# fengpeng-yue/speech-to-speech-translation

Hardware: AMD Instinct MI355X
Metric: mel-frames/sec (fwd+bwd+opt) on Fisher-shaped fbank80->mel80 (higher is better)
Workload: dtype bf16; 1 GPU; s2st_transformer base 12enc/6dec d512 nfps4 + aux ASR/ST(1x64) + CTC, recipe dropouts, max-tokens=20000 Fisher-shaped batches, update-freq 1; parallelism=dp1

## Files before the change

### include/s2st_hip.h

```cpp
#ifndef S2ST_HIP_H
#define S2ST_HIP_H
#include <stdint.h>
#ifdef __cplusplus
extern "C" {
#endif

#define S2ST_OK 0
#define S2ST_ERR_LAUNCH (-1)
#define S2ST_ERR_SHAPE (-2)
#define S2ST_ERR_WORKSPACE (-3)
#define S2ST_ERR_ARG (-4)
#define S2ST_ERR_COMM (-5)

typedef struct { int64_t ld; int64_t bs; int32_t per; int32_t _pad; } s2st_split;

typedef struct {
  const void* p;
  int32_t kmajor;
  int32_t dtype;
  s2st_split sp;
  int64_t zo, zi;
} s2st_gemm_operand;

#define S2ST_F32 0
// ... 53 lines not shown
  float scale, drop_p;
  uint64_t seed;
  int32_t ld_drop;
  const uint16_t* doh;
  float *dq, *dk, *dv;
  uint16_t *dqh, *dkh, *dvh;
  float *dbq, *dbk, *dbv;
} s2st_attn_args;
int s2st_flash_attn_fwd_bf16(const s2st_attn_args* args, void* stream);
int s2st_flash_attn_bwd_bf16(const s2st_attn_args* args, const float* dO, float* dvec_scratch, void* stream);

int s2st_layernorm_fwd_f32(const float* x, const float* gamma, const float* beta, float* y, float* mean, float* rstd, int32_t rows, int32_t cols, float eps, void* stream);

int s2st_layernorm_bwd_f32(const float* dy, const float* x, const float* gamma, const float* mean, const float* rstd, float* dx, int32_t dx_accumulate, float* dgamma, float* dbeta, float* scratch, int32_t rows, int32_t cols, void* stream);
int64_t s2st_layernorm_bwd_scratch(int32_t rows, int32_t cols);

int s2st_softmax_fwd_f32(const float* s, float* p, float* pd, const int32_t* klen, int32_t B, int32_t H, int32_t T, int32_t S, int32_t ld, int32_t causal, float drop_p, uint64_t seed, void* stream);

int s2st_softmax_bwd_f32(const float* p, const float* dpd, float* ds, int32_t B, int32_t H, int32_t T, int32_t S, int32_t ld, float drop_p, uint64_t seed, void* stream);

int s2st_colsum_f32(const float* x, int64_t ld, int32_t rows, int32_t cols, float* out, int32_t accumulate, void* stream);

int s2st_attn_headmean_f32(const float* p, float* out, int32_t B, int32_t H, int32_t T, int32_t S, int32_t ld, void* stream);

int s2st_copy_rows_f32(const float* x, s2st_split xsp, float* y, s2st_split ysp, int32_t rows, int32_t C, void* stream);

int s2st_glu_fwd_f32(const float* a, float* y, s2st_split ysp, int32_t rows, int32_t C, void* stream);

int s2st_glu_bwd_f32(const float* a, const float* dy, s2st_split dysp, float* da, s2st_split dasp, int32_t rows, int32_t C, void* stream);

int s2st_add_pe_f32(const float* x, float* y, const int32_t* pos, const float* table, int32_t rows, int32_t C, float scale, const float* alpha_ptr, float drop_p, uint64_t seed, void* stream);

int s2st_pe_alpha_bwd_f32(const float* dy, const int32_t* pos, const float* table, int32_t rows, int32_t C, float drop_p, uint64_t seed, float* dalpha, void* stream);

int s2st_embed_fwd_f32(const int64_t* tokens, const float* table, float* y, int32_t rows, int32_t C, float scale, void* stream);

int s2st_embed_bwd_f32(const int64_t* tokens, const float* dy, float* dtable, int32_t rows, int32_t C, float scale, int64_t pad, void* stream);
int s2st_embed_bwd_ordered_f32(const int64_t* tokens, const float* dy, float* dtable, int32_t rows, int32_t C, int32_t V, float scale, int64_t pad, void* stream);

int s2st_dropout_f32(const float* x, float* y, int64_t n, float a, float p, uint64_t seed, int32_t accumulate, void* stream);

int s2st_relu_drop_bwd_f32(const float* dy, const float* y, float* dz, int64_t n, float p, void* stream);

int s2st_conv_w_permute_f32(const float* w, float* wf, float* wd, int32_t O, int32_t I, int32_t Kw, void* stream);

int s2st_conv_w_unpermute_acc_f32(const float* dwf, float* dw, int32_t O, int32_t I, int32_t Kw, void* stream);

#define S2ST_BN_TMP_FLOATS(C) (130 * (long)(C))
int s2st_bn_stats_f32(const float* x, int32_t rows, int32_t C, float* mean, float* var, float* run_mean, float* run_var, float momentum, float* tmp, void* stream);

int s2st_bn_apply_f32(const float* x, const float* mean, const float* var, const float* gamma, const float* beta, float* y, s2st_split ysp, const float* resid, int32_t rows, int32_t C, float eps, int32_t tanh_, float drop_p, uint64_t seed, void* stream);

int s2st_bn_bwd_f32(const float* dy, s2st_split dysp, const float* x, const float* mean, const float* var, const float* gamma, const float* beta, float* dx, s2st_split dxsp, float* dgamma, float* dbeta, float* tmp, int32_t rows, int32_t C, float eps, int32_t tanh_, float drop_p, uint64_t seed, void* stream);

int s2st_mel_loss_f32(const float* feat, const float* post, const float* eos, const float* tgt, const int32_t* lens, int32_t B, int32_t D, int32_t F, float pos_weight, float* stats, float c_l1, float c_mse, float c_eos, float* dfeat, float* dpost, float* deos, void* stream);

int s2st_ls_ce_f32(const float* logits, const int64_t* target, int32_t rows, int32_t V, int64_t pad, float eps, float* stats, float* dlogits, float gscale, void* stream);

int s2st_log_softmax_rows_f32(const float* x, int64_t ldx, float* y, int64_t ldy, int32_t rows, int32_t V, int32_t log_out, void* stream);

int s2st_ctc_f32(const float* logits, const int64_t* targets, int32_t Lmax, const int32_t* in_lens, const int32_t* tgt_lens, int32_t B, int32_t E, int32_t V, float* lprobs, float* loss_per_utt, float* dlogits, float gscale, float* ws, void* stream);

int s2st_sumsq_f32(const float* x, int64_t n, float* out, void* stream);
int s2st_sumsq_parts_f32(const float* x, int64_t n, float* parts, void* stream);
int64_t s2st_sumsq_parts_count(int64_t n);

int s2st_adam_f32(float* p, float* g, float* m, float* v, int64_t n, const float* sumsq, float gmul, const float* gmul_dev, float max_norm, float lr, float beta1, float beta2, float eps, float wd, int32_t step, float* gnorm_out, void* p_bf16, int32_t* skipped, int32_t sumsq_parts, int32_t zero_grad, void* stream);

int s2st_grad_pack_bf16_f32(const float* g, uint16_t* out, int64_t n, void* stream);
int s2st_exchange_proxy_f32(const float* bucket, float* scratch, int64_t n, int64_t move_bytes, int32_t wgs, float gbps, void* stream);
int s2st_grad_unpack_bf16_f32(const uint16_t* in, float* g, int64_t n, void* stream);

int64_t s2st_ctc_workspace(int32_t B, int32_t E, int32_t Lmax);

typedef struct {
  int32_t enc_layers, dec_layers, enc_dim, dec_dim, enc_ffn, dec_ffn, enc_heads, dec_heads;
  int32_t enc_pre_ln, dec_pre_ln;
  int32_t in_dim, conv_channels, conv_k;
  int32_t out_dim;
  int32_t prenet_layers, prenet_dim, postnet_layers, postnet_dim, postnet_k;
  int32_t tap_asr, tap_st;
  int32_t has_asr, has_st, has_ctc;
  int32_t asr_layers, asr_dim, st_layers, st_dim, src_vocab, tgt_vocab;
  int32_t no_scale_embedding;
  int32_t precise;
  int32_t tap_dec, has_ctc_tgt;
  int32_t text_input, enc_conv_layers, enc_conv_k;
  int32_t n_speakers, spk_frozen;
  int32_t spk_dim;
  float dropout, attn_dropout, act_dropout, prenet_dropout, postnet_dropout;
  float ctc_weight, asr_weight, st_weight, w_l1, w_mse, w_eos, bce_pos_weight, label_smoothing;
  float ctc_tgt_weight;
  float enc_dropout;
  int32_t s2t_mode;
} s2st_model_config;

typedef struct {
  char name[120];
  int64_t offset;
  int64_t numel;
  int32_t ndim;
  int32_t shape[4];
  int32_t is_buffer;
} s2st_param_info;

typedef struct {
// ... 250 lines not shown
```

### speech-to-speech-translation_amd/csrc/attention.hip

```cpp
#include <cstdlib>
#include <type_traits>

#include "s2st_ops.h"
#include "s2st_prof.h"

namespace {

typedef unsigned short bf16_t;

template <int DH>
struct Img {
  static constexpr int PITCH = DH * 2;
  static constexpr int CH = DH / 8;
  static constexpr int BYTES = 32 * PITCH;
  __device__ static __forceinline__ int trkey(int row) { return DH >= 128 ? (row & 7) : ((row >> 1) & 3); }
  __device__ static __forceinline__ int row_off(int row, int ch) { return row * PITCH + ((ch ^ (row & (CH - 1))) << 4); }
  __device__ static __forceinline__ int tr_off(int row, int ch) {
    return row * PITCH + (((((ch >> 1) ^ trkey(row)) << 1) | (ch & 1)) << 4);
  }
  __device__ static __forceinline__ bf16x8 row_frag(const unsigned char* img, int rt, int ks, int lane) {
    const int row = rt + (lane & 15), ch = 4 * ks + (lane >> 4);
    return *reinterpret_cast<const bf16x8*>(img + row_off(row, ch));
  }
  __device__ static __forceinline__ bf16x8 tr_frag(const unsigned char* img, int dt, int lane) {
// ... 187 lines not shown
#pragma unroll
    for (int t2 = 0; t2 < 2; ++t2) {
      x[t2] = f32x4{0.f, 0.f, 0.f, 0.f};
#pragma unroll
      for (int ks = 0; ks < KS; ++ks)
        x[t2] = __builtin_amdgcn_mfma_f32_16x16x32_bf16(Img<DH>::row_frag(kimg, 16 * t2, ks, lane), qf[ks], x[t2], 0, 0, 0);
    }
    float s[8];
    float mt = -INFINITY;
#pragma unroll
    for (int e = 0; e < 8; ++e) {
      const int key = kt + 16 * (e >> 2) + 4 * g + (e & 3);
      const bool ok = key < klim && (!a.causal || key <= qi);
      s[e] = ok ? x[e >> 2][e & 3] * a.scale : -INFINITY;
      mt = fmaxf(mt, s[e]);
    }
    mt = fmaxf(mt, __shfl_xor(mt, 16));
    mt = fmaxf(mt, __shfl_xor(mt, 32));
    const float mn = fmaxf(m, mt);
    const float mu = mn == -INFINITY ? 0.f : mn;
    const float alpha = __expf(m - mu);
    float p[8], ps = 0.f;
#pragma unroll
    for (int e = 0; e < 8; ++e) {
      p[e] = __expf(s[e] - mu);
      ps += p[e];
    }
    if (a.drop_p > 0.f) {
#pragma unroll
      for (int e = 0; e < 8; ++e)
        p[e] *= drop_scale(a.seed, drow + (uint64_t)(kt + 16 * (e >> 2) + 4 * g + (e & 3)), a.drop_p, inv_keep);
    }
    l = l * alpha + ps;
    m = mn;
    const bf16x8 pf = pack_frag(p);
#pragma unroll
    for (int d = 0; d < DT; ++d) {
      o[d] *= alpha;
      o[d] = __builtin_amdgcn_mfma_f32_16x16x32_bf16(Img<DH>::tr_frag(vimg, d, lane), pf, o[d], 0, 0, 0);
    }
  };
  for (int kt = 0; kt < kmax; kt += 64) {
    tile(stg[0], kt);
    if (kt + 32 < kmax) tile(stg[1], kt + 32);
  }
  l += __shfl_xor(l, 16);
  l += __shfl_xor(l, 32);
  const float inv_l = l > 0.f ? 1.f / l : 0.f;
  if (qi < a.T) {
    const long ro = ((long)b * a.T + qi) * ((long)a.H * DH) + h * DH;
#pragma unroll
    for (int d = 0; d < DT; ++d) {
      const float4 v = make_float4(o[d][0] * inv_l, o[d][1] * inv_l, o[d][2] * inv_l, o[d][3] * inv_l);
      *reinterpret_cast<float4*>(a.o + ro + 16 * d + 4 * g) = v;
      if (a.oh) *reinterpret_cast<uint2*>(a.oh + ro + 16 * d + 4 * g) = pack_bf16x4(v.x, v.y, v.z, v.w);
    }
    if (g == 0 && a.lse) a.lse[(long)bh * a.T + qi] = l > 0.f ? m + __logf(l) : -INFINITY;
  }
}

template <int DH>
__global__ __launch_bounds__(256) void attn_dvec_kernel(const float* __restrict__ dO, const float* __restrict__ O,
                                                        float* __restrict__ D, int B, int H, int T) {
  constexpr int LPR = DH / 4;
  const long row = ((long)blockIdx.x * 256 + threadIdx.x) / LPR;
  const int l = threadIdx.x % LPR;
  const bool ok = row < (long)B * T * H;
  float s = 0.f;
  int h = 0;
  long bt = 0;
  if (ok) {
    h = (int)(row % H);
    bt = row / H;
    const long o = bt * ((long)H * DH) + (long)h * DH + 4 * l;
    const float4 a = *reinterpret_cast<const float4*>(dO + o);
    const float4 c = *reinterpret_cast<const float4*>(O + o);
    s = a.x * c.x + a.y * c.y + a.z * c.z + a.w * c.w;
  }
#pragma unroll
  for (int m = LPR / 2; m >= 1; m >>= 1) s += __shfl_xor(s, m);
  if (ok && l == 0) {
    const int t = (int)(bt % T), bb = (int)(bt / T);
    D[((long)bb * H + h) * T + t] = s;
  }
}

template <int DH, int NW>
__device__ __forceinline__ void flash_bwd_kv_body(const AttnArgs& a, unsigned char* smem, const int bx, const int bh) {
  constexpr int KS = DH / 32, DT = DH / 16;
  unsigned char* q_row = smem;
  unsigned char* q_tr = smem + Img<DH>::BYTES;
  unsigned char* do_row = smem + 2 * Img<DH>::BYTES;
  unsigned char* do_tr = smem + 3 * Img<DH>::BYTES;
  const int tid = threadIdx.x, lane = tid & 63, wave = tid >> 6, g = lane >> 4;
  const int b = bh / a.H, h = bh - b * a.H;
  const int k0 = bx * (16 * NW) + wave * 16;
  const int ki = k0 + (lane & 15);
  const bf16_t* qb = a.q + (long)b * a.T * a.ldq + h * DH;
  const bf16_t* kb = a.k + (long)b * a.S * a.ldk + h * DH;
  const bf16_t* vb = a.v + (long)b * a.S * a.ldv + h * DH;
  const bf16_t* dob = a.doh + (long)b * a.T * ((long)a.H * DH) + h * DH;
  const int klim = a.klen ? min((int)a.klen[b], a.S) : a.S;
  const bool key_ok = ki < klim;
  const int qbeg = a.causal ? (bx * (16 * NW)) & ~31 : 0;

  ATTN_STAMP(0);
  bf16x8 kf[KS], vf[KS];
// ... 474 lines not shown
  const float inv_keep = a.drop_p > 0.f ? 1.f / (1.f - a.drop_p) : 1.f;
  const uint64_t drow = ((uint64_t)bh * a.T + qi) * (uint64_t)a.ld_drop;
  for (int kt = 0; kt < kmax; kt += 32) {
    f32x4 x[2];
#pragma unroll
    for (int t2 = 0; t2 < 2; ++t2) {
      x[t2] = f32x4{0.f, 0.f, 0.f, 0.f};
#pragma unroll
      for (int ks = 0; ks < KS; ++ks)
        x[t2] = __builtin_amdgcn_mfma_f32_16x16x32_bf16(I::row_frag(kimg, kt + 16 * t2, ks, lane), qf[ks], x[t2], 0, 0, 0);
    }
    float sc[8];
    float mt = -INFINITY;
#pragma unroll
    for (int e = 0; e < 8; ++e) {
      const int key = kt + 16 * (e >> 2) + 4 * g + (e & 3);
      const bool ok = key < klim && (!a.causal || key <= qi);
      sc[e] = ok ? x[e >> 2][e & 3] * a.scale : -INFINITY;
      mt = fmaxf(mt, sc[e]);
    }
    mt = fmaxf(mt, __shfl_xor(mt, 16));
    mt = fmaxf(mt, __shfl_xor(mt, 32));
    const float mn = fmaxf(m, mt);
    const float mu = mn == -INFINITY ? 0.f : mn;
    const float alpha = __expf(m - mu);
    float p[8], ps = 0.f;
#pragma unroll
    for (int e = 0; e < 8; ++e) {
      p[e] = __expf(sc[e] - mu);
      ps += p[e];
    }
    if (a.drop_p > 0.f) {
#pragma unroll
      for (int e = 0; e < 8; ++e)
        p[e] *= drop_scale(a.seed, drow + (uint64_t)(kt + 16 * (e >> 2) + 4 * g + (e & 3)), a.drop_p, inv_keep);
    }
    l = l * alpha + ps;
    m = mn;
    const bf16x8 pf = pack_frag(p);
#pragma unroll
    for (int d = 0; d < DT; ++d) {
      o[d] *= alpha;
      o[d] = __builtin_amdgcn_mfma_f32_16x16x32_bf16(I::tr_frag(vimg, kt, d, lane), pf, o[d], 0, 0, 0);
    }
  }
  l += __shfl_xor(l, 16);
  l += __shfl_xor(l, 32);
  const float inv_l = l > 0.f ? 1.f / l : 0.f;
  if (qi < a.T) {
    const long ro = ((long)b * a.T + qi) * ((long)a.H * DH) + h * DH;
#pragma unroll
    for (int d = 0; d < DT; ++d) {
      const float4 v = make_float4(o[d][0] * inv_l, o[d][1] * inv_l, o[d][2] * inv_l, o[d][3] * inv_l);
      *reinterpret_cast<float4*>(a.o + ro + 16 * d + 4 * g) = v;
      if (a.oh) *reinterpret_cast<uint2*>(a.oh + ro + 16 * d + 4 * g) = pack_bf16x4(v.x, v.y, v.z, v.w);
    }
    if (g == 0 && a.lse) a.lse[(long)bh * a.T + qi] = l > 0.f ? m + __logf(l) : -INFINITY;
  }
}

constexpr int ANW = 4;
constexpr int attn_nw() { return ANW; }

bool short_configure() {
  static int ok = -1;
  if (ok < 0) {
    auto set = [](auto kern, int bytes) {
      return hipFuncSetAttribute(reinterpret_cast<const void*>(kern), hipFuncAttributeMaxDynamicSharedMemorySize, bytes) == hipSuccess;
    };
    ok = set(flash_fwd_short_kernel<128, 8>, short_fwd_lds_bytes(128, 128)) && set(flash_fwd_short_kernel<64, 8>, short_fwd_lds_bytes(64, 128)) &&
         set(flash_fwd_short_kernel<128, 4>, short_fwd_lds_bytes(128, 64)) && set(flash_fwd_short_kernel<64, 4>, short_fwd_lds_bytes(64, 64)) &&
         set(flash_bwd_short_kernel<128, 8>, short_lds_bytes(128, 128, 128)) && set(flash_bwd_short_kernel<64, 8>, short_lds_bytes(64, 128, 128)) &&
         set(flash_bwd_short_kernel<128, 4>, short_lds_bytes(128, 64, 64)) && set(flash_bwd_short_kernel<64, 4>, short_lds_bytes(64, 64, 64)) ? 1 : 0;
  }
  return ok == 1;
}
bool short_enabled() {
  const char* e = s2st_env_str("S2ST_ATTN_SHORT");
  return !(e && atoi(e) == 0);
}
bool short_fwd_enabled() { return short_enabled(); }

bool attn_args_ok(const s2st_attn_args& p) {
  auto al = [](const void* x, int n) { return ((uintptr_t)x % n) == 0; };
  return (p.dh == 64 || p.dh == 128) && p.ldq % 8 == 0 && p.ldk % 8 == 0 && p.ldv % 8 == 0 && al(p.q, 16) &&
         al(p.k, 16) && al(p.v, 16) && p.B > 0 && p.H > 0 && p.T > 0 && p.S > 0;
}

AttnArgs to_args(const s2st_attn_args& p) {
  AttnArgs a{};
  a.q = p.q; a.k = p.k; a.v = p.v;
  a.ldq = p.ldq; a.ldk = p.ldk; a.ldv = p.ldv;
  a.o = p.o; a.oh = p.oh; a.lse = p.lse; a.klen = p.klen;
  a.B = p.B; a.H = p.H; a.T = p.T; a.S = p.S; a.causal = p.causal;
  a.scale = p.scale; a.drop_p = p.drop_p; a.seed = p.seed; a.ld_drop = p.ld_drop;
  a.doh = p.doh; a.dq = p.dq; a.dk = p.dk; a.dv = p.dv;
  a.dqh = p.dqh; a.dkh = p.dkh; a.dvh = p.dvh; a.dbq = p.dbq; a.dbk = p.dbk; a.dbv = p.dbv;
  a.plain_order = 0;
  return a;
}

}

int s2st_flash_attn_supported(int dh) { return dh == 64 || dh == 128; }

int s2st_flash_attn_preload(hipStream_t st) {
  AttnArgs a{};
  auto go = [&](auto nwc) {
    constexpr int NW = decltype(nwc)::value;
    S2ST_LAUNCH((flash_fwd_kernel<128, NW>), dim3(1, 1), dim3(64 * NW), 0, st, a);
    S2ST_LAUNCH((flash_fwd_kernel<64, NW>), dim3(1, 1), dim3(64 * NW), 0, st, a);
    S2ST_LAUNCH((flash_bwd_kv_kernel<128, NW>), dim3(1, 1), dim3(64 * NW), 0, st, a);
    S2ST_LAUNCH((flash_bwd_kv_kernel<64, NW>), dim3(1, 1), dim3(64 * NW), 0, st, a);
    S2ST_LAUNCH((flash_bwd_q_kernel<128, NW>), dim3(1, 1), dim3(64 * NW), 0, st, a);
    S2ST_LAUNCH((flash_bwd_q_kernel<64, NW>), dim3(1, 1), dim3(64 * NW), 0, st, a);
    S2ST_LAUNCH((flash_bwd_kernel<128, NW>), dim3(1, 1), dim3(64 * NW), 0, st, a, 1);
    S2ST_LAUNCH((flash_bwd_kernel<64, NW>), dim3(1, 1), dim3(64 * NW), 0, st, a, 1);
  };
  go(std::integral_constant<int, ANW>{});
  if (!short_configure()) return S2ST_ERR_LAUNCH;
  S2ST_LAUNCH((flash_fwd_short_kernel<128, 8>), dim3(1), dim3(512), 0, st, a);
  S2ST_LAUNCH((flash_fwd_short_kernel<64, 8>), dim3(1), dim3(512), 0, st, a);
  S2ST_LAUNCH((flash_fwd_short_kernel<128, 4>), dim3(1), dim3(256), 0, st, a);
  S2ST_LAUNCH((flash_fwd_short_kernel<64, 4>), dim3(1), dim3(256), 0, st, a);
  S2ST_LAUNCH((flash_bwd_short_kernel<128, 8>), dim3(1), dim3(512), 0, st, a);
  S2ST_LAUNCH((flash_bwd_short_kernel<64, 8>), dim3(1), dim3(512), 0, st, a);
  S2ST_LAUNCH((flash_bwd_short_kernel<128, 4>), dim3(1), dim3(256), 0, st, a);
  S2ST_LAUNCH((flash_bwd_short_kernel<64, 4>), dim3(1), dim3(256), 0, st, a);
  return hipGetLastError() == hipSuccess ? 0 : S2ST_ERR_LAUNCH;
}

int s2st_flash_attn_fwd(const s2st_attn_args* p, hipStream_t st) {
  if (!p || !attn_args_ok(*p) || !p->o || !p->lse) return S2ST_ERR_ARG;
  AttnArgs a = to_args(*p);
  if (p->T <= SHORT_MAX && p->S <= SHORT_MAX && short_fwd_enabled() && short_configure()) {
    const double fl = 4.0 * p->B * p->H * (double)p->T * p->S * p->dh * (p->causal ? 0.5 : 1.0);
    const dim3 grid(p->B * p->H);
    const int lds = short_fwd_lds_bytes(p->dh, p->S);
    const bool w4 = p->T <= 64 && p->S <= 64;
    if (p->dh == 128 && w4) s2st_launch("flash_fwd_short_kernel<128, 4>", fl, 0.0, flash_fwd_short_kernel<128, 4>, grid, dim3(256), lds, st, a);
    else if (p->dh == 128) s2st_launch("flash_fwd_short_kernel<128, 8>", fl, 0.0, flash_fwd_short_kernel<128, 8>, grid, dim3(512), lds, st, a);
    else if (w4) s2st_launch("flash_fwd_short_kernel<64, 4>", fl, 0.0, flash_fwd_short_kernel<64, 4>, grid, dim3(256), lds, st, a);
    else s2st_launch("flash_fwd_short_kernel<64, 8>", fl, 0.0, flash_fwd_short_kernel<64, 8>, grid, dim3(512), lds, st, a);
    return hipGetLastError() == hipSuccess ? 0 : S2ST_ERR_LAUNCH;
  }
  auto go = [&](auto nwc) {
    constexpr int NW = decltype(nwc)::value;
    dim3 grid((p->T + 16 * NW - 1) / (16 * NW), p->B * p->H);
    const double fl = 4.0 * p->B * p->H * (double)p->T * p->S * p->dh * (p->causal ? 0.5 : 1.0);
    if (p->dh == 128) s2st_launch("flash_fwd_kernel<128>", fl, 0.0, flash_fwd_kernel<128, NW>, grid, dim3(64 * NW), 0, st, a);
    else s2st_launch("flash_fwd_kernel<64>", fl, 0.0, flash_fwd_kernel<64, NW>, grid, dim3(64 * NW), 0, st, a);
  };
  go(std::integral_constant<int, ANW>{});
  return hipGetLastError() == hipSuccess ? 0 : S2ST_ERR_LAUNCH;
}

long s2st_flash_attn_db_scratch_floats(const s2st_attn_args* p) {
  if (!p || (!p->dbq && !p->dbk && !p->dbv)) return 0;
  const int nw = attn_nw();
  const long C = (long)p->H * p->dh;
  const long sq = (long)p->B * ((p->T + 16 * nw - 1) / (16 * nw)) * nw, sk = (long)p->B * ((p->S + 16 * nw - 1) / (16 * nw)) * nw;
  return (sq + 2 * sk) * C;
}

void s2st_flash_attn_db_layout(const s2st_attn_args* p, int* slots_q, int* slots_k) {
  const int nw = attn_nw();
  *slots_q = p->B * ((p->T + 16 * nw - 1) / (16 * nw)) * nw;
  *slots_k = p->B * ((p->S + 16 * nw - 1) / (16 * nw)) * nw;
}

int s2st_flash_attn_bwd(const s2st_attn_args* p, const float* dO, float* dvec_scratch, hipStream_t st, int phase,
                        float* db_part) {
  if (!p || !attn_args_ok(*p) || !p->doh || (!p->dq && !p->dqh) || (!p->dk && !p->dkh) || (!p->dv && !p->dvh) || !p->lse)
    return S2ST_ERR_ARG;
  const bool own_d = p->oh && phase == 0;
  if (!own_d && (!dO || !dvec_scratch || !p->o)) return S2ST_ERR_ARG;
  AttnArgs a = to_args(*p);
  a.dvec = own_d ? nullptr : dvec_scratch;
#ifdef S2ST_ATTN_STAMP
  a.stamp = reinterpret_cast<long*>(dvec_scratch);
#endif
  const int nwp = attn_nw();
  const long Cp = (long)p->H * p->dh;
  const long slots_q = (long)p->B * ((p->T + 16 * nwp - 1) / (16 * nwp)) * nwp, slots_k = (long)p->B * ((p->S + 16 * nwp - 1) / (16 * nwp)) * nwp;
  const bool part = db_part && phase == 0 && (p->dbq || p->dbk || p->dbv);
  if (part) {
// ... 85 lines not shown
```

### speech-to-speech-translation_amd/csrc/c_api.cpp

```cpp
#include <hip/hip_ext.h>
#include "s2st_ops.h"

extern "C" {

int s2st_version(void) { return 100; }

int s2st_experimental_build(void) {
#ifdef S2ST_EXPERIMENTAL
  return 1;
#else
  return 0;
#endif
}

int s2st_device_count(void) {
  int n = 0;
  if (hipGetDeviceCount(&n) != hipSuccess) return 0;
  return n;
}

int s2st_exchange_proxy_f32(const float* bucket, float* scratch, int64_t n, int64_t move_bytes, int32_t wgs, float gbps, void* stream) {
  return s2st_exchange_proxy(bucket, scratch, (long)n, (long)move_bytes, wgs, gbps, (hipStream_t)stream);
}
int s2st_grad_pack_bf16_f32(const float* g, uint16_t* out, int64_t n, void* stream) {
// ... 50 lines not shown
}

int s2st_glu_bwd_f32(const float* a, const float* dy, s2st_split dysp, float* da, s2st_split dasp, int32_t rows, int32_t C, void* stream) {
  return s2st_glu_bwd(a, dy, dysp, da, dasp, rows, C, (hipStream_t)stream);
}

int s2st_add_pe_f32(const float* x, float* y, const int32_t* pos, const float* table, int32_t rows, int32_t C, float scale, const float* alpha_ptr, float drop_p, uint64_t seed, void* stream) {
  return s2st_add_pe(x, y, pos, table, rows, C, scale, alpha_ptr, drop_p, seed, (hipStream_t)stream);
}

int s2st_pe_alpha_bwd_f32(const float* dy, const int32_t* pos, const float* table, int32_t rows, int32_t C, float drop_p, uint64_t seed, float* dalpha, void* stream) {
  return s2st_pe_alpha_bwd(dy, pos, table, rows, C, drop_p, seed, dalpha, (hipStream_t)stream);
}

int s2st_embed_fwd_f32(const int64_t* tokens, const float* table, float* y, int32_t rows, int32_t C, float scale, void* stream) {
  return s2st_embed_fwd((const long*)tokens, table, y, rows, C, scale, (hipStream_t)stream);
}

int s2st_embed_bwd_f32(const int64_t* tokens, const float* dy, float* dtable, int32_t rows, int32_t C, float scale, int64_t pad, void* stream) {
  return s2st_embed_bwd((const long*)tokens, dy, dtable, rows, C, scale, pad, (hipStream_t)stream);
}

int s2st_embed_bwd_ordered_f32(const int64_t* tokens, const float* dy, float* dtable, int32_t rows, int32_t C, int32_t V, float scale, int64_t pad, void* stream) {
  if (V <= 0) return S2ST_ERR_ARG;
  return s2st_embed_bwd((const long*)tokens, dy, dtable, rows, C, scale, (long)pad, (hipStream_t)stream, V);
}

int s2st_dropout_f32(const float* x, float* y, int64_t n, float a, float p, uint64_t seed, int32_t accumulate, void* stream) {
  return s2st_dropout(x, y, n, a, p, seed, accumulate, (hipStream_t)stream);
}

int s2st_relu_drop_bwd_f32(const float* dy, const float* y, float* dz, int64_t n, float p, void* stream) {
  return s2st_relu_drop_bwd(dy, y, dz, n, p, (hipStream_t)stream);
}

int s2st_conv_w_permute_f32(const float* w, float* wf, float* wd, int32_t O, int32_t I, int32_t Kw, void* stream) {
  return s2st_conv_w_permute(w, wf, wd, O, I, Kw, (hipStream_t)stream);
}

int s2st_conv_w_unpermute_acc_f32(const float* dwf, float* dw, int32_t O, int32_t I, int32_t Kw, void* stream) {
  return s2st_conv_w_unpermute_acc(dwf, dw, O, I, Kw, (hipStream_t)stream);
}

int s2st_bn_stats_f32(const float* x, int32_t rows, int32_t C, float* mean, float* var, float* run_mean, float* run_var, float momentum, float* tmp, void* stream) {
  return s2st_bn_stats(x, rows, C, mean, var, run_mean, run_var, momentum, tmp, (hipStream_t)stream);
}

int s2st_bn_apply_f32(const float* x, const float* mean, const float* var, const float* gamma, const float* beta, float* y, s2st_split ysp, const float* resid, int32_t rows, int32_t C, float eps, int32_t tanh_, float drop_p, uint64_t seed, void* stream) {
  return s2st_bn_apply(x, mean, var, gamma, beta, y, ysp, resid, rows, C, eps, tanh_, drop_p, seed, (hipStream_t)stream);
}

int s2st_bn_bwd_f32(const float* dy, s2st_split dysp, const float* x, const float* mean, const float* var, const float* gamma, const float* beta, float* dx, s2st_split dxsp, float* dgamma, float* dbeta, float* tmp, int32_t rows, int32_t C, float eps, int32_t tanh_, float drop_p, uint64_t seed, void* stream) {
  return s2st_bn_bwd(dy, dysp, x, mean, var, gamma, beta, dx, dxsp, dgamma, dbeta, tmp, rows, C, eps, tanh_, drop_p, seed, (hipStream_t)stream);
}

int s2st_mel_loss_f32(const float* feat, const float* post, const float* eos, const float* tgt, const int32_t* lens, int32_t B, int32_t D, int32_t F, float pos_weight, float* stats, float c_l1, float c_mse, float c_eos, float* dfeat, float* dpost, float* deos, void* stream) {
  return s2st_mel_loss(feat, post, eos, tgt, lens, B, D, F, pos_weight, stats, c_l1, c_mse, c_eos, dfeat, dpost, deos, (hipStream_t)stream);
}

int s2st_ls_ce_f32(const float* logits, const int64_t* target, int32_t rows, int32_t V, int64_t pad, float eps, float* stats, float* dlogits, float gscale, void* stream) {
  return s2st_ls_ce(logits, (const long*)target, rows, V, pad, eps, stats, dlogits, gscale, (hipStream_t)stream);
}

int s2st_ctc_f32(const float* logits, const int64_t* targets, int32_t Lmax, const int32_t* in_lens, const int32_t* tgt_lens, int32_t B, int32_t E, int32_t V, float* lprobs, float* loss_per_utt, float* dlogits, float gscale, float* ws, void* stream) {
  return s2st_ctc(logits, (const long*)targets, Lmax, in_lens, tgt_lens, B, E, V, lprobs, loss_per_utt, dlogits, gscale, ws, (hipStream_t)stream);
}

int s2st_sumsq_parts_f32(const float* x, int64_t n, float* parts, void* stream) {
  return s2st_sumsq_parts(x, n, parts, (hipStream_t)stream);
}
int64_t s2st_sumsq_parts_count(int64_t n) { return s2st_sumsq_nparts((long)n); }
int s2st_sumsq_f32(const float* x, int64_t n, float* out, void* stream) {
  return s2st_sumsq(x, n, out, (hipStream_t)stream);
}

int s2st_adam_f32(float* p, float* g, float* m, float* v, int64_t n, const float* sumsq, float gmul, const float* gmul_dev, float max_norm, float lr, float beta1, float beta2, float eps, float wd, int32_t step, float* gnorm_out, void* p_bf16, int32_t* skipped, int32_t sumsq_parts, int32_t zero_grad, void* stream) {
  return s2st_adam(p, g, m, v, n, sumsq, gmul, gmul_dev, max_norm, lr, beta1, beta2, eps, wd, step, gnorm_out, (hipStream_t)stream, (uint16_t*)p_bf16, skipped, sumsq_parts, zero_grad);
}

int64_t s2st_layernorm_bwd_scratch(int32_t rows, int32_t cols) { return (int64_t)s2st_layernorm_bwd_blocks(rows, cols) * 2 * cols; }
int64_t s2st_ctc_workspace(int32_t B, int32_t E, int32_t Lmax) { return s2st_ctc_workspace_floats(B, E, Lmax); }

int s2st_flash_attn_fwd_bf16(const s2st_attn_args* args, void* stream) { return s2st_flash_attn_fwd(args, (hipStream_t)stream); }
int s2st_flash_attn_bwd_bf16(const s2st_attn_args* args, const float* dO, float* dvec_scratch, void* stream) {
  return s2st_flash_attn_bwd(args, dO, dvec_scratch, (hipStream_t)stream, 0);
}

int s2st_argmax_dim1_f32(const float* x, int64_t* idx, int32_t B, int32_t E, int32_t D, void* stream) {
  return s2st_argmax_dim1(x, (long*)idx, B, E, D, (hipStream_t)stream);
}
int s2st_affine_cols_f32(const float* x, const float* scale, const float* shift, float* y, int64_t rows, int32_t C, void* stream) {
  return s2st_affine_cols(x, scale, shift, y, rows, C, (hipStream_t)stream);
}
int s2st_exp_transpose_f32(const float* x, float* y, int32_t T, int32_t C, void* stream) {
  return s2st_exp_transpose(x, y, T, C, (hipStream_t)stream);
}
int s2st_clamp_min_f32(float* x, int64_t n, float lo, void* stream) { return s2st_clamp_min(x, n, lo, (hipStream_t)stream); }
int s2st_gl_polar_f32(const float* mag, const float* ang, float* X, int32_t F, int32_t T, void* stream) {
  return s2st_gl_polar(mag, ang, X, F, T, (hipStream_t)stream);
}
int s2st_gl_project_f32(const float* mag, const float* Y, float* X, int32_t F, int32_t T, void* stream) {
  return s2st_gl_project(mag, Y, X, F, T, (hipStream_t)stream);
}
int s2st_reflect_pad_f32(const float* x, float* y, int32_t n, int32_t pad, void* stream) {
  return s2st_reflect_pad(x, y, n, pad, (hipStream_t)stream);
}
// ... 156 lines not shown
```

### speech-to-speech-translation_amd/csrc/elementwise.hip

```cpp
#include <cstdlib>

#include "s2st_ops.h"
#include "s2st_prof.h"

namespace {

constexpr int EW_BLOCK = 256;

inline unsigned ew_grid(long n, int per_thread = 1) {
  long b = (n + (long)EW_BLOCK * per_thread - 1) / ((long)EW_BLOCK * per_thread);
  return (unsigned)(b < 1 ? 1 : b);
}

__global__ __launch_bounds__(256) void copy_rows_kernel(const float* __restrict__ x, Split xsp,
                                                        float* __restrict__ y, Split ysp, int rows,
                                                        int C4) {
  long i = (long)blockIdx.x * EW_BLOCK + threadIdx.x;
  long n = (long)rows * C4;
  if (i >= n) return;
  int r = (int)(i / C4), c = (int)(i - (long)r * C4);
  reinterpret_cast<float4*>(y + split_off(ysp, r))[c] =
      reinterpret_cast<const float4*>(x + split_off(xsp, r))[c];
}

// ... 88 lines not shown
  const int local = (int)(id - t.tile0[lo]), tc = (C + 63) / 64;
  const int r0 = (local / tc) * 64, c0 = (local % tc) * 64;
  for (int i = threadIdx.x; i < 64 * 8; i += 256) {
    const int r = i >> 3, c = (i & 7) * 8;
    uint4 v = make_uint4(0, 0, 0, 0);
    if (r0 + r < R && c0 + c < C) v = *reinterpret_cast<const uint4*>(x + (long)(r0 + r) * C + c0 + c);
    *reinterpret_cast<uint4*>(&tile[r][c]) = v;
  }
  __syncthreads();
  for (int i = threadIdx.x; i < 64 * 8; i += 256) {
    const int c = i >> 3, r = (i & 7) * 8;
    if (r0 + r < R && c0 + c < C) {
      unsigned w[4];
#pragma unroll
      for (int j = 0; j < 4; ++j) w[j] = (unsigned)tile[r + 2 * j][c] | ((unsigned)tile[r + 2 * j + 1][c] << 16);
      *reinterpret_cast<uint4*>(y + (long)(c0 + c) * R + r0 + r) = make_uint4(w[0], w[1], w[2], w[3]);
    }
  }
}

__device__ __forceinline__ float sigmoidf_(float v) { return 1.f / (1.f + expf(-v)); }

__global__ __launch_bounds__(256) void glu_fwd_kernel(const float* __restrict__ a,
                                                      float* __restrict__ y, Split ysp, int rows,
                                                      int C) {
  long i = (long)blockIdx.x * EW_BLOCK + threadIdx.x;
  long n = (long)rows * C;
  if (i >= n) return;
  int r = (int)(i / C), c = (int)(i - (long)r * C);
  const float* ar = a + (long)r * 2 * C;
  y[split_off(ysp, r) + c] = ar[c] * sigmoidf_(ar[c + C]);
}

__global__ __launch_bounds__(256) void glu_bwd_kernel(const float* __restrict__ a,
                                                      const float* __restrict__ dy, Split dysp,
                                                      float* __restrict__ da, Split dasp, int rows,
                                                      int C, uint16_t* __restrict__ dah, long ldh) {
  long i = (long)blockIdx.x * EW_BLOCK + threadIdx.x;
  long n = (long)rows * C;
  if (i >= n) return;
  int r = (int)(i / C), c = (int)(i - (long)r * C);
  const float* ar = a + (long)r * 2 * C;
  float g = dy[split_off(dysp, r) + c];
  float s = sigmoidf_(ar[c + C]);
  float* dr = da + split_off(dasp, r);
  const float d0 = g * s, d1 = g * ar[c] * s * (1.f - s);
  dr[c] = d0;
  dr[c + C] = d1;
  if (dah) {
    const unsigned pk = pack_bf16x4(d0, d1, 0.f, 0.f).x;
    dah[(long)r * ldh + c] = (uint16_t)(pk & 0xffffu);
    dah[(long)r * ldh + c + C] = (uint16_t)(pk >> 16);
  }
}

__global__ __launch_bounds__(256) void add_pe_kernel(const float* __restrict__ x,
                                                     float* __restrict__ y,
                                                     const int* __restrict__ pos,
                                                     const float* __restrict__ table, int rows,
                                                     int C, float scale,
                                                     const float* __restrict__ alpha_ptr,
                                                     float drop_p, uint64_t seed,
                                                     const float* __restrict__ spk_table,
                                                     const long* __restrict__ spk_ids, int T) {
  long i = (long)blockIdx.x * EW_BLOCK + threadIdx.x;
  long n = (long)rows * C;
  if (i >= n) return;
  int r = (int)(i / C), c = (int)(i - (long)r * C);
  float alpha = alpha_ptr ? alpha_ptr[0] : 1.f;
  float v = scale * x[i] + alpha * table[(long)pos[r] * C + c];
  if (spk_table) v += spk_table[spk_ids[r / T] * C + c];
  if (drop_p > 0.f) v *= drop_scale(seed, (uint64_t)i, drop_p, 1.f / (1.f - drop_p));
  y[i] = v;
}

__global__ __launch_bounds__(256) void speaker_bwd_kernel(const float* __restrict__ dy, const long* __restrict__ ids, int B,
                                                          int T, int T_sum, int C, int n_spk, float drop_p, uint64_t seed,
                                                          float* __restrict__ dtable) {
  const int c = blockIdx.x * 256 + threadIdx.x, sp = blockIdx.y;
  if (c >= C || sp >= n_spk) return;
  const float inv_keep = drop_p > 0.f ? 1.f / (1.f - drop_p) : 1.f;
  float a = 0.f;
  for (int b = 0; b < B; ++b) {
    if (ids[b] != sp) continue;
    for (int t = 0; t < T_sum; ++t) {
      const long i = ((long)b * T + t) * C + c;
      float g = dy[i];
      if (drop_p > 0.f) g *= drop_scale(seed, (uint64_t)i, drop_p, inv_keep);
      a += g;
    }
  }
  dtable[(long)sp * C + c] += a;
}

__global__ __launch_bounds__(256) void speaker_set_rows_kernel(const float* __restrict__ table, const long* __restrict__ ids,
                                                               float* __restrict__ y, int B, int T, int C) {
  const long i = (long)blockIdx.x * 256 + threadIdx.x;
  if (i >= (long)B * C) return;
  const int b = (int)(i / C), c = (int)(i - (long)b * C);
  y[(long)b * T * C + c] = table[ids[b] * C + c];
}

__global__ __launch_bounds__(256) void speaker_fill_cols_kernel(const float* __restrict__ table, const long* __restrict__ ids,
                                                                float* __restrict__ y, int B, int T, int ld, int coff, int Sd) {
  const long i = (long)blockIdx.x * 256 + threadIdx.x;
  if (i >= (long)B * T * Sd) return;
// ... 260 lines not shown
  }
}
__global__ __launch_bounds__(256) void colreduce2_fold_kernel(const float* __restrict__ part, int slabs, int cols,
                                                              float* __restrict__ out0, float* __restrict__ out1,
                                                              float* __restrict__ acc0, float* __restrict__ acc1) {
  const int c = blockIdx.x * 256 + threadIdx.x;
  if (c >= cols) return;
  float s0 = 0.f, s1 = 0.f;
  for (int sb = 0; sb < slabs; sb += 16) {
    float v0[16], v1[16];
#pragma unroll
    for (int j = 0; j < 16; ++j) {
      const int s = min(sb + j, slabs - 1);
      v0[j] = part[((long)s * 2 + 0) * cols + c];
      v1[j] = part[((long)s * 2 + 1) * cols + c];
    }
#pragma unroll
    for (int j = 0; j < 16; ++j)
      if (sb + j < slabs) {
        s0 += v0[j];
        s1 += v1[j];
      }
  }
  out0[c] = s0;
  if (out1) out1[c] = s1;
  if (acc0) acc0[c] += s0;
  if (acc1) acc1[c] += s1;
}

template <class F>
int colreduce2(F f, int rows, int cols, float* out0, float* out1, float* scratch, hipStream_t st,
               float* acc0 = nullptr, float* acc1 = nullptr, int* slabs_out = nullptr) {
  int cb = (cols + 63) / 64;
  int slabs = (512 + cb - 1) / cb;
  if (slabs > CR_MAX_SLABS) slabs = CR_MAX_SLABS;
  int rpb = (rows + slabs - 1) / slabs;
  if (rpb < 16) rpb = 16;
  slabs = (rows + rpb - 1) / rpb;
  S2ST_LAUNCH((colreduce2_kernel<F>), dim3(cb, slabs), dim3(256), 0, st, f, rows, cols, rpb, scratch);
  if (slabs_out) *slabs_out = slabs;
  if (out0)
    S2ST_LAUNCH(colreduce2_fold_kernel, dim3((cols + 255) / 256), dim3(256), 0, st, (const float*)scratch, slabs,
                       cols, out0, out1, acc0, acc1);
  return hipGetLastError() == hipSuccess ? 0 : S2ST_ERR_LAUNCH;
}

struct ShiftSqF {
  const float* x; int C;
  __device__ float2 operator()(int r, int c) const {
    const float d = x[(long)r * C + c] - x[c];
    return make_float2(d, d * d);
  }
};
__global__ __launch_bounds__(256) void bn_finalize_shift_kernel(const float* __restrict__ x0, const float* __restrict__ part,
                                                                int slabs, float* __restrict__ mean,
                                                                float* __restrict__ var, float* __restrict__ run_mean,
                                                                float* __restrict__ run_var, int C, int rows,
                                                                float momentum) {
  int c = blockIdx.x * EW_BLOCK + threadIdx.x;
  if (c >= C) return;
  float s1 = 0.f, s2 = 0.f;
  for (int sb = 0; sb < slabs; sb += 16) {
    float v1[16], v2[16];
#pragma unroll
    for (int j = 0; j < 16; ++j) {
      const long s = min(sb + j, slabs - 1);
      v1[j] = part[(s * 2 + 0) * C + c];
      v2[j] = part[(s * 2 + 1) * C + c];
    }
#pragma unroll
    for (int j = 0; j < 16; ++j)
      if (sb + j < slabs) { s1 += v1[j]; s2 += v2[j]; }
  }
  const float d1 = s1 / rows;
  const float m = x0[c] + d1;
  const float v = fmaxf(s2 / rows - d1 * d1, 0.f);
  mean[c] = m;
  var[c] = v;
  if (run_mean) {
    run_mean[c] = (1.f - momentum) * run_mean[c] + momentum * m;
    float unb = rows > 1 ? v * ((float)rows / (float)(rows - 1)) : v;
    run_var[c] = (1.f - momentum) * run_var[c] + momentum * unb;
  }
}


__global__ __launch_bounds__(256) void bn_apply_kernel(
    const float* __restrict__ x, const float* __restrict__ mean, const float* __restrict__ var,
    const float* __restrict__ gamma, const float* __restrict__ beta, float* __restrict__ y,
    Split ysp, const float* __restrict__ resid, int rows, int C, float eps, int tanh_, float drop_p,
    uint64_t seed) {
  long i = (long)blockIdx.x * EW_BLOCK + threadIdx.x;
  long n = (long)rows * C;
  if (i >= n) return;
  int r = (int)(i / C), c = (int)(i - (long)r * C);
  float u = gamma[c] * (x[i] - mean[c]) * rsqrtf(var[c] + eps) + beta[c];
  if (tanh_ == 1) u = tanhf(u);
  else if (tanh_ == 2) u = fmaxf(u, 0.f);
  if (drop_p > 0.f) u *= drop_scale(seed, (uint64_t)i, drop_p, 1.f / (1.f - drop_p));
  if (resid) u += resid[i];
  y[split_off(ysp, r) + c] = u;
}

__global__ __launch_bounds__(256) void bn_apply_img_kernel(
    const float* __restrict__ x, const float* __restrict__ mean, const float* __restrict__ var,
    const float* __restrict__ gamma, const float* __restrict__ beta, float* __restrict__ y, uint16_t* __restrict__ img,
    int B, int T, int pad, int C4, float eps, int tanh_, float drop_p, uint64_t seed) {
  const long i = (long)blockIdx.x * EW_BLOCK + threadIdx.x;
  const int Th = T + 2 * pad;
  if (i >= (long)B * Th * C4) return;
  const int c = (int)(i % C4) * 4;
  const long bu = i / C4;
  const int u = (int)(bu % Th), b = (int)(bu / Th);
  uint2 h = make_uint2(0u, 0u);
  if (u >= pad && u < pad + T) {
    const long e0 = ((long)b * T + (u - pad)) * (4L * C4) + c;
    const float4 xv = *reinterpret_cast<const float4*>(x + e0);
    const float xs[4] = {xv.x, xv.y, xv.z, xv.w};
    float o[4];
#pragma unroll
    for (int k = 0; k < 4; ++k) {
      float t = gamma[c + k] * (xs[k] - mean[c + k]) * rsqrtf(var[c + k] + eps) + beta[c + k];
      if (tanh_ == 1) t = tanhf(t);
      else if (tanh_ == 2) t = fmaxf(t, 0.f);
      if (drop_p > 0.f) t *= drop_scale(seed, (uint64_t)(e0 + k), drop_p, 1.f / (1.f - drop_p));
      o[k] = t;
    }
    if (y) *reinterpret_cast<float4*>(y + e0) = make_float4(o[0], o[1], o[2], o[3]);
    h = pack_bf16x4(o[0], o[1], o[2], o[3]);
  }
  reinterpret_cast<uint2*>(img)[i] = h;
}

struct BnBwdF {
  const float* dy; Split dysp; const float* x; const float* mean; const float* var;
  const float* gamma; const float* beta; int C; float eps; int tanh_; float drop_p; uint64_t seed;
  __device__ float2 operator()(int r, int c) const {
    long i = (long)r * C + c;
    float xh = (x[i] - mean[c]) * rsqrtf(var[c] + eps);
    float g = dy[split_off(dysp, r) + c];
    if (drop_p > 0.f) g *= drop_scale(seed, (uint64_t)i, drop_p, 1.f / (1.f - drop_p));
    if (tanh_ == 1) {
      float t = tanhf(gamma[c] * xh + beta[c]);
      g *= (1.f - t * t);
    } else if (tanh_ == 2) {
      g = (gamma[c] * xh + beta[c]) > 0.f ? g : 0.f;
    }
    return make_float2(g, g * xh);
  }
};

__global__ __launch_bounds__(256) void bn_bwd_dx_kernel(BnBwdF f, const float* __restrict__ sums,
                                                        float* __restrict__ dx, Split dxsp,
                                                        int rows, int C, uint16_t* __restrict__ dxh, long ldh) {
  long i = (long)blockIdx.x * EW_BLOCK + threadIdx.x;
  long n = (long)rows * C;
  if (i >= n) return;
  int r = (int)(i / C), c = (int)(i - (long)r * C);
  float2 v = f(r, c);
  float rstd = rsqrtf(f.var[c] + f.eps);
  float xh = (f.x[i] - f.mean[c]) * rstd;
  float inv = 1.f / rows;
  const float d = f.gamma[c] * rstd * (v.x - sums[c] * inv - xh * sums[C + c] * inv);
  dx[split_off(dxsp, r) + c] = d;
  if (dxh) dxh[(long)r * ldh + c] = (uint16_t)(pack_bf16x4(d, 0.f, 0.f, 0.f).x & 0xffffu);
}

__global__ __launch_bounds__(256) void add_vec_kernel(const float* __restrict__ a,
                                                      float* __restrict__ b, int n) {
  int i = blockIdx.x * EW_BLOCK + threadIdx.x;
  if (i < n) b[i] += a[i];
}

}

#define LAUNCH_OK() (hipGetLastError() == hipSuccess ? 0 : S2ST_ERR_LAUNCH)

int s2st_copy_rows(const float* x, Split xsp, float* y, Split ysp, int rows, int C,
                   hipStream_t st) {
  if (rows <= 0) return 0;
  if (C % 4) return S2ST_ERR_SHAPE;
  long n = (long)rows * (C / 4);
  S2ST_LAUNCH(copy_rows_kernel, dim3(ew_grid(n)), dim3(EW_BLOCK), 0, st, x, xsp, y, ysp, rows, C / 4);
  return LAUNCH_OK();
}

int s2st_copy_rows_bf16(const uint16_t* x, Split xsp, uint16_t* y, Split ysp, int rows, int C, hipStream_t st) {
  if (rows <= 0 || C <= 0) return 0;
  if (C % 4 || xsp.ld % 4 || ysp.ld % 4 || xsp.bs % 4 || ysp.bs % 4 || ((uintptr_t)x % 8) || ((uintptr_t)y % 8))
    return S2ST_ERR_SHAPE;
  long n = (long)rows * (C / 4);
  S2ST_LAUNCH(copy_rows_bf16_kernel, dim3(ew_grid(n)), dim3(EW_BLOCK), 0, st, x, xsp, y, ysp, rows, C / 4);
  return LAUNCH_OK();
}

int s2st_halo_image_bf16(const uint16_t* x, long ldx, uint16_t* y, int B, int Tout, int Th, int O, int pad, int stride,
                         hipStream_t st) {
  if (B <= 0 || Th <= 0 || O <= 0) return 0;
  if (O % 8 || ldx % 8 || stride < 1 || ((uintptr_t)x % 16) || ((uintptr_t)y % 16)) return S2ST_ERR_SHAPE;
  const long n = (long)B * Th * (O / 8);
  S2ST_LAUNCH(halo_image_bf16_kernel, dim3(ew_grid(n)), dim3(EW_BLOCK), 0, st, x, ldx, y, B, Tout, Th, O / 8, pad, stride);
  return LAUNCH_OK();
}

int s2st_cast_bf16_halo(const float* x, uint16_t* y, int B, int T, int pad, int C, hipStream_t st, int plain) {
  if (B <= 0 || T + 2 * pad <= 0 || C <= 0) return 0;
  if (C % 4 || ((uintptr_t)x % 16) || ((uintptr_t)y % 8)) return S2ST_ERR_SHAPE;
  const long n = (long)B * (T + 2 * pad) * (C / 4);
  S2ST_LAUNCH(cast_bf16_halo_kernel, dim3(ew_grid(n)), dim3(EW_BLOCK), 0, st, x, y, B, T, pad, C / 4, plain);
  return LAUNCH_OK();
}

int s2st_cast_bf16_rows(const float* x, long ldx, uint16_t* y, long ldy, long rows, int cols, hipStream_t st) {
  if (rows <= 0 || cols <= 0) return 0;
  if (ldy % 4 != 0 || ldy < cols) return S2ST_ERR_SHAPE;
  const int vec = ((uintptr_t)x % 16 == 0) && (ldx % 4 == 0);
  long n = rows * (ldy >> 2);
  S2ST_LAUNCH(cast_bf16_rows_kernel, dim3(ew_grid(n)), dim3(EW_BLOCK), 0, st, x, ldx, y, ldy, rows, cols, vec);
  return hipGetLastError() == hipSuccess ? 0 : S2ST_ERR_LAUNCH;
}

int s2st_transpose_bf16(const uint16_t* x, uint16_t* y, int R, int C, hipStream_t st) {
  if (R <= 0 || C <= 0) return 0;
  S2ST_LAUNCH(transpose_bf16_kernel, dim3((C + 63) / 64, (R + 63) / 64), dim3(256), 0, st, x, y, R, C);
  return hipGetLastError() == hipSuccess ? 0 : S2ST_ERR_LAUNCH;
}

int s2st_transpose_bf16_batched(const uint16_t* x_base, uint16_t* y_base, const s2st_transpose_table& t, hipStream_t st) {
  if (t.n <= 0) return 0;
  if (t.n > S2ST_TRANSPOSE_MAX) return S2ST_ERR_ARG;
  S2ST_LAUNCH(transpose_bf16_batched_kernel, dim3(t.tile0[t.n]), dim3(256), 0, st, x_base, y_base, t);
  return hipGetLastError() == hipSuccess ? 0 : S2ST_ERR_LAUNCH;
}

int s2st_glu_fwd(const float* a, float* y, Split ysp, int rows, int C, hipStream_t st) {
  long n = (long)rows * C;
  if (n <= 0) return 0;
  S2ST_LAUNCH(glu_fwd_kernel, dim3(ew_grid(n)), dim3(EW_BLOCK), 0, st, a, y, ysp, rows, C);
  return LAUNCH_OK();
}

int s2st_glu_bwd(const float* a, const float* dy, Split dysp, float* da, Split dasp, int rows,
                 int C, hipStream_t st, uint16_t* dah, long ldh) {
  long n = (long)rows * C;
  if (n <= 0) return 0;
  S2ST_LAUNCH(glu_bwd_kernel, dim3(ew_grid(n)), dim3(EW_BLOCK), 0, st, a, dy, dysp, da, dasp, rows, C, dah, ldh);
  return LAUNCH_OK();
}

int s2st_add_pe(const float* x, float* y, const int* pos, const float* table, int rows, int C,
                float scale, const float* alpha_ptr, float drop_p, uint64_t seed, hipStream_t st,
                const float* spk_table, const long* spk_ids, int T) {
  long n = (long)rows * C;
  if (n <= 0) return 0;
  if (spk_table && (!spk_ids || T <= 0)) return S2ST_ERR_ARG;
  S2ST_LAUNCH(add_pe_kernel, dim3(ew_grid(n)), dim3(EW_BLOCK), 0, st, x, y, pos, table, rows, C,
                     scale, alpha_ptr, drop_p, seed, spk_table, spk_ids, T > 0 ? T : 1);
  return LAUNCH_OK();
}

int s2st_speaker_bwd(const float* dy, const long* ids, int B, int T, int T_sum, int C, int n_spk, float drop_p,
                     uint64_t seed, float* dtable, hipStream_t st) {
  if (B <= 0 || C <= 0 || n_spk <= 0) return 0;
  S2ST_LAUNCH(speaker_bwd_kernel, dim3((C + 255) / 256, n_spk), dim3(256), 0, st, dy, ids, B, T, T_sum, C, n_spk, drop_p,
              seed, dtable);
  return LAUNCH_OK();
}

int s2st_speaker_fill_cols(const float* table, const long* ids, float* y, int B, int T, int ld, int coff, int Sd, hipStream_t st) {
  if (B <= 0 || T <= 0 || Sd <= 0) return 0;
  if (!table || !ids || !y || coff < 0 || coff + Sd > ld) return S2ST_ERR_ARG;
  S2ST_LAUNCH(speaker_fill_cols_kernel, dim3((unsigned)(((long)B * T * Sd + 255) / 256)), dim3(256), 0, st, table, ids, y, B, T,
              ld, coff, Sd);
  return LAUNCH_OK();
}

int s2st_speaker_cols_bwd(const float* dy, const long* ids, int B, int T, int ld, int coff, int Sd, int n_spk, float* dtable,
                          hipStream_t st) {
  if (B <= 0 || T <= 0 || Sd <= 0 || n_spk <= 0) return 0;
  if (!dy || !ids || !dtable || coff < 0 || coff + Sd > ld) return S2ST_ERR_ARG;
  S2ST_LAUNCH(speaker_cols_bwd_kernel, dim3((Sd + 255) / 256, n_spk), dim3(256), 0, st, dy, ids, B, T, ld, coff, Sd, n_spk, dtable);
  return LAUNCH_OK();
}

int s2st_split_cols(const float* g, int ldg, float* dx, int ldx, int rows, int C, int acc, hipStream_t st) {
  if (rows <= 0 || C <= 0) return 0;
  if (!g || !dx || C > ldg || C > ldx) return S2ST_ERR_ARG;
  S2ST_LAUNCH(split_cols_kernel, dim3((unsigned)(((long)rows * C + 255) / 256)), dim3(256), 0, st, g, ldg, dx, ldx, rows, C, acc);
  return LAUNCH_OK();
}

// ... 127 lines not shown
  dim3 grid(cb, slabs);
  if (!dbias) part = nullptr;
  if (mode == 0) S2ST_LAUNCH(dpre_kernel<0>, grid, dim3(256), 0, st, dy, y, yb, dph, ldp, dpre, dbias, M, N, rpb, p, ik, seed, part);
  else if (mode == 1) S2ST_LAUNCH(dpre_kernel<1>, grid, dim3(256), 0, st, dy, y, yb, dph, ldp, dpre, dbias, M, N, rpb, p, ik, seed, part);
  else S2ST_LAUNCH(dpre_kernel<2>, grid, dim3(256), 0, st, dy, y, yb, dph, ldp, dpre, dbias, M, N, rpb, p, ik, seed, part);
  if (part && slabs_out) { *slabs_out = slabs; return LAUNCH_OK(); }
  if (part) return s2st_colsum_fold(part, slabs, N, dbias, st);
  return LAUNCH_OK();
}

int s2st_axpy(const float* x, float* y, long n, float a, hipStream_t st) {
  if (n <= 0) return 0;
  S2ST_LAUNCH(axpy_kernel, dim3(ew_grid(n)), dim3(EW_BLOCK), 0, st, x, y, n, a);
  return LAUNCH_OK();
}

int s2st_scale(float* x, long n, float a, hipStream_t st) {
  if (n <= 0) return 0;
  S2ST_LAUNCH(scale_kernel, dim3(ew_grid(n)), dim3(EW_BLOCK), 0, st, x, n, a);
  return LAUNCH_OK();
}

int s2st_conv_w_permute(const float* w, float* wf, float* wd, int O, int I, int Kw, hipStream_t st, uint16_t* wfh,
                        uint16_t* wdh) {
  long n = (long)O * I * Kw;
  if (n <= 0) return 0;
  if (O >= 32 && I >= 32 && Kw <= 64) {
    S2ST_LAUNCH(conv_w_permute_tiled_kernel, dim3((I + 31) / 32, (O + 31) / 32, Kw), dim3(256), 0, st, w, wf, wd, O, I, Kw,
                wfh, wdh);
    return LAUNCH_OK();
  }
  S2ST_LAUNCH(conv_w_permute_kernel, dim3(ew_grid(n)), dim3(EW_BLOCK), 0, st, w, wf, wd, O, I, Kw, wfh, wdh);
  return LAUNCH_OK();
}

int s2st_conv_w_unpermute_acc(const float* dwf, float* dw, int O, int I, int Kw, hipStream_t st, int slabs) {
  long n = (long)O * I * Kw;
  if (n <= 0) return 0;
  S2ST_LAUNCH(conv_w_unpermute_acc_kernel, dim3(ew_grid(n)), dim3(EW_BLOCK), 0, st, dwf, dw, O, I, Kw, slabs < 1 ? 1 : slabs);
  return LAUNCH_OK();
}

int s2st_bn_stats(const float* x, int rows, int C, float* mean, float* var, float* run_mean,
                  float* run_var, float momentum, float* tmp, hipStream_t st) {
  if (rows <= 0 || C <= 0) return 0;
  int slabs = 0;
  int rc = colreduce2(ShiftSqF{x, C}, rows, C, nullptr, nullptr, tmp + 2 * (long)C, st, nullptr, nullptr, &slabs);
  if (rc) return rc;
  S2ST_LAUNCH(bn_finalize_shift_kernel, dim3((C + EW_BLOCK - 1) / EW_BLOCK), dim3(EW_BLOCK), 0, st, x,
              (const float*)(tmp + 2 * (long)C), slabs, mean, var, run_mean, run_var, C, rows, momentum);
  return LAUNCH_OK();
}

int s2st_bn_apply(const float* x, const float* mean, const float* var, const float* gamma,
                  const float* beta, float* y, Split ysp, const float* resid, int rows, int C,
                  float eps, int tanh_, float drop_p, uint64_t seed, hipStream_t st) {
  long n = (long)rows * C;
  if (n <= 0) return 0;
  S2ST_LAUNCH(bn_apply_kernel, dim3(ew_grid(n)), dim3(EW_BLOCK), 0, st, x, mean, var, gamma,
                     beta, y, ysp, resid, rows, C, eps, tanh_, drop_p, seed);
  return LAUNCH_OK();
}

int s2st_bn_apply_img(const float* x, const float* mean, const float* var, const float* gamma, const float* beta, float* y,
                      uint16_t* img, int B, int T, int pad, int C, float eps, int tanh_, float drop_p, uint64_t seed,
                      hipStream_t st) {
  if (B <= 0 || T <= 0 || C <= 0) return 0;
  if (C % 4 || ((uintptr_t)x % 16) || ((uintptr_t)img % 8) || (y && (uintptr_t)y % 16)) return S2ST_ERR_SHAPE;
  const long n = (long)B * (T + 2 * pad) * (C / 4);
  S2ST_LAUNCH(bn_apply_img_kernel, dim3(ew_grid(n)), dim3(EW_BLOCK), 0, st, x, mean, var, gamma, beta, y, img, B, T, pad, C / 4,
              eps, tanh_, drop_p, seed);
  return LAUNCH_OK();
}

int s2st_bn_bwd(const float* dy, Split dysp, const float* x, const float* mean, const float* var,
                const float* gamma, const float* beta, float* dx, Split dxsp, float* dgamma,
                float* dbeta, float* tmp, int rows, int C, float eps, int tanh_, float drop_p,
                uint64_t seed, hipStream_t st, uint16_t* dxh, long ldh) {
  long n = (long)rows * C;
  if (n <= 0) return 0;
  BnBwdF f{dy, dysp, x, mean, var, gamma, beta, C, eps, tanh_, drop_p, seed};
  int rc = colreduce2(f, rows, C, tmp, tmp + C, tmp + 2 * (long)C, st, dbeta, dgamma);
  if (rc) return rc;
  S2ST_LAUNCH(bn_bwd_dx_kernel, dim3(ew_grid(n)), dim3(EW_BLOCK), 0, st, f, tmp, dx, dxsp, rows, C, dxh, ldh);
  return LAUNCH_OK();
}
```

### speech-to-speech-translation_amd/csrc/engine.cpp

```cpp
#include <cmath>
#include <cstdio>
#include <cstdlib>
#include <cstring>
#include <functional>
#include <string>
#include <vector>

#include "s2st_ops.h"
#include <hip/hip_ext.h>

namespace {

struct PInfo {
  std::string name;
  long off, numel;
  int ndim;
  int shape[4];
  int is_buffer;
};

struct Ten {
  float* d = nullptr;
  float* g = nullptr;
  bf16raw* h = nullptr;
  bf16raw* gh = nullptr;
  int rows = 0, cols = 0;
  bool needs_grad = true;
  bool want_gh = false;
  int act_mode = 0;
  float act_p = 0.f;
  long act_bias = -1;
  bool drop2_ok = false, ln_seen = false;
  float drop2_p = 0.f;
  uint64_t drop2_seed = 0;
  long drop2_bias = -1;
  bool lin_plain = false;
  bf16raw* gpre_h = nullptr;
  long n() const { return (long)rows * cols; }
  int hld() const { return (cols + 7) & ~7; }
};

struct LinP { long w, b; int N, K; };
struct LNP { long g, b; int C; };
struct AttnP { long kvq_w, kvq_b, out_w, out_b; };
struct XAttnP { long kv_w, kv_b, q_w, q_b, out_w, out_b; };
struct EncLayerP { AttnP sa; LNP ln1; LinP fc1, fc2; LNP ln2; };
struct DecLayerP { AttnP sa; LNP ln1; XAttnP xa; LNP ln2; LinP fc1, fc2; LNP ln3; };
struct ConvP { long w, b; int O, I, Kw; };
struct BNP { long g, b, rm, rv; int C; };
struct AuxP {
  long embed; int V, in_dim, d, layers, out_dim;
  long proj_in;
  std::vector<DecLayerP> L;
  LNP ln; bool has_ln;
  long proj_out;
  long out_proj;
};

}

struct s2st_engine {
  s2st_model_config c;
  std::vector<PInfo> infos;
  long n_params = 0, n_buffers = 0;
  float *P = nullptr, *G = nullptr, *BUF = nullptr;
  hipStream_t side_ = nullptr;
  hipEvent_t ev_fork_ = nullptr, ev_join_ = nullptr, ev_taps_ = nullptr;
  bool overlap_aux = true;
  bool hoist_kv = true;
  hipEvent_t ev_kv_ = nullptr;
  bool kv_wait_ = false;
  hipEvent_t ev_auxb_ = nullptr;
  size_t aux_wait_idx = 0, aux_lo_idx = 0, aux_hi_idx = 0;
  bool aux_bwd_on_side = false;
  int dec_overlap = 3;
  hipEvent_t ev_head_ = nullptr;
  bool side_events_ = false;
  size_t tail_lo_idx = 0, tail_hi_idx = 0;
  bool tail_bwd_on_side = false, tail_side_ = false;
  bool dec_early_active = false;
  size_t xattn0_idx = 0;
// ... 68 lines not shown
  int chain_parts(int rows, Part* p) {
    if (chain_count(rows) == 1) {
      if (live()) sync_chains();
      p[0] = Part{0, rows, st_, 0};
      return 1;
    }
    const int per = rows / bt.B, b0 = bt.B / 2;
    if (live()) ensure_forked();
    p[0] = Part{0, b0 * per, main_, 0};
    p[1] = Part{b0 * per, rows - b0 * per, chain1_, CHAIN_SALT};
    return 2;
  }
  void ensure_forked() {
    if (forked_) return;
    hipEventRecord(ev_cfork_, main_);
    hipStreamWaitEvent(chain1_, ev_cfork_, 0);
    forked_ = true;
  }
  void sync_chains() {
    if (!forked_) return;
    hipEventRecord(ev_cjoin_, chain1_);
    hipStreamWaitEvent(main_, ev_cjoin_, 0);
    forked_ = false;
  }
  void set_aware() {
    tape_aware.resize(tape.size(), 0);
    if (!tape.empty()) tape_aware.back() = in_region_ ? 1 : 0;
  }
  void chains_wait(hipEvent_t ev) {
    if (forked_) hipStreamWaitEvent(chain1_, ev, 0);
  }
  const s2st_decode_replay* replay_ = nullptr;
  const int* dec_row_map = nullptr;
  bool stop_after_encoder = false;
  Ten* enc_out_keep = nullptr;
  struct Dec {
    float* base = nullptr; int B = 0, E = 0, maxT = 0; const int* enc_lens = nullptr; const float* pe_dec = nullptr;
    float* pe_alpha = nullptr;
  } dec_st;
  float* dec_selfK(int l) const { return dec_st.base + (long)l * 2 * dec_st.B * dec_st.maxT * c.dec_dim; }
  float* dec_selfV(int l) const { return dec_selfK(l) + (long)dec_st.B * dec_st.maxT * c.dec_dim; }
  float* dec_crossKV(int l) const {
    return dec_st.base + (long)c.dec_layers * 2 * dec_st.B * dec_st.maxT * c.dec_dim + (long)l * dec_st.B * dec_st.E * 2 * c.dec_dim;
  }
  bool use_ln_skinny = true;
  bool use_skinny = true;
  bool use_ln_fuse = true;
  bool use_only_h = true;
  bool use_attn_gfuse = true;
  int attn_gfuse_mode = 1;
  bool ordered_sums = true;
  bool use_act_fuse = true;
  bool use_flash = true;
  int ffn_act = 1;
  bool is_hubert = false;
  s2st_hubert_config hc{};
  struct HubP {
    long conv_w[8]; long gn_g, gn_b; LNP ln; LinP proj; long pos_w, pos_b; std::vector<EncLayerP> L; LNP enc_ln;
  } hp;
  float* ws_for(hipStream_t s) const { return (side_ && s == side_) ? skws_side : ((chain1_ && s == chain1_) ? skws_c1 : skws); }
  float* skws = nullptr;
  long skws_n = 0;
  bool ph_fresh = false;
  bf16raw* PHT = nullptr;
  bool pht_valid = false;
  struct WT { long off; int N, K; };
  std::vector<WT> wt_list;
  void reg_wt(long off, int N, int K) { if (N % 8 == 0 && K % 8 == 0) wt_list.push_back(WT{off, N, K}); }
  bool has_wt(long off, int N, int K) const {
    if (!pht_valid) return false;
    for (const WT& t : wt_list) if (t.off == off && t.N == N && t.K == K) return true;
    return false;
  }
  std::vector<s2st_transpose_table> wt_tables;
  void build_wt_tables() {
    s2st_transpose_table cur{};
    for (const WT& t : wt_list) {
      if (cur.n == S2ST_TRANSPOSE_MAX) { wt_tables.push_back(cur); cur = s2st_transpose_table{}; }
      const int i = cur.n++;
      cur.off[i] = (unsigned)t.off; cur.rows8[i] = (unsigned short)(t.N / 8); cur.cols8[i] = (unsigned short)(t.K / 8);
      cur.tile0[i + 1] = cur.tile0[i] + (unsigned)(((t.N + 63) / 64) * ((t.K + 63) / 64));
    }
    if (cur.n) wt_tables.push_back(cur);
  }
  bf16raw* PH = nullptr;
  bool f32_operands = false;
  bool fast() const { return c.precise == 0 && !f32_operands; }

  ConvP sub[2];
  std::vector<EncLayerP> enc;
  LNP enc_ln; bool has_enc_ln = false;
  LNP asr_norm, st_norm;
  long pos_alpha = 0;
  std::vector<LinP> prenet;
  std::vector<DecLayerP> dec;
  LNP dec_ln; bool has_dec_ln = false;
  LinP feat_proj, eos_proj;
  std::vector<ConvP> post_conv;
  std::vector<BNP> post_bn;
  LinP ctc_proj, ctc_proj_tgt;
  AuxP asr, st;
  AuxP s2t;

  float* ws = nullptr;
  long ws_cap = 0, ws_top = 0, ws_peak = 0;
  bool dry = false, oom = false;
// ... 612 lines not shown
```

### speech-to-speech-translation_amd/csrc/engine_convnets.h

```cpp
  ConvW make_conv_scratch(const ConvP& p, bool need_wd, bool tr) {
    ConvW s;
    const bool fm = fast();
    long n = (long)p.O * p.I * p.Kw;
    s.wf = fm ? nullptr : alloc(n);
    s.wd = (need_wd && !fm) ? alloc(n) : nullptr;
    s.dwf = alloc(n, tr);
    bf16raw* wfh = fm ? alloc_h((n + 7) / 8 * 8) : nullptr;
    bf16raw* wdh = fm && need_wd ? alloc_h((n + 7) / 8 * 8) : nullptr;
    if (live() && adam_pending && st_ != side_) adam_wait_upto(p.w + n);
    if (live()) chk(s2st_conv_w_permute(P + p.w, s.wf, s.wd, p.O, p.I, p.Kw, st_, wfh, wdh));
    s.wfh = wfh;
    s.wdh = wdh;
    return s;
  }

  Ten* postnet(Ten* feat, int B, int D, bool tr, std::vector<ConvW>& csp, float* post_out) {
    const bool fm = fast();
    Ten* cur = feat;
    const int pp = c.postnet_k / 2;
    float* curh = fm ? nullptr : alloc((long)B * (D + 2 * pp) * c.out_dim, true);
    if (live() && !fm) {
      Split xs{(long)c.out_dim, 0, 0, 0};
      Split ys{(long)c.out_dim, (long)(D + 2 * pp) * c.out_dim, D, 0};
      chk(s2st_copy_rows(feat->d, xs, curh + (long)pp * c.out_dim, ys, B * D, c.out_dim, st_));
    }
    const bf16raw* curhh = fm ? cast_halo(feat->d, B, D, pp, c.out_dim, true) : nullptr;
    Ten* post = nullptr;
    float* bn_tmp = alloc(S2ST_BN_TMP_FLOATS(c.postnet_dim > c.out_dim ? c.postnet_dim : c.out_dim));
    for (int i = 0; i < c.postnet_layers; ++i) {
      const ConvP& pc = post_conv[i];
      const BNP& bn = post_bn[i];
      const bool last = i == c.postnet_layers - 1;
      Ten* z = conv(ConvIn{curh, cur, D, curhh}, pc, B, 1, csp[i]);
      float* mean = alloc(bn.C);
      float* var = alloc(bn.C);
      touch(bn.b + bn.C);
      const float pdrop = tr ? c.postnet_dropout : 0.f;
      const uint64_t sd = pdrop > 0.f ? next_seed(S2ST_SITE_NORM, pdrop, (long)B * D, bn.C) : 0;
      float* nexth = nullptr;
      bf16raw* nexthh = nullptr;
      Ten* out;
      Split osp;
      if (last) {
        out = newT(B * D, bn.C, post_out);
        osp = Split{(long)bn.C, 0, 0, 0};
      } else if (fm) {
        nexthh = alloc_h(((long)B * (D + 2 * pp) * bn.C + 7) / 8 * 8);
        out = newT(B * D, bn.C, nullptr, false);
        osp = Split{(long)bn.C, 0, 0, 0};
      } else {
        nexth = alloc((long)B * (D + 2 * pp) * bn.C, true);
        out = newT(B * D, bn.C, nexth + (long)pp * bn.C);
        osp = Split{(long)bn.C, (long)(D + 2 * pp) * bn.C, D, 0};
      }
      if (live()) {
        const float *m = BUF + bn.rm, *v = BUF + bn.rv;
        if (tr) {
          chk(s2st_bn_stats(z->d, B * D, bn.C, mean, var, BUF + bn.rm, BUF + bn.rv, 0.1f, bn_tmp, st_));
          m = mean; v = var;
        }
        if (nexthh)
          chk(s2st_bn_apply_img(z->d, m, v, P + bn.g, P + bn.b, nullptr, nexthh, B, D, pp, bn.C, 1e-5f, 1, pdrop, sd, st_));
        else
          chk(s2st_bn_apply(z->d, m, v, P + bn.g, P + bn.b, out->d, osp, last ? feat->d : nullptr, B * D,
                            bn.C, 1e-5f, last ? 0 : 1, pdrop, sd, st_));
      }
      BNP bnp = bn;
      tape.push_back([=]() {
        if (!out->g) return;
        if (last) {
          bool acc;
          float* df = gradbuf(feat, acc);
          if (live()) chk(s2st_dropout(out->g, df, feat->n(), 1.f, 0.f, 0, acc ? 1 : 0, st_));
        }
        bool acc;
        float* dz = gradbuf(z, acc);
        (void)acc;
        Split ps{(long)bnp.C, 0, 0, 0};
        if (fast() && !z->gh) z->gh = alloc_h((long)z->rows * z->hld());
        if (live())
          chk(s2st_bn_bwd(out->g, ps, z->d, mean, var, P + bnp.g, P + bnp.b, dz, ps, G + bnp.g, G + bnp.b,
                          bn_tmp, B * D, bnp.C, 1e-5f, last ? 0 : 1, pdrop, sd, st_, z->gh, z->hld()));
      });
      cur = out;
      curh = nexth;
      curhh = nexthh;
      if (last) post = out;
    }
    return post;
  }

  Ten* text_prenet(Ten* emb, int B, int T, bool tr, std::vector<ConvW>& csp) {
    const bool fm = fast();
    const int C = c.enc_dim, pp = c.enc_conv_k / 2;
    Ten* cur = emb;
    float* curh = fm ? nullptr : alloc((long)B * (T + 2 * pp) * C, true);
    if (live() && !fm) {
      Split xs{(long)C, 0, 0, 0};
      Split ys{(long)C, (long)(T + 2 * pp) * C, T, 0};
      chk(s2st_copy_rows(emb->d, xs, curh + (long)pp * C, ys, B * T, C, st_));
    }
    const bf16raw* curhh = fm ? cast_halo(emb->d, B, T, pp, C, true) : nullptr;
    float* bn_tmp = alloc(S2ST_BN_TMP_FLOATS(C));
    const int n = (int)enc_conv.size();
    for (int i = 0; i < n; ++i) {
      const ConvP& pc = enc_conv[i];
      const BNP& bn = enc_bn[i];
      const bool last = i == n - 1;
      Ten* z = conv(ConvIn{curh, cur, T, curhh}, pc, B, 1, csp[i]);
      float* mean = alloc(C);
      float* var = alloc(C);
      touch(bn.b + C);
      const float pdrop = tr ? c.enc_dropout : 0.f;
      const uint64_t sd = pdrop > 0.f ? next_seed(S2ST_SITE_NORM, pdrop, (long)B * T, C) : 0;
      float* nexth = nullptr;
      bf16raw* nexthh = nullptr;
      Ten* out;
      Split osp;
      if (last) {
        out = newT(B * T, C);
        osp = Split{(long)C, 0, 0, 0};
      } else if (fm) {
        nexthh = alloc_h(((long)B * (T + 2 * pp) * C + 7) / 8 * 8);
        out = newT(B * T, C, nullptr, false);
        osp = Split{(long)C, 0, 0, 0};
      } else {
        nexth = alloc((long)B * (T + 2 * pp) * C, true);
        out = newT(B * T, C, nexth + (long)pp * C);
        osp = Split{(long)C, (long)(T + 2 * pp) * C, T, 0};
      }
      if (live()) {
        const float *m = BUF + bn.rm, *v = BUF + bn.rv;
        if (tr) {
          chk(s2st_bn_stats(z->d, B * T, C, mean, var, BUF + bn.rm, BUF + bn.rv, 0.1f, bn_tmp, st_));
          m = mean; v = var;
        }
        if (nexthh)
          chk(s2st_bn_apply_img(z->d, m, v, P + bn.g, P + bn.b, nullptr, nexthh, B, T, pp, C, 1e-5f, 2 , pdrop, sd, st_));
        else
          chk(s2st_bn_apply(z->d, m, v, P + bn.g, P + bn.b, out->d, osp, nullptr, B * T, C, 1e-5f, 2 , pdrop, sd, st_));
      }
      BNP bnp = bn;
      tape.push_back([=]() {
        if (!out->g) return;
        bool acc;
        float* dz = gradbuf(z, acc);
        (void)acc;
        Split ps{(long)bnp.C, 0, 0, 0};
        if (fast() && !z->gh) z->gh = alloc_h((long)z->rows * z->hld());
        if (live())
          chk(s2st_bn_bwd(out->g, ps, z->d, mean, var, P + bnp.g, P + bnp.b, dz, ps, G + bnp.g, G + bnp.b, bn_tmp, B * T,
                          bnp.C, 1e-5f, 2, pdrop, sd, st_, z->gh, z->hld()));
      });
      cur = out;
      curh = nexth;
      curhh = nexthh;
    }
    return cur;
  }
```

### speech-to-speech-translation_amd/csrc/engine_ops.h

```cpp
  Ten* linear(Ten* x, long w, long b, int N, int K, int act = 0, float drop_p = 0.f,
              Ten* resid = nullptr, float* ext_out = nullptr, bool only_h = false, const float* resid_row = nullptr) {
    const int M = x->rows;
    const bool fm = fast();
    const bool skinny = fm && !bt.training && use_skinny && M <= S2ST_SKINNY_MAX_ROWS && K % 32 == 0 && x->d && x->cols == K &&
                        (act == 0 || act == 1 || act == 3);
    only_h = only_h && fast() && use_only_h && N % 8 == 0 && !ext_out && !resid && !skinny;
    Ten* y = newT(M, N, ext_out, !only_h);
    touch(w + (long)N * K);
    if (b >= 0) touch(b + N);
    const uint64_t sd = drop_p > 0.f ? next_seed(S2ST_SITE_LINEAR, drop_p, M, N) : 0;
    if (skinny) {
      const uint64_t* seed_ptr = nullptr;
      if (replay_ && drop_p > 0.f) {
        if (site < 1 || site > 8) { if (!err) err = S2ST_ERR_SHAPE; return y; }
        seed_ptr = replay_->seeds + (site - 1);
      }
      if (live())
        chk(s2st_gemm_skinny(x->d, K, PH + w, K, y->d, N, b >= 0 ? P + b : nullptr, act, drop_p, sd,
                             resid ? resid->d : resid_row, resid ? N : 0, M, N, K, st_, nullptr, nullptr, 1e-5f, seed_ptr,
                             drop_p > 0.f ? dec_row_map : nullptr));
      return y;
    }
    if (replay_ && drop_p > 0.f && !err) err = S2ST_ERR_SHAPE;
    const bf16raw* xh = fm ? half_of(x) : nullptr;
// ... 70 lines not shown
          if (live()) chk(s2st_relu_drop_bwd(dy, y->d, dpre, y->n(), drop_p, st_));
        } else if (drop_p > 0.f) {
          dpre = alloc(y->n());
          if (live()) chk(s2st_dropout(dy, dpre, y->n(), 1.f, drop_p, sd, 0, st_));
        }
        if (fm) {
          bf16raw* t = alloc_h((long)M * ldp);
          if (live()) chk(s2st_cast_bf16_rows(dpre, N, t, ldp, M, N, st_));
          dph = t;
        }
      }
      float* cpart = (b >= 0 && !bias_done && ordered_sums) ? alloc(s2st_colsum_scratch_floats(M, N)) : nullptr;
      if (live()) {
        GemmArgs g{};
        g.A = fm ? gemm_colmajor(dph, ldp) : gemm_colmajor(dpre, N);
        g.B = fm ? gemm_colmajor(xh, x->hld()) : gemm_colmajor(x->d, x->cols);
        g.C = gemm_out(G + w, K);
        g.ep = gemm_epi_default();
        g.ep.accumulate = 1;
        constexpr bool on_main = false;
        g.M = N; g.N = K; g.K = M; g.batch = 1; g.zdiv = 1; g.precise = c.precise;
        if (fm && !on_main && group_wgrad && s2st_gemm_group_ok(g)) {
          push_wgrad(g);
        } else {
          if (!(fm && !on_main)) sync_chains();
          hipStream_t ws_st = fm && !on_main ? fork_side() : st_;
          g.ws = ws_for(ws_st); g.ws_floats = skws_n;
          chk(s2st_gemm(g, ws_st));
        }
        if (b >= 0 && !bias_done) {
          int slabs = 0;
          chk(s2st_colsum(dpre, N, M, N, G + b, 1, st_, cpart, cpart ? &slabs : nullptr));
          if (cpart) add_fold(cpart, slabs, N, G + b);
        }
      }
      if (x->needs_grad) {
        bool acc;
        float* dx = gradbuf(x, acc);
        if (fm && !acc && x->want_gh && x->hld() == x->cols) x->gh = alloc_h(x->n());
        const bool fuse_act = fm && !acc && x->act_mode == 1 && x->h && x->hld() == x->cols && use_act_fuse;
        if (fuse_act) x->gpre_h = alloc_h(x->n());
        float* cs_part[2] = {nullptr, nullptr};
        for (int ci = 0; ci < nb; ++ci)
          cs_part[ci] = (fuse_act && ordered_sums && x->act_bias >= 0) ? alloc((long)2 * ((M + 63) / 64) * K) : nullptr;
        if (live()) {
          if (nb == 2) ensure_forked();
          for (int ci = 0; ci < nb; ++ci) {
            const long r0 = bp[ci].r0;
            GemmArgs g{};
            g.A = fm ? gemm_rowmajor(dph + r0 * ldp, ldp) : gemm_rowmajor(dpre + r0 * N, N);
            g.B = fm ? (has_wt(w, N, K) ? gemm_rowmajor(PHT + w, N) : gemm_colmajor(PH + w, K)) : gemm_colmajor(P + w, K);
            g.C = gemm_out(dx + r0 * x->cols, x->cols);
            if (fm && !acc && x->gh) g.C.h = x->gh + r0 * x->cols;
            g.ep = gemm_epi_default();
            if (fuse_act) {
              g.C.p = nullptr;
              g.C.h = x->gpre_h + r0 * x->cols;
              g.ep.mask_y = x->h + r0 * x->cols;
              g.ep.mask_scale = x->act_p > 0.f ? 1.f / (1.f - x->act_p) : 1.f;
              g.ep.colsum = x->act_bias >= 0 ? G + x->act_bias : nullptr;
            }
            g.ep.accumulate = acc ? 1 : 0;
            g.ws = ws_for(bp[ci].st); g.ws_floats = skws_n;
            g.M = bp[ci].nr; g.N = K; g.K = N; g.batch = 1; g.zdiv = 1; g.precise = c.precise;
            if (fuse_act && g.ep.colsum && ordered_sums) {
              g.ep.colsum_part = cs_part[ci];
              int tile = 0;
              chk(s2st_gemm(g, bp[ci].st, &tile));
              const int bm = tile / 1000;
              if (bm > 0) add_fold(cs_part[ci], 2 * ((bp[ci].nr + bm - 1) / bm), K, g.ep.colsum);
              else if (!err) err = S2ST_ERR_LAUNCH;
            } else
            chk(s2st_gemm(g, bp[ci].st));
          }
        }
      }
    });
    set_aware();
    return y;
  }

  Ten* ln_linear(Ten* x, const LNP& ln, long w, long b, int N, int K, int act = 0, float* ext_out = nullptr) {
    const bool fused = fast() && !bt.training && use_skinny && use_ln_skinny && x->rows <= S2ST_SKINNY_MAX_ROWS && K % 64 == 0 &&
                       x->d && x->cols == K && (act == 0 || act == 1 || act == 3);
    if (!fused) return linear(layernorm(x, ln), w, b, N, K, act, 0.f, nullptr, ext_out);
    Ten* y = newT(x->rows, N, ext_out);
    touch(w + (long)N * K);
    if (b >= 0) touch(b + N);
    touch(ln.b + ln.C);
    if (live())
      chk(s2st_gemm_skinny(x->d, K, PH + w, K, y->d, N, b >= 0 ? P + b : nullptr, act, 0.f, 0, nullptr, 0, x->rows, N, K,
                           st_, P + ln.g, P + ln.b, 1e-5f));
    return y;
  }

  Ten* layernorm(Ten* x, const LNP& p, float* ext_out = nullptr, bool only_h = false) {
    only_h = only_h && fast() && use_only_h && x->cols % 8 == 0 && !ext_out;
    Ten* y = newT(x->rows, x->cols, ext_out, !only_h);
    float* mean = alloc(x->rows);
    float* rstd = alloc(x->rows);
    touch(p.b + p.C);
    if (fast() && x->cols % 8 == 0) y->h = alloc_h(y->n());
    Part pt[2];
    const int np = chain_parts(x->rows, pt);
    if (live())
      for (int ci = 0; ci < np; ++ci) {
// ... 9 lines not shown
      if (!y->g) return;
      const bool region_was = in_region_;
      in_region_ = region;
      struct Restore { bool& r; bool v; ~Restore() { r = v; } } restore_{in_region_, region_was};
      Part bp[2];
      const int nb = chain_parts(x->rows, bp);
      bool acc;
      float* dx = gradbuf(x, acc);
      const bool fuse = fuse_cand && !x->gpre_h;
      float* scratch = alloc((long)s2st_layernorm_bwd_blocks(x->rows, x->cols) * (fuse ? 3 : 2) * x->cols);
      float* scratch1 = nb == 2 ? alloc((long)s2st_layernorm_bwd_blocks(x->rows, x->cols) * (fuse ? 3 : 2) * x->cols) : nullptr;
      bf16raw* dph = nullptr;
      if (fuse) dph = x->gpre_h = alloc_h(x->n());
      float* dbias = fuse && x->drop2_bias >= 0 ? G + x->drop2_bias : nullptr;
      if (live()) {
        if (nb == 2) ensure_forked();
        if (!ln_bwd_split) {
          for (int ci = 0; ci < nb; ++ci) {
            const long r0 = bp[ci].r0, o = r0 * x->cols;
            float* sc = ci == 0 ? scratch : scratch1;
            chk(s2st_layernorm_bwd(y->g + o, x->d + o, P + pp.g, mean + r0, rstd + r0, dx + o, acc ? 1 : 0, G + pp.g, G + pp.b, sc,
                                   bp[ci].nr, x->cols, bp[ci].st, 3, dph ? dph + o : nullptr, x->drop2_p, x->drop2_seed ^ bp[ci].salt,
                                   dbias));
            if (pending_lnfold.n == S2ST_LNFOLD_MAX) flush_lnfold();
            chk(s2st_lnfold_add(pending_lnfold, sc, bp[ci].nr, x->cols, fuse ? 3 : 2, G + pp.g, G + pp.b, dbias));
          }
        } else {
          auto pass = [&](int ci, int phase, hipStream_t st) {
            const long r0 = bp[ci].r0, o = r0 * x->cols;
            chk(s2st_layernorm_bwd(y->g + o, x->d + o, P + pp.g, mean + r0, rstd + r0, dx + o, acc ? 1 : 0, G + pp.g, G + pp.b,
                                   ci == 0 ? scratch : scratch1, bp[ci].nr, x->cols, st, phase, dph ? dph + o : nullptr, x->drop2_p,
                                   x->drop2_seed ^ bp[ci].salt, dbias));
          };
          for (int ci = 0; ci < nb; ++ci) pass(ci, 1, bp[ci].st);
          hipStream_t rs = side_ ? fork_side() : (sync_chains(), st_);
          for (int ci = 0; ci < nb; ++ci) pass(ci, 2, rs);
        }
      }
    });
    set_aware();
    return y;
  }

  struct AttnIO {
    Ten* qt; int qoff, ldq;
    Ten* kt; int koff, ldk;
    Ten* vt; int voff, ldv;
  };
  Ten* attention(const AttnIO& io, int B, int T, int S, int H, int dh, const int* klen, int causal,
                 float drop_p, float* attn_mean_out ) {
    const int C = H * dh;
    const int ld = (S + 7) / 8 * 8;
    const bool fm = fast();
    Ten* o = newT(B * T, C);
    o->want_gh = true;
    if (fm && C % 8 == 0) o->h = alloc_h(o->n());
    if (fm && use_flash && s2st_flash_attn_supported(dh) && !attn_mean_out && o->h && io.ldq % 8 == 0 &&
        io.ldk % 8 == 0 && io.ldv % 8 == 0) {
      const uint64_t sd = drop_p > 0.f ? next_seed(S2ST_SITE_ATTN, drop_p, B, H, T, S, ld) : 0;
      float* lse = alloc((long)B * H * T);
      s2st_attn_args fa{};
      fa.q = half_of(io.qt) + io.qoff; fa.k = half_of(io.kt) + io.koff; fa.v = half_of(io.vt) + io.voff;
      fa.ldq = io.ldq; fa.ldk = io.ldk; fa.ldv = io.ldv;
      fa.o = o->d; fa.oh = o->h; fa.lse = lse; fa.klen = klen;
      fa.B = B; fa.H = H; fa.T = T; fa.S = S; fa.dh = dh; fa.causal = causal;
      fa.scale = 1.0f / sqrtf((float)dh); fa.drop_p = drop_p; fa.seed = sd; fa.ld_drop = ld;
      auto chain_args = [=](s2st_attn_args a, int b0, int nbat, uint64_t salt) {
        a.q += (long)b0 * T * a.ldq; a.k += (long)b0 * S * a.ldk; a.v += (long)b0 * S * a.ldv;
        a.o += (long)b0 * T * C; if (a.oh) a.oh += (long)b0 * T * C;
        a.lse += (long)b0 * H * T; if (a.klen) a.klen += b0;
        if (a.doh) a.doh += (long)b0 * T * C;
        if (a.dq) a.dq += (long)b0 * T * a.ldq; if (a.dk) a.dk += (long)b0 * S * a.ldk; if (a.dv) a.dv += (long)b0 * S * a.ldv;
        if (a.dqh) a.dqh += (long)b0 * T * a.ldq; if (a.dkh) a.dkh += (long)b0 * S * a.ldk; if (a.dvh) a.dvh += (long)b0 * S * a.ldv;
        a.B = nbat; a.seed ^= salt;
        return a;
      };
      Part pt[2];
      const int np = chain_parts(B * T, pt);
      if (live())
        for (int ci = 0; ci < np; ++ci) {
          const s2st_attn_args a = chain_args(fa, pt[ci].r0 / T, pt[ci].nr / T, pt[ci].salt);
          chk(s2st_flash_attn_fwd(&a, pt[ci].st));
        }
      AttnIO io3 = io;
      const bool region = in_region_;
      tape.push_back([=]() {
        if (!o->g) return;
        const bool region_was = in_region_;
        in_region_ = region;
        struct Restore { bool& r; bool v; ~Restore() { r = v; } } restore_{in_region_, region_was};
        float* dvec = alloc((long)B * H * T);
        s2st_attn_args fb = fa;
        fb.doh = ghalf_of(o);
        Part bp[2];
        const int nb = chain_parts(B * T, bp);
        const bool gf = use_attn_gfuse && io3.qt->lin_plain && io3.kt->lin_plain && io3.vt->lin_plain &&
                        !io3.qt->g && !io3.kt->g && !io3.vt->g;
        if (gf) {
          for (Ten* t : {io3.qt, io3.kt, io3.vt})
            if (!t->gpre_h) t->gpre_h = alloc_h(t->n());
          fb.dqh = io3.qt->gpre_h + io3.qoff; fb.dkh = io3.kt->gpre_h + io3.koff; fb.dvh = io3.vt->gpre_h + io3.voff;
        } else {
          bool aq, ak, av;
          float* gq = gradbuf(io3.qt, aq);
          float* gk = gradbuf(io3.kt, ak);
          float* gv = gradbuf(io3.vt, av);
          (void)aq; (void)ak; (void)av;
          fb.dq = gq + io3.qoff; fb.dk = gk + io3.koff; fb.dv = gv + io3.voff;
        }
        const bool gf_db = gf && attn_gfuse_mode != 3;
        float* dbp[2] = {nullptr, nullptr};
        if (gf_db) {
          if (io3.qt->act_bias >= 0) fb.dbq = G + io3.qt->act_bias + io3.qoff;
          if (io3.kt->act_bias >= 0) fb.dbk = G + io3.kt->act_bias + io3.koff;
          if (io3.vt->act_bias >= 0) fb.dbv = G + io3.vt->act_bias + io3.voff;
          if (attn_gfuse_mode != 2)
            for (int ci = 0; ci < nb; ++ci) dbp[ci] = alloc(s2st_flash_attn_db_scratch_floats(&fb));
        }
        for (int ci = 0; ci < nb; ++ci) {
          const int b0 = bp[ci].r0 / T, nbat = bp[ci].nr / T;
          const s2st_attn_args a = chain_args(fb, b0, nbat, bp[ci].salt);
          if (live()) chk(s2st_flash_attn_bwd(&a, o->g + (long)b0 * T * C, dvec + (long)b0 * H * T, bp[ci].st, 0, dbp[ci]));
// ... 114 lines not shown
    }
    AttnIO io{q, 0, C, kv, 0, 2 * C, kv, C, 2 * C};
    Ten* o = attention(io, B, T, S, H, C / H, klen, 0, bt.training ? c.attn_dropout : 0.f, attn_mean_out);
    if (kv_pre && !xattn0_idx) xattn0_idx = tape.size() - 1;
    return linear(o, a.out_w, a.out_b, C, C, 0, bt.training ? c.dropout : 0.f, resid);
  }
  Ten* ffn_block(Ten* x, const LinP& fc1, const LinP& fc2, Ten* resid) {
    Ten* h = linear(x, fc1.w, fc1.b, fc1.N, fc1.K, ffn_act, bt.training ? c.act_dropout : 0.f, nullptr, nullptr,
                    ffn_act == 1 || is_hubert || is_w2v);
    return linear(h, fc2.w, fc2.b, fc2.N, fc2.K, 0, bt.training ? c.dropout : 0.f, resid);
  }
  Ten* enc_layer(Ten* x, const EncLayerP& l, int B, int T) {
    const int H = c.enc_heads;
    if (c.enc_pre_ln) {
      x = self_attn_block(layernorm(x, l.ln1, nullptr, true), l.sa, B, T, H, bt.enc_lens, 0, x);
      return ffn_block(layernorm(x, l.ln2, nullptr, true), l.fc1, l.fc2, x);
    }
    x = layernorm(self_attn_block(x, l.sa, B, T, H, bt.enc_lens, 0, x), l.ln1);
    return layernorm(ffn_block(x, l.fc1, l.fc2, x), l.ln2);
  }
  struct DecHead { Ten* x = nullptr; Ten* q = nullptr; };
  DecHead dec_head(Ten* x, const DecLayerP& l, int B, int T, int H, bool pre_ln, const int* self_klen) {
    DecHead h;
    Ten* xn;
    if (pre_ln) {
      h.x = self_attn_block(layernorm(x, l.ln1, nullptr, true), l.sa, B, T, H, self_klen, 1, x);
      xn = layernorm(h.x, l.ln2, nullptr, true);
    } else {
      h.x = xn = layernorm(self_attn_block(x, l.sa, B, T, H, self_klen, 1, x), l.ln1);
    }
    const int C = xn->cols;
    h.q = linear(xn, l.xa.q_w, l.xa.q_b, C, C, 0, 0.f, nullptr, nullptr, true);
    return h;
  }
  Ten* dec_layer(Ten* x, Ten* encx, const DecLayerP& l, int B, int T, int S, int H, bool pre_ln,
                 const int* self_klen, float* attn_mean_out, Ten* kv_pre = nullptr, const DecHead* head = nullptr) {
    const DecHead h = head ? *head : dec_head(x, l, B, T, H, pre_ln, self_klen);
    x = cross_attn_block(h.q, encx, l.xa, B, T, S, H, bt.enc_lens, h.x, attn_mean_out, kv_pre);
    if (pre_ln) return ffn_block(layernorm(x, l.ln3, nullptr, true), l.fc1, l.fc2, x);
    x = layernorm(x, l.ln2);
    return layernorm(ffn_block(x, l.fc1, l.fc2, x), l.ln3);
  }

  struct ConvIn { float* xh; Ten* src; int Tin; const bf16raw* xhh; };
  struct ConvW { float *wf, *wd, *dwf; const bf16raw *wfh, *wdh; };
  Ten* conv(const ConvIn& in, const ConvP& p, int B, int stride, const ConvW& cw) {
    float *wf = cw.wf, *wd = cw.wd, *dwf = cw.dwf;
    const bf16raw *wfh = cw.wfh, *wdh = cw.wdh;
    const bool fm = fast();
    const int pad = p.Kw / 2;
    const int Tin = in.Tin, Tout = (Tin + 2 * pad - p.Kw) / stride + 1;
    const int Th = Tin + 2 * pad;
    Ten* z = newT(B * Tout, p.O);
    touch(p.w + (long)p.O * p.I * p.Kw);
    touch(p.b + p.O);
    if (live()) {
      GemmArgs g{};
      g.A = fm ? gemm_rowmajor(in.xhh, (long)stride * p.I) : gemm_rowmajor(in.xh, (long)stride * p.I);
      g.A.sp.per = Tout; g.A.sp.bs = (long)Th * p.I;
      g.B = fm ? gemm_rowmajor(wfh, (long)p.Kw * p.I) : gemm_rowmajor(wf, (long)p.Kw * p.I);
      g.C = gemm_out(z->d, p.O);
      g.ep = gemm_epi_default();
      g.ep.bias = P + p.b;
      g.M = B * Tout; g.N = p.O; g.K = p.Kw * p.I; g.batch = 1; g.zdiv = 1; g.precise = c.precise;
      chk(s2st_gemm(g, st_));
    }
    ConvP pp = p;
    ConvIn in2 = in;
    tape.push_back([=]() {
      if (!z->g) return;
      const int M = B * Tout;
      const bf16raw* dzh = fm ? ghalf_of(z) : nullptr;
      float* cpart = ordered_sums ? alloc(s2st_colsum_scratch_floats(M, pp.O)) : nullptr;
      const bool no_dgrad = !(in2.src && in2.src->needs_grad);
      const bool direct = fm && pp.O % 8 == 0;
      const bool need_img = !no_dgrad;
      float* up = (need_img && !direct) ? alloc((long)B * Th * pp.O, true) : nullptr;
      bf16raw* upd = (need_img && direct) ? alloc_h((long)B * Th * pp.O) : nullptr;
      if (need_img && live()) {
        Split xs{(long)pp.O, 0, 0, 0};
        Split ys{(long)stride * pp.O, (long)Th * pp.O, Tout, 0};
        if (direct) {
          chk(s2st_halo_image_bf16(dzh, z->hld(), upd, B, Tout, Th, pp.O, pad, stride, st_));
        } else {
          chk(s2st_copy_rows(z->g, xs, up + (long)pad * pp.O, ys, M, pp.O, st_));
        }
      }
      if (live()) {
        hipStream_t side_st = fm ? fork_side() : st_;
        hipStream_t ws_st = (fm && !no_dgrad) ? side_st : st_;
        {
          GemmArgs g{};
          g.A = fm ? gemm_colmajor(dzh, z->hld()) : gemm_colmajor(z->g, pp.O);
          g.B = fm ? gemm_colmajor(in2.xhh, (long)stride * pp.I) : gemm_colmajor(in2.xh, (long)stride * pp.I);
          g.B.sp.per = Tout; g.B.sp.bs = (long)Th * pp.I;
          g.C = gemm_out(dwf, (long)pp.Kw * pp.I);
          g.ep = gemm_epi_default();
          g.ep.accumulate = 1;
          g.ws = ws_for(ws_st); g.ws_floats = skws_n;
          g.M = pp.O; g.N = pp.Kw * pp.I; g.K = M; g.batch = 1; g.zdiv = 1; g.precise = c.precise;
          chk(s2st_gemm(g, ws_st));
        }
        {
          int slabs = 0;
          chk(s2st_colsum(z->g, pp.O, M, pp.O, G + pp.b, 1, side_st, cpart, cpart ? &slabs : nullptr));
          if (cpart) add_fold(cpart, slabs, pp.O, G + pp.b);
        }
        chk(s2st_conv_w_unpermute_acc(dwf, G + pp.w, pp.O, pp.I, pp.Kw, ws_st, 1));
      }
      if (!no_dgrad) {
        bool acc;
        float* dx = gradbuf(in2.src, acc);
        const bf16raw* uph = direct ? upd : (fm ? cast_buf(up, (long)B * Th * pp.O) : nullptr);
        if (live()) {
          GemmArgs g{};
          g.A = fm ? gemm_rowmajor(uph, pp.O) : gemm_rowmajor(up, pp.O);
          g.A.sp.per = Tin; g.A.sp.bs = (long)Th * pp.O;
          g.B = fm ? gemm_rowmajor(wdh, (long)pp.Kw * pp.O) : gemm_rowmajor(wd, (long)pp.Kw * pp.O);
          g.C = gemm_out(dx, pp.I);
          g.ep = gemm_epi_default();
          g.ep.accumulate = acc ? 1 : 0;
          g.ws = ws_for(st_); g.ws_floats = skws_n;
          g.M = B * Tin; g.N = pp.I; g.K = pp.Kw * pp.O; g.batch = 1; g.zdiv = 1; g.precise = c.precise;
          chk(s2st_gemm(g, st_));
        }
      }
    });
    return z;
  }

  Ten* glu_to(Ten* z, float* y, Split ysp, int Cc) {
    Ten* holder = newT(z->rows, Cc, y);
    if (live()) chk(s2st_glu_fwd(z->d, y, ysp, z->rows, Cc, st_));
    tape.push_back([=]() {
      if (!holder->g) return;
      bool acc;
      float* dz = gradbuf(z, acc);
      (void)acc;
      Split ds{(long)Cc, 0, 0, 0}, das{(long)2 * Cc, 0, 0, 0};
      if (fast() && !z->gh) z->gh = alloc_h((long)z->rows * z->hld());
      if (live()) chk(s2st_glu_bwd(z->d, holder->g, ds, dz, das, z->rows, Cc, st_, z->gh, z->hld()));
    });
    return holder;
  }

  Ten* add_pe(Ten* x, const int* pos, const float* table, float scale, long alpha_off, float drop_p, long spk_off = -1,
              int T = 0) {
    Ten* y = newT(x->rows, x->cols);
    const uint64_t sd = drop_p > 0.f ? next_seed(S2ST_SITE_ROWS, drop_p, x->rows, x->cols) : 0;
    if (alpha_off >= 0) touch(alpha_off + 1);
    const bool spk = spk_off >= 0 && bt.speaker != nullptr;
    if (spk) touch_spk(spk_off + (long)c.n_speakers * x->cols);
    const long* spk_ids = (const long*)bt.speaker;
    const int Bn = T > 0 ? x->rows / T : 0;
    if (live())
      chk(s2st_add_pe(x->d, y->d, pos, table, x->rows, x->cols, scale, alpha_off >= 0 ? P + alpha_off : nullptr,
                      drop_p, sd, st_, spk ? spk_tab(spk_off) : nullptr, spk ? spk_ids : nullptr, T));
    tape.push_back([=]() {
      if (!y->g) return;
      if (spk && !c.spk_frozen && live())
        chk(s2st_speaker_bwd(y->g, spk_ids, Bn, T, T, x->cols, c.n_speakers, drop_p, sd, G + spk_off, st_));
      float* apart = (alpha_off >= 0 && ordered_sums) ? alloc(1024) : nullptr;
      if (alpha_off >= 0 && live()) {
        int np = 0;
        chk(s2st_pe_alpha_bwd(y->g, pos, table, x->rows, x->cols, drop_p, sd, G + alpha_off, st_, apart, apart ? &np : nullptr));
        if (apart) add_fold(apart, np, 1, G + alpha_off);
      }
      if (x->needs_grad) {
        bool acc;
        float* dx = gradbuf(x, acc);
        if (live()) chk(s2st_dropout(y->g, dx, x->n(), scale, drop_p, sd, acc ? 1 : 0, st_));
      }
    });
    return y;
  }

  Ten* aux_decoder(const AuxP& a, Ten* tap, const long* prev_tok, const int* pos, const int* lens, int B,
                   int L, const float* pe, float* logits_out) {
    const int E = bt.E;
    Ten* emb = newT(B * L, a.in_dim);
    const float scale = c.no_scale_embedding ? 1.f : sqrtf((float)a.d);
    touch(a.embed + (long)a.V * a.in_dim);
    if (live()) chk(s2st_embed_fwd(prev_tok, P + a.embed, emb->d, B * L, a.in_dim, scale, st_));
    long embed_off = a.embed;
    int in_dim = a.in_dim;
    const int vocab = a.V;
    tape.push_back([=]() {
      if (!emb->g) return;
      if (live()) chk(s2st_embed_bwd(prev_tok, emb->g, G + embed_off, B * L, in_dim, scale, 1, st_, ordered_sums ? vocab : 0));
    });
    Ten* x = emb;
    if (a.proj_in >= 0) x = linear(x, a.proj_in, -1, a.d, a.in_dim);
    const char* who = &a == &asr ? "asr" : (&a == &st ? "st" : "s2t");
    snprintf(site_ctx, sizeof site_ctx, "%s.pe", who);
// ... 11 lines not shown
```

### speech-to-speech-translation_amd/csrc/engine_step.h

```cpp
  bool use_streamk = s2st_env_on("S2ST_GEMM_STREAMK");
  void reset_call() {
    pending_wgrad.clear();
    pending_lnfold = s2st_lnfold_table{};
    s2st_gemm_streamk_unbind_all();
    for (Ten* t : tens) delete t;
    tens.clear();
    tape.clear();
    tape_aware.clear();
    forked_ = false;
    in_region_ = false;
    marks.clear();
    ws_top = 0;
    ws_peak = 0;
    oom = false;
    err = 0;
    site = 0;
    site_log.clear();
    xattn0_idx = 0;
    tail_bwd_on_side = tail_side_ = dec_early_active = false;
    site_ctx[0] = 0;
    param_watermark = 0;
    next_segment = 0;
    skws = nullptr; skws_n = 0; skws_side = nullptr;
  }
// ... 112 lines not shown
      const uint64_t site0 = site;
      const long wm0 = param_watermark;
      const size_t t0 = tape.size(), l0 = site_log.size();
      early.site_first = site0;
      early.site_lo = site = site0 + n_enc_sites;
      if (live()) { st_ = fork_side(); dec_early_active = st_ == side_; }
      Ten* prev = newT(B * D, c.out_dim, const_cast<float*>(bt.prev));
      prev->needs_grad = false;
      early.y = dec_front(prev);
      early.n_front = tape.size() - t0;
      early.wm_front = param_watermark;
      set_ctx("dec.L%d", 0);
      early.head = dec_head(early.y, dec[0], B, D, c.dec_heads, c.dec_pre_ln != 0, bt.tgt_lens);
      early.wm_head = param_watermark;
      early.site_hi = site;
      early.tape.assign(std::make_move_iterator(tape.begin() + t0), std::make_move_iterator(tape.end()));
      tape.resize(t0);
      if (tape_aware.size() > t0) tape_aware.resize(t0);
      early.log.assign(site_log.begin() + l0, site_log.end());
      site_log.resize(l0);
      site = site0;
      param_watermark = wm0;
      site_ctx[0] = 0;
      if (live()) hipEventRecord(ev_head_, st_);
      st_ = main_st;
    }

    mark();
    Ten* x = nullptr;
    if (c.text_input) {
      Ten* emb = newT(B * E, C);
      touch(enc_embed + (long)c.src_vocab * C);
      if (live()) chk(s2st_embed_fwd((const long*)bt.src_txt, P + enc_embed, emb->d, B * E, C, 1.f, st_));
      const long eoff = enc_embed;
      tape.push_back([=]() {
        if (!emb->g) return;
        if (live()) chk(s2st_embed_bwd((const long*)bt.src_txt, emb->g, G + eoff, B * E, C, 1.f, 1, st_, ordered_sums ? c.src_vocab : 0));
      });
      set_ctx("enc.prenet");
      Ten* pn = text_prenet(emb, B, E, tr, cst);
      Ten* pj = linear(pn, enc_prenet_proj.w, enc_prenet_proj.b, C, C);
      set_ctx("enc.pe");
      x = add_pe(pj, bt.enc_pos, pe_enc, 1.f, enc_pos_alpha, tr ? c.dropout : 0.f);
    } else {
    float* xh0 = fm ? nullptr : alloc((long)B * (S + 2 * pad) * c.in_dim, true);
    if (live() && !fm) {
      Split xs{(long)c.in_dim, 0, 0, 0};
      Split ys{(long)c.in_dim, (long)(S + 2 * pad) * c.in_dim, S, 0};
      chk(s2st_copy_rows(bt.src, xs, xh0 + (long)pad * c.in_dim, ys, B * S, c.in_dim, st_));
    }
    const bf16raw* xh0h = fm ? cast_halo(bt.src, B, S, pad, c.in_dim, true) : nullptr;
    Ten* z1 = conv(ConvIn{xh0, nullptr, S, xh0h}, sub[0], B, 2, cs0);
    const int C1 = c.conv_channels / 2;
    float* g1h = alloc((long)B * (T1 + 2 * pad) * C1, !fm);
    Ten* g1 = glu_to(z1, g1h + (long)pad * C1, Split{(long)C1, (long)(T1 + 2 * pad) * C1, T1, 0}, C1);
    const bf16raw* g1hh = fm ? cast_halo(g1h, B, T1, pad, C1) : nullptr;
    Ten* z2 = conv(ConvIn{g1h, g1, T1, g1hh}, sub[1], B, 2, cs1);
    float* x0d = alloc((long)B * E * C);
    Ten* x0 = glu_to(z2, x0d, Split{(long)C, 0, 0, 0}, C);
    set_ctx("enc.pe");
    x = add_pe(x0, bt.enc_pos, pe_enc, c.no_scale_embedding ? 1.f : sqrtf((float)C), -1,
                    tr ? c.dropout : 0.f, enc_spk, E);
    }
    mark();
    Ten *tap_asr = nullptr, *tap_st = nullptr;
    in_region_ = two_chains;
    for (int i = 0; i < c.enc_layers; ++i) {
      set_ctx("enc.L%d", i);
      x = enc_layer(x, enc[i], B, E);
      if (i == c.tap_asr) tap_asr = x;
      if (i == c.tap_st) tap_st = x;
      if (i % 3 == 2) mark();
    }
    const bool t2s_spk = c.text_input && enc_spk >= 0 && bt.speaker != nullptr;
    Ten* enc_out = has_enc_ln ? layernorm(x, enc_ln, t2s_spk ? nullptr : outs.enc_out) : x;
    in_region_ = false;
    if (live()) sync_chains();
    if (t2s_spk) {
      const int Sd = c.spk_dim;
      Ten* cat = newT(B * E, C + Sd);
      Ten* xin = enc_out;
      touch_spk(enc_spk + (long)c.n_speakers * Sd);
      if (live()) {
        chk(s2st_copy_rows(xin->d, Split{(long)C, 0, 0, 0}, cat->d, Split{(long)(C + Sd), 0, 0, 0}, B * E, C, st_));
        chk(s2st_speaker_fill_cols(spk_tab(enc_spk), (const long*)bt.speaker, cat->d, B, E, C + Sd, C, Sd, st_));
      }
      const long soff = enc_spk;
      tape.push_back([=]() {
        if (!cat->g) return;
        if (!c.spk_frozen && live())
          chk(s2st_speaker_cols_bwd(cat->g, (const long*)bt.speaker, B, E, C + Sd, C, Sd, c.n_speakers, G + soff, st_));
        if (xin->needs_grad) {
          bool acc;
          float* dx = gradbuf(xin, acc);
          if (live()) chk(s2st_split_cols(cat->g, C + Sd, dx, C, B * E, C, acc ? 1 : 0, st_));
        }
      });
      enc_out = linear(cat, enc_spk_proj.w, enc_spk_proj.b, C, C + Sd, 0, 0.f, nullptr, outs.enc_out);
    } else if (!has_enc_ln && outs.enc_out && live())
      hipMemcpyAsync(outs.enc_out, x->d, sizeof(float) * (size_t)x->n(), hipMemcpyDeviceToDevice, st_);
    if (!c.has_asr && tap_asr && outs.tap0 && live())
      hipMemcpyAsync(outs.tap0, tap_asr->d, sizeof(float) * (size_t)tap_asr->n(), hipMemcpyDeviceToDevice, st_);
    if (c.has_asr && tap_asr) tap_asr = layernorm(tap_asr, asr_norm, outs.tap0);
    if (c.has_st && tap_st) tap_st = layernorm(tap_st, st_norm, outs.tap1);
    const bool aux_on_side = side_ && ev_taps_ && live() && overlap_aux && !(c.text_input && c.has_ctc);
    const bool kv_on_side = side_ && ev_taps_ && ev_kv_ && live() && hoist_kv && !stop_after_encoder;
    if (aux_on_side || kv_on_side) hipEventRecord(ev_taps_, st_);
    aux_wait_idx = tape.size();
    mark();
// ... 120 lines not shown
    float* ctc_per = (with_loss && c.has_ctc) ? alloc(B) : nullptr;
    float *ctc_lp = nullptr, *ctc_ws = nullptr, *ctc_dl = nullptr;
    if (with_loss && c.has_ctc && ctc_logits) {
      ctc_lp = (outs.ctc_lprobs && !t2s_ctc) ? outs.ctc_lprobs : alloc((long)B * ctc_T * c.src_vocab);
      ctc_ws = alloc(s2st_ctc_workspace_floats(B, ctc_T, bt.Ls));
      ctc_dl = tr ? alloc(ctc_logits->n()) : nullptr;
      if (live()) {
        hipStream_t cs = aux_on_side ? st_ : fork_side();
        chk(s2st_ctc(ctc_logits->d, (const long*)bt.src_txt, bt.Ls, ctc_ilens, bt.src_txt_lens, B, ctc_T,
                     c.src_vocab, ctc_lp, ctc_per, ctc_dl, ctc_dl ? c.ctc_weight / B : 0.f, ctc_ws, cs));
      }
    }
    Ten *asr_logits = nullptr, *st_logits = nullptr;
    if (c.has_asr && tap_asr && bt.prev_src_txt)
      asr_logits = aux_decoder(asr, tap_asr, (const long*)bt.prev_src_txt, bt.src_txt_pos, bt.src_txt_lens, B,
                               bt.Ls, pe_asr, outs.asr_logits);
    if (c.has_st && tap_st && bt.prev_tgt_txt)
      st_logits = aux_decoder(st, tap_st, (const long*)bt.prev_tgt_txt, bt.tgt_txt_pos, bt.tgt_txt_lens, B,
                              bt.Lt, pe_st, outs.st_logits);
    st_ = main_st;
    aux_hi_idx = tape.size();
    aux_bwd_on_side = aux_on_side && tr;
    mark();
    if (with_loss) {
      float* stats = outs.stats;
      const float nr = (float)bt.ntokens, nf = nr * c.out_dim;
      float* loss_ws = alloc(3L * S2ST_LOSS_ORDERED_FLOATS);
      if (live()) {
        hipMemsetAsync(stats, 0, sizeof(float) * 32, st_);
        s2st_loss_parts lp{};
        float* ow[3] = {nullptr, nullptr, nullptr};
        if (ordered_sums)
          for (int q = 0; q < 3; ++q) lp.part[q] = ow[q] = loss_ws + (long)q * S2ST_LOSS_ORDERED_FLOATS;
        chk(s2st_mel_loss(feat->d, post->d, eos->d, bt.tgt, bt.tgt_lens, B, D, c.out_dim, c.bce_pos_weight,
                          stats + S2ST_STAT_L1_SUM, 0, 0, 0, nullptr, nullptr, nullptr, st_, ow[0], &lp.nblocks[0]));
        join_side();
        if (asr_logits)
          chk(s2st_ls_ce(asr_logits->d, (const long*)bt.src_txt, B * bt.Ls, c.src_vocab, 1, c.label_smoothing,
                         stats + S2ST_STAT_ASR_NLL, nullptr, 0.f, st_, ow[1], &lp.nblocks[1]));
        if (st_logits)
          chk(s2st_ls_ce(st_logits->d, (const long*)bt.tgt_txt, B * bt.Lt, c.tgt_vocab, 1, c.label_smoothing,
                         stats + S2ST_STAT_ST_NLL, nullptr, 0.f, st_, ow[2], &lp.nblocks[2]));
        chk(s2st_loss_finalize(stats, ctc_per, B, nf, nr, c.w_l1, c.w_mse, c.w_eos, c.ctc_weight,
                               c.asr_weight, c.st_weight, c.label_smoothing, c.src_vocab, c.tgt_vocab,
                               (float)bt.src_txt_ntokens, (float)bt.tgt_txt_ntokens, st_, ctc_tgt_per, c.ctc_tgt_weight,
                               ordered_sums ? &lp : nullptr));
      }
      tape.push_back([=]() {
        const float gs = gscale;
        bool a1, a2, a3;
        float* dfeat = gradbuf(feat, a1);
        float* dpost = gradbuf(post, a2);
        float* deos = gradbuf(eos, a3);
        if (live())
          chk(s2st_mel_loss(feat->d, post->d, eos->d, bt.tgt, bt.tgt_lens, B, D, c.out_dim, c.bce_pos_weight,
                            nullptr, gs * c.w_l1 / nf, gs * c.w_mse / nf, gs * c.w_eos / nr, dfeat, dpost, deos,
                            st_));
        if (ctc_logits) {
          bool a;
          float* dl = gradbuf(ctc_logits, a);
          if (live()) {
            if (ctc_dl) chk(s2st_dropout(ctc_dl, dl, ctc_logits->n(), gs, 0.f, 0, 0, st_));
            else
              chk(s2st_ctc(ctc_logits->d, (const long*)bt.src_txt, bt.Ls, ctc_ilens, bt.src_txt_lens, B, ctc_T,
                           c.src_vocab, ctc_lp, ctc_per, dl, gs * c.ctc_weight / B, ctc_ws, st_));
          }
        }
        if (ctc_tgt_logits && ctc_tgt_dl) {
          bool a;
          float* dl = gradbuf(ctc_tgt_logits, a);
          if (live()) chk(s2st_dropout(ctc_tgt_dl, dl, ctc_tgt_logits->n(), gs, 0.f, 0, 0, st_));
        }
        if (asr_logits) {
          bool a;
          float* dl = gradbuf(asr_logits, a);
          if (live())
            chk(s2st_ls_ce(asr_logits->d, (const long*)bt.src_txt, B * bt.Ls, c.src_vocab, 1, c.label_smoothing,
                           nullptr, dl, gs * c.asr_weight / (float)bt.src_txt_ntokens, st_));
        }
        if (st_logits) {
          bool a;
          float* dl = gradbuf(st_logits, a);
          if (live())
            chk(s2st_ls_ce(st_logits->d, (const long*)bt.tgt_txt, B * bt.Lt, c.tgt_vocab, 1, c.label_smoothing,
                           nullptr, dl, gs * c.st_weight / (float)bt.tgt_txt_ntokens, st_));
        }
      });
    }
    if (adam_pending && live()) adam_wait_all(st_);
    join_side();
    mark();
    return err;
  }

  int forward_s2t(Ten* enc_out, bool with_loss) {
    const int B = bt.B;
    if (!bt.prev_src_txt || bt.Ls <= 0) return err;
    Ten* logits = aux_decoder(s2t, enc_out, (const long*)bt.prev_src_txt, bt.src_txt_pos, bt.src_txt_lens, B, bt.Ls,
                              bt.pe_asr, outs.asr_logits);
    mark();
    if (with_loss && bt.src_txt) {
      float* stats = outs.stats;
      float* loss_ws = alloc(3L * S2ST_LOSS_ORDERED_FLOATS);
      if (live()) {
        hipMemsetAsync(stats, 0, sizeof(float) * 32, st_);
        s2st_loss_parts lp{};
        float* ow = nullptr;
        if (ordered_sums) lp.part[1] = ow = loss_ws + S2ST_LOSS_ORDERED_FLOATS;
        chk(s2st_ls_ce(logits->d, (const long*)bt.src_txt, B * bt.Ls, c.tgt_vocab, 1, c.label_smoothing,
                       stats + S2ST_STAT_ASR_NLL, nullptr, 0.f, st_, ow, &lp.nblocks[1]));
// ... 54 lines not shown
```

### speech-to-speech-translation_amd/csrc/losses.hip

```cpp
#include "s2st_ops.h"
#include "s2st_prof.h"

namespace {

__device__ __forceinline__ float softplusf_(float x) {
  return fmaxf(x, 0.f) + log1pf(expf(-fabsf(x)));
}

__device__ __forceinline__ void block_stats_out(float* __restrict__ stats, int K, const float (*red)[4],
                                                float* __restrict__ ordered) {
  const int tid = threadIdx.x;
  if (tid >= K) return;
  const float v = red[tid][0] + red[tid][1] + red[tid][2] + red[tid][3];
  if (ordered) ordered[(long)tid * gridDim.x + blockIdx.x] = v;
  else atomicAdd(&stats[tid], v);
}

__global__ __launch_bounds__(256) void mel_loss_kernel(
    const float* __restrict__ feat, const float* __restrict__ post, const float* __restrict__ eos,
    const float* __restrict__ tgt, const int* __restrict__ lens, int B, int D, int F,
    float pos_weight, float* __restrict__ stats, float c_l1, float c_mse, float c_eos,
    float* __restrict__ dfeat, float* __restrict__ dpost, float* __restrict__ deos, float* __restrict__ ordered) {
  __shared__ float red[3][4];
  const long n = (long)B * D * F;
  float a1 = 0.f, a2 = 0.f, a3 = 0.f;
  for (long i = (long)blockIdx.x * 256 + threadIdx.x; i < n; i += (long)gridDim.x * 256) {
    long row = i / F;
    int f = (int)(i - row * F);
    int b = (int)(row / D), t = (int)(row - (long)b * D);
    int len = lens[b];
    bool valid = t < len;
    float gt = tgt[i];
    float e1 = feat[i] - gt, e2 = post[i] - gt;
    if (valid) {
      a1 += fabsf(e1) + fabsf(e2);
      a2 += e1 * e1 + e2 * e2;
    }
    if (dfeat) {
      float s1 = e1 > 0.f ? 1.f : (e1 < 0.f ? -1.f : 0.f);
      float s2 = e2 > 0.f ? 1.f : (e2 < 0.f ? -1.f : 0.f);
      dfeat[i] = valid ? c_l1 * s1 + c_mse * 2.f * e1 : 0.f;
      dpost[i] = valid ? c_l1 * s2 + c_mse * 2.f * e2 : 0.f;
    }
    if (f == 0) {
      float x = eos[row];
      float y = (t == len - 1) ? 1.f : 0.f;
      if (valid) a3 += pos_weight * y * softplusf_(-x) + (1.f - y) * softplusf_(x);
      if (deos) {
        float sg = 1.f / (1.f + expf(-x));
        deos[row] = valid ? c_eos * (-pos_weight * y * (1.f - sg) + (1.f - y) * sg) : 0.f;
      }
    }
  }
  if (stats) {
    a1 = wave_sum(a1); a2 = wave_sum(a2); a3 = wave_sum(a3);
    int w = threadIdx.x >> 6;
    if ((threadIdx.x & 63) == 0) { red[0][w] = a1; red[1][w] = a2; red[2][w] = a3; }
    __syncthreads();
    block_stats_out(stats, 3, red, ordered);
  }
}

__global__ __launch_bounds__(256) void ls_ce_kernel(const float* __restrict__ logits,
                                                    const long* __restrict__ target, int rows,
                                                    int V, long pad, float eps,
                                                    float* __restrict__ stats,
                                                    float* __restrict__ dlogits, float gscale,
                                                    float* __restrict__ ordered) {
  __shared__ float red[4][4];
  const int lane = threadIdx.x & 63, wave = threadIdx.x >> 6;
  float nll_a = 0.f, sm_a = 0.f, cor_a = 0.f, tot_a = 0.f;
  const float eps_i = eps / (float)(V - 1);
  for (int row = blockIdx.x * 4 + wave; row < rows; row += gridDim.x * 4) {
    const float* x = logits + (long)row * V;
    const long tg = target[row];
    float mx = -INFINITY;
    int am = 0;
    for (int c = lane; c < V; c += 64) {
      float v = x[c];
      if (v > mx) { mx = v; am = c; }
    }
#pragma unroll
    for (int m = 32; m >= 1; m >>= 1) {
      float ov = __shfl_xor(mx, m);
      int oi = __shfl_xor(am, m);
      if (ov > mx || (ov == mx && oi < am)) { mx = ov; am = oi; }
    }
    float se = 0.f, sx = 0.f;
    for (int c = lane; c < V; c += 64) {
      se += expf(x[c] - mx);
      sx += x[c];
    }
    se = wave_sum(se);
    sx = wave_sum(sx);
    const float lse = logf(se) + mx;
// ... 228 lines not shown
    ctc = w_ctc * ctc / (float)B;
  }
  float ctc_tgt = 0.f;
  if (ctc_tgt_per) {
    for (int b = 0; b < B; ++b) ctc_tgt += ctc_tgt_per[b];
    ctc_tgt = w_ctc_tgt * ctc_tgt / (float)B;
  }
  float asr = 0.f, st = 0.f;
  if (w_asr > 0.f && src_ntok > 0.f) {
    float ei = eps / (float)(Vs - 1);
    asr = w_asr * ((1.f - eps - ei) * stats[S2ST_STAT_ASR_NLL] + ei * stats[S2ST_STAT_ASR_SMOOTH]) / src_ntok;
  }
  if (w_st > 0.f && tgt_ntok > 0.f) {
    float ei = eps / (float)(Vt - 1);
    st = w_st * ((1.f - eps - ei) * stats[S2ST_STAT_ST_NLL] + ei * stats[S2ST_STAT_ST_SMOOTH]) / tgt_ntok;
  }
  stats[S2ST_STAT_L1] = l1;
  stats[S2ST_STAT_MSE] = mse;
  stats[S2ST_STAT_EOS] = eos;
  stats[S2ST_STAT_CTC] = ctc;
  stats[S2ST_STAT_ASR] = asr;
  stats[S2ST_STAT_ST] = st;
  stats[S2ST_STAT_CTC_TGT] = ctc_tgt;
  stats[S2ST_STAT_LOSS] = l1 + mse + eos + ctc + ctc_tgt + asr + st;
}

__global__ __launch_bounds__(256) void log_softmax_rows_kernel(const float* __restrict__ x, long ldx, float* __restrict__ y,
                                                               long ldy, int rows, int V, int log_out) {
  const int lane = threadIdx.x & 63;
  const int row = blockIdx.x * 4 + (threadIdx.x >> 6);
  if (row >= rows) return;
  const float* xr = x + (long)row * ldx;
  float mx = -INFINITY;
  for (int c = lane; c < V; c += 64) mx = fmaxf(mx, xr[c]);
  mx = wave_max(mx);
  float s = 0.f;
  for (int c = lane; c < V; c += 64) s += expf(xr[c] - mx);
  s = wave_sum(s);
  const float ls = logf(s);
  float* yr = y + (long)row * ldy;
  for (int c = lane; c < V; c += 64) {
    const float v = xr[c] - mx - ls;
    yr[c] = log_out ? v : expf(v);
  }
}

}

#define LAUNCH_OK() (hipGetLastError() == hipSuccess ? 0 : S2ST_ERR_LAUNCH)

int s2st_mel_loss(const float* feat, const float* post, const float* eos, const float* tgt,
                  const int* lens, int B, int D, int F, float pos_weight, float* stats, float c_l1,
                  float c_mse, float c_eos, float* dfeat, float* dpost, float* deos,
                  hipStream_t st, float* ordered, int* nblocks_out) {
  long n = (long)B * D * F;
  if (n <= 0) return 0;
  long blocks = (n + 256 * 4 - 1) / (256 * 4);
  if (blocks > 2048) blocks = 2048;
  S2ST_LAUNCH(mel_loss_kernel, dim3((unsigned)blocks), dim3(256), 0, st, feat, post, eos, tgt,
                     lens, B, D, F, pos_weight, stats, c_l1, c_mse, c_eos, dfeat, dpost, deos, ordered);
  if (nblocks_out) *nblocks_out = (int)blocks;
  return LAUNCH_OK();
}

int s2st_ls_ce(const float* logits, const long* target, int rows, int V, long pad, float eps,
               float* stats, float* dlogits, float gscale, hipStream_t st, float* ordered, int* nblocks_out) {
  if (rows <= 0) return 0;
  int blocks = (rows + 3) / 4;
  if (blocks > 1024) blocks = 1024;
  S2ST_LAUNCH(ls_ce_kernel, dim3(blocks), dim3(256), 0, st, logits, target, rows, V, pad, eps,
                     stats, dlogits, gscale, ordered);
  if (nblocks_out) *nblocks_out = blocks;
  return LAUNCH_OK();
}

long s2st_ctc_workspace_floats(int B, int E, int Lmax) {
  long ss = ((2L * Lmax + 1 + 3) / 4) * 4;
  return 2L * B * E * ss + B;
}

int s2st_ctc(const float* logits, const long* targets, int Lmax, const int* in_lens,
             const int* tgt_lens, int B, int E, int V, float* lprobs, float* loss_per_utt,
             float* dlogits, float gscale, float* ws, hipStream_t st) {
  if (B <= 0) return 0;
  if (2 * Lmax + 1 > CTC_MAXS || V > CTC_MAXV || E <= 0) return S2ST_ERR_SHAPE;
  const int S = 2 * Lmax + 1, ss = ((S + 3) / 4) * 4;
  float* ll = ws + 2L * B * E * ss;
  S2ST_LAUNCH(log_softmax_rows_kernel, dim3((B * E + 3) / 4), dim3(256), 0, st, logits, (long)V, lprobs, (long)V, B * E, V, 1);
  const unsigned lds_ab = (unsigned)(ss * 5 * 4);
#define CTC_AB(PER) S2ST_LAUNCH(ctc_ab_kernel<PER>, dim3(B), dim3(256), lds_ab, st, lprobs, targets, Lmax, in_lens, tgt_lens, E, V, ws, ss, ll, loss_per_utt)
  if (S <= 256) CTC_AB(2);
  else if (S <= 512) CTC_AB(4);
  else CTC_AB(16);
#undef CTC_AB
  if (dlogits) {
    const unsigned lds_g = (unsigned)(ss * (4 * 4 + 4 + 2) + (V + 1) * 4 + 16);
    S2ST_LAUNCH(ctc_grad_kernel, dim3((E + CTC_FR - 1) / CTC_FR, B), dim3(256), lds_g, st, lprobs, targets, Lmax, in_lens,
                tgt_lens, E, V, ws, ss, ll, dlogits, gscale);
  }
  return LAUNCH_OK();
}

int s2st_loss_finalize(float* stats, const float* ctc_per, int B, float nf, float nr, float w_l1,
                       float w_mse, float w_eos, float w_ctc, float w_asr, float w_st, float eps, int Vs,
                       int Vt, float src_ntok, float tgt_ntok, hipStream_t st, const float* ctc_tgt_per, float w_ctc_tgt,
                       const s2st_loss_parts* parts) {
  s2st_loss_parts pt{};
  if (parts) { pt = *parts; pt.on = 1; }
  S2ST_LAUNCH(loss_finalize_kernel, dim3(1), dim3(parts ? 256 : 64), 0, st, stats, ctc_per, B, nf, nr, w_l1, w_mse,
                     w_eos, w_ctc, w_asr, w_st, eps, Vs, Vt, src_ntok, tgt_ntok, ctc_tgt_per, w_ctc_tgt, pt);
  return LAUNCH_OK();
}

// ... 6 lines not shown
```

### speech-to-speech-translation_amd/csrc/s2st_ops.h

```cpp
#pragma once
#include <cstdlib>
static inline const char* s2st_env_str(const char* name) { return getenv(name); }
static inline int s2st_env_int(const char* name, int dflt) { const char* e = getenv(name); return e ? atoi(e) : dflt; }
static inline bool s2st_env_on(const char* name) { return s2st_env_int(name, 0) != 0; }

#include <hip/hip_runtime.h>
#include <stdint.h>
#include "s2st_common.h"

typedef s2st_gemm_operand GemmOperand;
typedef s2st_gemm_out GemmOut;
typedef s2st_gemm_epilogue GemmEpilogue;
typedef s2st_gemm_args GemmArgs;

inline GemmOperand gemm_rowmajor(const float* p, long ld) {
  GemmOperand o;
  o.p = p; o.kmajor = 1; o.dtype = S2ST_F32; o.sp.ld = ld; o.sp.bs = 0; o.sp.per = 0; o.sp._pad = 0;
  o.zo = o.zi = 0;
  return o;
}
inline GemmOperand gemm_colmajor(const float* p, long ld) {
  GemmOperand o = gemm_rowmajor(p, ld);
  o.kmajor = 0;
  return o;
// ... 64 lines not shown
#define S2ST_LNFOLD_MAX 24
struct s2st_lnfold_item { const float* part; float *dgamma, *dbeta, *dbias; int nblocks, cols, nout; const float* part2; int nblocks2; };
struct s2st_lnfold_table { int n; int blk0[S2ST_LNFOLD_MAX + 1]; s2st_lnfold_item item[S2ST_LNFOLD_MAX]; };
int s2st_lnfold_add(s2st_lnfold_table& t, const float* part, int rows, int cols, int nout, float* dgamma, float* dbeta,
                    float* dbias);
int s2st_layernorm_bwd_fold(const s2st_lnfold_table& t, hipStream_t st);
int s2st_fold_add(s2st_lnfold_table& t, const float* part, int nblocks, int cols, int nout, float* out0, float* out1,
                  float* out2);
int s2st_layernorm_bwd(const float* dy, const float* x, const float* gamma, const float* mean,
                       const float* rstd, float* dx, int dx_accumulate, float* dgamma,
                       float* dbeta, float* scratch, int rows, int cols, hipStream_t st, int phase = 0,
                       uint16_t* dph = nullptr, float drop_p = 0.f, uint64_t seed = 0, float* dbias = nullptr);

int s2st_softmax_fwd(const float* s, float* p, float* pd, const int* klen, int B, int H, int T,
                     int S, int ld, int causal, float drop_p, uint64_t seed, hipStream_t st,
                     uint16_t* pdh = nullptr );
int s2st_softmax_bwd(const float* p, const float* dpd, float* ds, int B, int H, int T, int S,
                     int ld, float drop_p, uint64_t seed, hipStream_t st,
                     uint16_t* dsh = nullptr );

int s2st_colsum(const float* x, long ld, int rows, int cols, float* out, int accumulate,
                hipStream_t st, float* part = nullptr ,
                int* slabs_out = nullptr );
long s2st_colsum_scratch_floats(int rows, int cols);
int s2st_colsum_fold(const float* part, int slabs, int cols, float* out, hipStream_t st);
int s2st_colsum_bf16(const uint16_t* x, long ld, int rows, int cols, float* out, hipStream_t st);
long s2st_colsum_bf16_scratch_floats(int rows, int cols);
int s2st_colsum_bf16_ordered(const uint16_t* x, long ld, int rows, int cols, float* out, float* scratch, hipStream_t st);
int s2st_attn_headmean(const float* p, float* out, int B, int H, int T, int S, int ld,
                       hipStream_t st);

int s2st_cast_bf16_rows(const float* x, long ldx, uint16_t* y, long ldy, long rows, int cols, hipStream_t st);
int s2st_grad_pack_bf16(const float* g, uint16_t* out, long n, hipStream_t st);
int s2st_exchange_proxy(const float* bucket, float* scratch, long n, long move_bytes, int wgs, float gbps, hipStream_t st);
int s2st_grad_unpack_bf16(const uint16_t* in, float* g, long n, hipStream_t st);
int s2st_transpose_bf16(const uint16_t* x, uint16_t* y, int R, int C, hipStream_t st);
#define S2ST_TRANSPOSE_MAX 200
struct s2st_transpose_table {
  int n;
  unsigned off[S2ST_TRANSPOSE_MAX];
  unsigned short rows8[S2ST_TRANSPOSE_MAX], cols8[S2ST_TRANSPOSE_MAX];
  unsigned tile0[S2ST_TRANSPOSE_MAX + 1];
};
int s2st_transpose_bf16_batched(const uint16_t* x_base, uint16_t* y_base, const s2st_transpose_table& t, hipStream_t st);
int s2st_copy_rows_bf16(const uint16_t* x, Split xsp, uint16_t* y, Split ysp, int rows, int C, hipStream_t st);
int s2st_cast_bf16_halo(const float* x, uint16_t* y, int B, int T, int pad, int C, hipStream_t st, int plain = 0);
int s2st_halo_image_bf16(const uint16_t* x, long ldx, uint16_t* y, int B, int Tout, int Th, int O, int pad, int stride,
                         hipStream_t st);
int s2st_copy_rows(const float* x, Split xsp, float* y, Split ysp, int rows, int C,
                   hipStream_t st);
int s2st_glu_fwd(const float* a, float* y, Split ysp, int rows, int C, hipStream_t st);
int s2st_glu_bwd(const float* a, const float* dy, Split dysp, float* da, Split dasp, int rows,
                 int C, hipStream_t st, uint16_t* dah = nullptr , long ldh = 0);
int s2st_add_pe(const float* x, float* y, const int* pos, const float* table, int rows, int C,
                float scale, const float* alpha_ptr, float drop_p, uint64_t seed, hipStream_t st,
                const float* spk_table = nullptr, const long* spk_ids = nullptr, int T = 0);
int s2st_speaker_bwd(const float* dy, const long* ids, int B, int T, int T_sum, int C, int n_spk, float drop_p,
                     uint64_t seed, float* dtable, hipStream_t st);
int s2st_speaker_fill_cols(const float* table, const long* ids, float* y, int B, int T, int ld, int coff, int Sd, hipStream_t st);
int s2st_speaker_cols_bwd(const float* dy, const long* ids, int B, int T, int ld, int coff, int Sd, int n_spk, float* dtable,
                          hipStream_t st);
int s2st_split_cols(const float* g, int ldg, float* dx, int ldx, int rows, int C, int acc, hipStream_t st);
int s2st_speaker_set_rows(const float* table, const long* ids, float* y, int B, int T, int C, hipStream_t st);
int s2st_pe_alpha_bwd(const float* dy, const int* pos, const float* table, int rows, int C,
                      float drop_p, uint64_t seed, float* dalpha, hipStream_t st,
                      float* part = nullptr ,
                      int* nparts_out = nullptr);
int s2st_embed_fwd(const long* tokens, const float* table, float* y, int rows, int C, float scale,
                   hipStream_t st);
int s2st_embed_bwd(const long* tokens, const float* dy, float* dtable, int rows, int C, float scale,
                   long pad, hipStream_t st, int V = 0 );
int s2st_dropout(const float* x, float* y, long n, float a, float p, uint64_t seed, int accumulate,
                 hipStream_t st);
int s2st_relu_drop_bwd(const float* dy, const float* y, float* dz, long n, float p,
                       hipStream_t st);
int s2st_linear_bwd_prep(const float* dy, const float* y, const uint16_t* yb , int mode,
                         float p, uint64_t seed, uint16_t* dph, long ldp, float* dpre, float* dbias, int M, int N,
                         hipStream_t st, float* part = nullptr ,
                         int* slabs_out = nullptr );
long s2st_linear_bwd_prep_scratch_floats(int M, int N, long ldp);
int s2st_axpy(const float* x, float* y, long n, float a, hipStream_t st);
int s2st_scale(float* x, long n, float a, hipStream_t st);
int s2st_conv_w_permute(const float* w, float* wf, float* wd, int O, int I, int Kw, hipStream_t st,
                        uint16_t* wfh = nullptr, uint16_t* wdh = nullptr );
int s2st_conv_w_unpermute_acc(const float* dwf, float* dw, int O, int I, int Kw, hipStream_t st, int slabs = 1);
int s2st_bn_stats(const float* x, int rows, int C, float* mean, float* var, float* run_mean,
                  float* run_var, float momentum, float* tmp, hipStream_t st);
int s2st_bn_apply(const float* x, const float* mean, const float* var, const float* gamma,
                  const float* beta, float* y, Split ysp, const float* resid, int rows, int C,
                  float eps, int tanh_, float drop_p, uint64_t seed, hipStream_t st);
int s2st_bn_apply_img(const float* x, const float* mean, const float* var, const float* gamma, const float* beta, float* y,
                      uint16_t* img, int B, int T, int pad, int C, float eps, int tanh_, float drop_p, uint64_t seed,
                      hipStream_t st);
int s2st_bn_bwd(const float* dy, Split dysp, const float* x, const float* mean, const float* var,
                const float* gamma, const float* beta, float* dx, Split dxsp, float* dgamma,
                float* dbeta, float* tmp, int rows, int C, float eps, int tanh_, float drop_p,
                uint64_t seed, hipStream_t st, uint16_t* dxh = nullptr ,
                long ldh = 0);

int s2st_flash_attn_supported(int dh);
int s2st_flash_attn_preload(hipStream_t st);
int s2st_flash_attn_fwd(const s2st_attn_args* p, hipStream_t st);
int s2st_flash_attn_bwd(const s2st_attn_args* p, const float* dO, float* dvec_scratch, hipStream_t st, int phase = 0,
                        float* db_part = nullptr );
long s2st_flash_attn_db_scratch_floats(const s2st_attn_args* p);
void s2st_flash_attn_db_layout(const s2st_attn_args* p, int* slots_q, int* slots_k);
int s2st_flash_attn_db_fold(const s2st_attn_args* p, const float* db_part, hipStream_t st);

int s2st_hubert_conv0_gn_gelu(const float* x, const float* w, const float* gamma, const float* beta, float* y,
                              uint16_t* yh, float* stats , int B, int N, int T, int C, int k,
                              int stride, float eps, hipStream_t st);
long s2st_hubert_conv0_stats_floats(int B, int T, int C);
int s2st_posconv_prep(float* x, const int* lens, float* img, uint16_t* imgh, int B, int T, int E, int G, int pad,
                      int Tp, hipStream_t st);

int s2st_w2v_wave_norm(const float* x, const int* lens, float* y, int B, int N, float eps, hipStream_t st);
int s2st_w2v_conv0_ln_gelu(const float* x, const float* w, const float* bias, const float* gamma, const float* beta, float* y,
                           uint16_t* yh, int B, int N, int T, int C, int k, int stride, float eps, hipStream_t st);
int s2st_w2v_ln_gelu_rows(const float* x, const float* gamma, const float* beta, float* y, uint16_t* yh, int rows, int C,
                          float eps, hipStream_t st);
int s2st_w2v_ctc_greedy(const float* logits, const int* lens, int* ids, int* counts, int B, int T, int V, int blank,
                        hipStream_t st);
int s2st_resample_sinc(const float* x, const int* n_in, const float* table, float* y, int B, int N_in, int N_out, int L, int M,
                       int KL, int KW, hipStream_t st);

int s2st_fbank_kaldi(const float* wave, const int* len, const float* win, const float* tw, const float* banks, const int* range,
                     float* out, int* offs, int U, int Lmax, int size, int shift, int padded, int n_bins, float eps, long n_pairs,
                     long out_rows, hipStream_t st);
int s2st_logmel(const float* wave, const int* len, const float* win, const float* tw, const float* mel, const int* range,
                float* out, int* offs, int U, int Lmax, int n_fft, int hop, int n_mels, float eps, long n_pairs, long out_rows,
                hipStream_t st);
int s2st_logmel_frame_split(const float* wave, const int* len, uint16_t* As, int* offs, int U, int Lmax, int n_fft, int hop,
                            long rows, hipStream_t st);
int s2st_logmel_from_stft(const float* Y, const float* mel, const int* range, float* out, long rows, int F, int Fp, int n_mels,
                          float eps, hipStream_t st);
int s2st_feature_moments(const float* feats, const int* offs, float* mom, int U, int n_bins, hipStream_t st);

struct s2st_hifigan_conv_args {
  const void* in;
  const void* w;
  const float* bias;
  const float* resid;
  float* out;
  void* img;
  const int* frames;
  int B, cin, lin, cout, lout, nq, ntap, dil, up, off[8];
// ... 8 lines not shown

int s2st_decode_attn(const float* q, long ldq, float* kc, float* vc, long ldk, long kbs, const int* klen,
                     int nkeys, int B, int H, int dh, float scale, float* o, long ldo, float* attn_mean, int S,
                     hipStream_t st, const float* k_new = nullptr, const float* v_new = nullptr, long ld_new = 0,
                     int pos_new = 0, int kv_bf16 = 0,
                     const int* step_ptr = nullptr);
int s2st_scale_rows(const float* x, const float* a, float* y, long n, hipStream_t st);
int s2st_cache_reorder(const float* src, float* dst, const int* idx, int nb, int Bb, long row_floats, long valid_floats, hipStream_t st);
int s2st_decode_stop_update(const float* eos_prob, float thr, int step, int max_iter, int B, int* finished, int* out_lens,
                            int* klen_next, int* n_done, hipStream_t st);
int s2st_decode_replay_init(int* step, uint64_t* seeds, float* cur_feat, long n_feat, float* pe_cur, const float* pe_alpha, int Cd,
                            uint64_t seed0, hipStream_t st);
int s2st_decode_replay_commit(int* step, uint64_t* seeds, const float* cur_feat, const float* cur_eos, const float* cur_attn,
                              float* pe_cur, const float* pe_alpha, int pe_rows, int Cd, uint64_t seed0, float thr, int max_iter,
                              int B, int out_dim, int E, int* finished, int* out_lens, int* klen_next, int* n_done,
                              float* feat_all, float* eos_all, float* attn_all, hipStream_t st);
int s2st_sigmoid(const float* x, float* y, long n, hipStream_t st);
int s2st_argmax_dim1(const float* x, long* idx, int B, int E, int D, hipStream_t st);
int s2st_affine_cols(const float* x, const float* scale, const float* shift, float* y, long rows, int C, hipStream_t st);
int s2st_exp_transpose(const float* x, float* y, int T, int C, hipStream_t st);
int s2st_clamp_min(float* x, long n, float lo, hipStream_t st);
int s2st_gl_polar(const float* mag, const float* ang, float* X, int F, int T, hipStream_t st);
int s2st_gl_project(const float* mag, const float* Y, float* X, int F, int T, hipStream_t st);
int s2st_reflect_pad(const float* x, float* y, int n, int pad, hipStream_t st);
int s2st_gl_polar_split(const float* mag, const float* aux, int from_spectrum, const int* tl, uint16_t* Xs, int U, int F,
                        int Fp, int Tmax, hipStream_t st);
int s2st_gl_frame_split(const float* wave, const int* tl, uint16_t* As, int U, int Tmax, int hop, int n_fft, int Lw,
                        hipStream_t st);
int s2st_gl_overlap_add_b(const float* frames, const float* wsq_all, const long* wsq_off, const int* tl, float* wave,
                          int U, int Tmax, int n_fft, int hop, int Lw, hipStream_t st);
bool s2st_gl_fft_supported(int n_fft);
int s2st_gl_polar_c(const float* mag, const float* ang, const int* tl, float* X, int U, int F, int Tmax, hipStream_t st);
int s2st_exp_inplace(float* x, long n, hipStream_t st);
int s2st_gl_polar_u(const float* mag, const double* uni, const long* uoff, const int* tl, uint64_t seed, float* X, int U, int F,
                    int Tmax, hipStream_t st);
int s2st_gl_stft_project(const float* wave, const int* tl, const float* win, const float* tw, const float* mag, float* X, int U,
                         int Tmax, int n_fft, int hop, int Lw, hipStream_t st);
int s2st_gl_istft_ola(const float* X, const int* tl, const float* win, const float* tw, const float* wsq_all, const long* wsq_off,
                      float* wave, int U, int Tmax, int n_fft, int hop, int Lw, hipStream_t st);
int s2st_gl_istft_frames(const float* X, const int* tl, const float* win, const float* tw, float* frames, int U, int Tmax,
                         int n_fft, int hop, hipStream_t st);
int s2st_gl_overlap_add(const float* frames, const float* wsq, float* wave, int T, int n_fft, int hop, int n_out,
                        hipStream_t st);

int s2st_dtw(const float* dist, const int* shapes, int B, int M, int N, float* cum, int* backptr, int* pathmap,
             hipStream_t st);
int s2st_rms_dist(const float* x1, const float* x2, float* out, int m, int n, int D, long ldo, hipStream_t st);
int s2st_power_spec(const float* Y, float* P, int T, int F, hipStream_t st);
int s2st_log_offset(float* x, long n, float eps, hipStream_t st);

int s2st_mel_loss(const float* feat, const float* post, const float* eos, const float* tgt,
                  const int* lens, int B, int D, int F, float pos_weight, float* stats, float c_l1,
                  float c_mse, float c_eos, float* dfeat, float* dpost, float* deos,
                  hipStream_t st, float* ordered = nullptr, int* nblocks_out = nullptr);
#define S2ST_LOSS_ORDERED_FLOATS (4 * 2048)
struct s2st_loss_parts {
  const float* part[3];
  int nblocks[3];
  int on;
};
int s2st_ls_ce(const float* logits, const long* target, int rows, int V, long pad, float eps,
               float* stats, float* dlogits, float gscale, hipStream_t st, float* ordered = nullptr,
               int* nblocks_out = nullptr);
long s2st_ctc_workspace_floats(int B, int E, int Lmax);
int s2st_ctc(const float* logits, const long* targets, int Lmax, const int* in_lens,
             const int* tgt_lens, int B, int E, int V, float* lprobs, float* loss_per_utt,
             float* dlogits, float gscale, float* ws, hipStream_t st);

int s2st_log_softmax_rows(const float* x, long ldx, float* y, long ldy, int rows, int V, int log_out, hipStream_t st);
int s2st_loss_finalize(float* stats, const float* ctc_per, int B, float nf, float nr, float w_l1,
                       float w_mse, float w_eos, float w_ctc, float w_asr, float w_st, float eps, int Vs,
                       int Vt, float src_ntok, float tgt_ntok, hipStream_t st, const float* ctc_tgt_per = nullptr,
                       float w_ctc_tgt = 0.f, const s2st_loss_parts* parts = nullptr);

int s2st_sumsq(const float* x, long n, float* out , hipStream_t st);
#define S2ST_SUMSQ_PARTS 1024
int s2st_sumsq_parts(const float* x, long n, float* parts, hipStream_t st);
long s2st_sumsq_nparts(long n);
int s2st_adam(float* p, float* g, float* m, float* v, long n, const float* sumsq, float gmul,
              const float* gmul_dev, float max_norm, float lr, float beta1, float beta2, float eps, float wd, int step,
              float* gnorm_out, hipStream_t st, uint16_t* p_bf16 = nullptr ,
              int* skipped = nullptr ,
              int sumsq_parts = 0 ,
              int zero_grad = 0 );
```

Before: 1.477 million mel-frames/s.

## Fuse conv-subsampler and postnet elementwise ops into bf16 halo-image producers

Adds kernels that write GLU outputs and gradients straight into padded bf16 halo images for the next conv, fuses BN stats finalize with apply and with backward, and folds the postnet residual gradient into the mel loss kernel. Attention forward can now skip its fp32 output when only the bf16 copy is needed. Together these are meant to cut separate cast/halo and reduction launches and the fp32 intermediate traffic in the conv front-end and postnet. The fused paths depend on the convnet_fuse flag and shape conditions, and add more code paths whose correctness must match the unfused ones.

```diff
diff --git a/include/s2st_hip.h b/include/s2st_hip.h
--- a/include/s2st_hip.h
+++ b/include/s2st_hip.h
@@ -129,6 +129,27 @@
 int s2st_bn_apply_f32(const float* x, const float* mean, const float* var, const float* gamma, const float* beta, float* y, s2st_split ysp, const float* resid, int32_t rows, int32_t C, float eps, int32_t tanh_, float drop_p, uint64_t seed, void* stream);
 
 int s2st_bn_bwd_f32(const float* dy, s2st_split dysp, const float* x, const float* mean, const float* var, const float* gamma, const float* beta, float* dx, s2st_split dxsp, float* dgamma, float* dbeta, float* tmp, int32_t rows, int32_t C, float eps, int32_t tanh_, float drop_p, uint64_t seed, void* stream);
+
+int s2st_bn_apply_img_f32(const float* x, const float* mean, const float* var, const float* gamma, const float* beta, float* y, uint16_t* img, int32_t B, int32_t T, int32_t pad, int32_t C, float eps, int32_t tanh_, float drop_p, uint64_t seed, void* stream);
+
+int s2st_bn_stats_apply_f32(const float* x, int32_t rows, int32_t C, float* mean, float* var, float* run_mean, float* run_var, float momentum, float* tmp, const float* gamma, const float* beta, float* y, s2st_split ysp, const float* resid, float eps, int32_t tanh_, float drop_p, uint64_t seed, void* stream);
+int s2st_bn_stats_apply_img_f32(const float* x, int32_t B, int32_t T, int32_t pad, int32_t C, float* mean, float* var, float* run_mean, float* run_var, float momentum, float* tmp, const float* gamma, const float* beta, float* y, uint16_t* img, float eps, int32_t tanh_, float drop_p, uint64_t seed, void* stream);
+
+int s2st_bn_bwd_twin_f32(const float* dy, s2st_split dysp, const float* x, const float* mean, const float* var, const float* gamma, const float* beta, float* dx, s2st_split dxsp, float* dgamma, float* dbeta, float* tmp, int32_t rows, int32_t C, float eps, int32_t tanh_, float drop_p, uint64_t seed, uint16_t* dxh, int64_t ldh, void* stream);
+
+int s2st_bn_bwd_fused_f32(const float* dy, s2st_split dysp, const float* x, const float* mean, const float* var, const float* gamma, const float* beta, float* dx, s2st_split dxsp, float* dgamma, float* dbeta, float* tmp, int32_t B, int32_t T, int32_t pad, int32_t C, float eps, int32_t tanh_, float drop_p, uint64_t seed, uint16_t* dxh, int64_t ldh, uint16_t* img, void* stream);
+
+int s2st_halo_image_bf16_f32(const uint16_t* x, int64_t ldx, uint16_t* y, int32_t B, int32_t Tout, int32_t Th, int32_t O, int32_t pad, int32_t stride, void* stream);
+
+int s2st_cast_bf16_halo_f32(const float* x, uint16_t* y, int32_t B, int32_t T, int32_t pad, int32_t C, int32_t plain, void* stream);
+
+int s2st_glu_fwd_img_f32(const float* a, uint16_t* img, int32_t B, int32_t T, int32_t pad, int32_t C, void* stream);
+
+int s2st_glu_bwd_twin_f32(const float* a, const float* dy, s2st_split dysp, float* da, s2st_split dasp, int32_t rows, int32_t C, uint16_t* dah, int64_t ldh, void* stream);
+
+int s2st_glu_bwd_img_f32(const float* a, const float* dy, s2st_split dysp, float* da, s2st_split dasp, int32_t B, int32_t Tout, int32_t Th, int32_t pad, int32_t stride, int32_t C, uint16_t* dah, int64_t ldh, uint16_t* img, void* stream);
+
+int s2st_mel_loss_resid_f32(const float* feat, const float* post, const float* eos, const float* tgt, const int32_t* lens, int32_t B, int32_t D, int32_t F, float pos_weight, float c_l1, float c_mse, float c_eos, float* dfeat, float* dpost, float* deos, void* stream);
 
 int s2st_mel_loss_f32(const float* feat, const float* post, const float* eos, const float* tgt, const int32_t* lens, int32_t B, int32_t D, int32_t F, float pos_weight, float* stats, float c_l1, float c_mse, float c_eos, float* dfeat, float* dpost, float* deos, void* stream);
 
diff --git a/speech-to-speech-translation_amd/csrc/attention.hip b/speech-to-speech-translation_amd/csrc/attention.hip
--- a/speech-to-speech-translation_amd/csrc/attention.hip
+++ b/speech-to-speech-translation_amd/csrc/attention.hip
@@ -263,7 +263,7 @@
 #pragma unroll
     for (int d = 0; d < DT; ++d) {
       const float4 v = make_float4(o[d][0] * inv_l, o[d][1] * inv_l, o[d][2] * inv_l, o[d][3] * inv_l);
-      *reinterpret_cast<float4*>(a.o + ro + 16 * d + 4 * g) = v;
+      if (a.o) *reinterpret_cast<float4*>(a.o + ro + 16 * d + 4 * g) = v;
       if (a.oh) *reinterpret_cast<uint2*>(a.oh + ro + 16 * d + 4 * g) = pack_bf16x4(v.x, v.y, v.z, v.w);
     }
     if (g == 0 && a.lse) a.lse[(long)bh * a.T + qi] = l > 0.f ? m + __logf(l) : -INFINITY;
@@ -844,7 +844,7 @@
 #pragma unroll
     for (int d = 0; d < DT; ++d) {
       const float4 v = make_float4(o[d][0] * inv_l, o[d][1] * inv_l, o[d][2] * inv_l, o[d][3] * inv_l);
-      *reinterpret_cast<float4*>(a.o + ro + 16 * d + 4 * g) = v;
+      if (a.o) *reinterpret_cast<float4*>(a.o + ro + 16 * d + 4 * g) = v;
       if (a.oh) *reinterpret_cast<uint2*>(a.oh + ro + 16 * d + 4 * g) = pack_bf16x4(v.x, v.y, v.z, v.w);
     }
     if (g == 0 && a.lse) a.lse[(long)bh * a.T + qi] = l > 0.f ? m + __logf(l) : -INFINITY;
@@ -923,7 +923,7 @@
 }
 
 int s2st_flash_attn_fwd(const s2st_attn_args* p, hipStream_t st) {
-  if (!p || !attn_args_ok(*p) || !p->o || !p->lse) return S2ST_ERR_ARG;
+  if (!p || !attn_args_ok(*p) || (!p->o && !p->oh) || !p->lse) return S2ST_ERR_ARG;
   AttnArgs a = to_args(*p);
   if (p->T <= SHORT_MAX && p->S <= SHORT_MAX && short_fwd_enabled() && short_configure()) {
     const double fl = 4.0 * p->B * p->H * (double)p->T * p->S * p->dh * (p->causal ? 0.5 : 1.0);
diff --git a/speech-to-speech-translation_amd/csrc/c_api.cpp b/speech-to-speech-translation_amd/csrc/c_api.cpp
--- a/speech-to-speech-translation_amd/csrc/c_api.cpp
+++ b/speech-to-speech-translation_amd/csrc/c_api.cpp
@@ -126,6 +126,50 @@
 
 int s2st_bn_bwd_f32(const float* dy, s2st_split dysp, const float* x, const float* mean, const float* var, const float* gamma, const float* beta, float* dx, s2st_split dxsp, float* dgamma, float* dbeta, float* tmp, int32_t rows, int32_t C, float eps, int32_t tanh_, float drop_p, uint64_t seed, void* stream) {
   return s2st_bn_bwd(dy, dysp, x, mean, var, gamma, beta, dx, dxsp, dgamma, dbeta, tmp, rows, C, eps, tanh_, drop_p, seed, (hipStream_t)stream);
+}
+
+int s2st_bn_apply_img_f32(const float* x, const float* mean, const float* var, const float* gamma, const float* beta, float* y, uint16_t* img, int32_t B, int32_t T, int32_t pad, int32_t C, float eps, int32_t tanh_, float drop_p, uint64_t seed, void* stream) {
+  return s2st_bn_apply_img(x, mean, var, gamma, beta, y, img, B, T, pad, C, eps, tanh_, drop_p, seed, (hipStream_t)stream);
+}
+
+int s2st_bn_stats_apply_f32(const float* x, int32_t rows, int32_t C, float* mean, float* var, float* run_mean, float* run_var, float momentum, float* tmp, const float* gamma, const float* beta, float* y, s2st_split ysp, const float* resid, float eps, int32_t tanh_, float drop_p, uint64_t seed, void* stream) {
+  return s2st_bn_stats_apply(x, rows, C, mean, var, run_mean, run_var, momentum, tmp, gamma, beta, y, ysp, resid, eps, tanh_, drop_p, seed, (hipStream_t)stream);
+}
+
+int s2st_bn_stats_apply_img_f32(const float* x, int32_t B, int32_t T, int32_t pad, int32_t C, float* mean, float* var, float* run_mean, float* run_var, float momentum, float* tmp, const float* gamma, const float* beta, float* y, uint16_t* img, float eps, int32_t tanh_, float drop_p, uint64_t seed, void* stream) {
+  return s2st_bn_stats_apply_img(x, B, T, pad, C, mean, var, run_mean, run_var, momentum, tmp, gamma, beta, y, img, eps, tanh_, drop_p, seed, (hipStream_t)stream);
+}
+
+int s2st_bn_bwd_twin_f32(const float* dy, s2st_split dysp, const float* x, const float* mean, const float* var, const float* gamma, const float* beta, float* dx, s2st_split dxsp, float* dgamma, float* dbeta, float* tmp, int32_t rows, int32_t C, float eps, int32_t tanh_, float drop_p, uint64_t seed, uint16_t* dxh, int64_t ldh, void* stream) {
+  return s2st_bn_bwd(dy, dysp, x, mean, var, gamma, beta, dx, dxsp, dgamma, dbeta, tmp, rows, C, eps, tanh_, drop_p, seed, (hipStream_t)stream, dxh, (long)ldh);
+}
+
+int s2st_bn_bwd_fused_f32(const float* dy, s2st_split dysp, const float* x, const float* mean, const float* var, const float* gamma, const float* beta, float* dx, s2st_split dxsp, float* dgamma, float* dbeta, float* tmp, int32_t B, int32_t T, int32_t pad, int32_t C, float eps, int32_t tanh_, float drop_p, uint64_t seed, uint16_t* dxh, int64_t ldh, uint16_t* img, void* stream) {
+  return s2st_bn_bwd_fused(dy, dysp, x, mean, var, gamma, beta, dx, dxsp, dgamma, dbeta, tmp, B, T, pad, C, eps, tanh_, drop_p, seed, (hipStream_t)stream, dxh, (long)ldh, img);
+}
+
+int s2st_halo_image_bf16_f32(const uint16_t* x, int64_t ldx, uint16_t* y, int32_t B, int32_t Tout, int32_t Th, int32_t O, int32_t pad, int32_t stride, void* stream) {
+  return s2st_halo_image_bf16(x, (long)ldx, y, B, Tout, Th, O, pad, stride, (hipStream_t)stream);
+}
+
+int s2st_cast_bf16_halo_f32(const float* x, uint16_t* y, int32_t B, int32_t T, int32_t pad, int32_t C, int32_t plain, void* stream) {
+  return s2st_cast_bf16_halo(x, y, B, T, pad, C, (hipStream_t)stream, plain);
+}
+
+int s2st_glu_fwd_img_f32(const float* a, uint16_t* img, int32_t B, int32_t T, int32_t pad, int32_t C, void* stream) {
+  return s2st_glu_fwd_img(a, img, B, T, pad, C, (hipStream_t)stream);
+}
+
+int s2st_glu_bwd_twin_f32(const float* a, const float* dy, s2st_split dysp, float* da, s2st_split dasp, int32_t rows, int32_t C, uint16_t* dah, int64_t ldh, void* stream) {
+  return s2st_glu_bwd(a, dy, dysp, da, dasp, rows, C, (hipStream_t)stream, dah, (long)ldh);
+}
+
+int s2st_glu_bwd_img_f32(const float* a, const float* dy, s2st_split dysp, float* da, s2st_split dasp, int32_t B, int32_t Tout, int32_t Th, int32_t pad, int32_t stride, int32_t C, uint16_t* dah, int64_t ldh, uint16_t* img, void* stream) {
+  return s2st_glu_bwd_img(a, dy, dysp, da, dasp, B, Tout, Th, pad, stride, C, (hipStream_t)stream, dah, (long)ldh, img);
+}
+
+int s2st_mel_loss_resid_f32(const float* feat, const float* post, const float* eos, const float* tgt, const int32_t* lens, int32_t B, int32_t D, int32_t F, float pos_weight, float c_l1, float c_mse, float c_eos, float* dfeat, float* dpost, float* deos, void* stream) {
+  return s2st_mel_loss(feat, post, eos, tgt, lens, B, D, F, pos_weight, nullptr, c_l1, c_mse, c_eos, dfeat, dpost, deos, (hipStream_t)stream, nullptr, nullptr, 1);
 }
 
 int s2st_mel_loss_f32(const float* feat, const float* post, const float* eos, const float* tgt, const int32_t* lens, int32_t B, int32_t D, int32_t F, float pos_weight, float* stats, float c_l1, float c_mse, float c_eos, float* dfeat, float* dpost, float* deos, void* stream) {
diff --git a/speech-to-speech-translation_amd/csrc/elementwise.hip b/speech-to-speech-translation_amd/csrc/elementwise.hip
--- a/speech-to-speech-translation_amd/csrc/elementwise.hip
+++ b/speech-to-speech-translation_amd/csrc/elementwise.hip
@@ -164,6 +164,63 @@
     dah[(long)r * ldh + c] = (uint16_t)(pk & 0xffffu);
     dah[(long)r * ldh + c + C] = (uint16_t)(pk >> 16);
   }
+}
+
+__global__ __launch_bounds__(256) void glu_fwd_img_kernel(const float* __restrict__ a, uint16_t* __restrict__ img, int B, int T,
+                                                          int pad, int C4) {
+  const long i = (long)blockIdx.x * EW_BLOCK + threadIdx.x;
+  const int Th = T + 2 * pad;
+  if (i >= (long)B * Th * C4) return;
+  const int c = (int)(i % C4) * 4;
+  const long bu = i / C4;
+  const int u = (int)(bu % Th), b = (int)(bu / Th);
+  uint2 h = make_uint2(0u, 0u);
+  if (u >= pad && u < pad + T) {
+    const float* ar = a + ((long)b * T + (u - pad)) * (8L * C4);
+    const float4 v = *reinterpret_cast<const float4*>(ar + c), w = *reinterpret_cast<const float4*>(ar + c + 4 * C4);
+    h = pack_bf16x4(v.x * sigmoidf_(w.x), v.y * sigmoidf_(w.y), v.z * sigmoidf_(w.z), v.w * sigmoidf_(w.w));
+  }
+  reinterpret_cast<uint2*>(img)[i] = h;
+}
+
+__global__ __launch_bounds__(256) void glu_bwd_img_kernel(const float* __restrict__ a, const float* __restrict__ dy, Split dysp,
+                                                          float* __restrict__ da, Split dasp, int B, int Tout, int Th, int pad,
+                                                          int stride, int C4, uint16_t* __restrict__ dah, long ldh,
+                                                          uint16_t* __restrict__ img) {
+  const long i = (long)blockIdx.x * EW_BLOCK + threadIdx.x;
+  if (i >= (long)B * Th * C4) return;
+  const int C = 4 * C4;
+  const int c = (int)(i % C4) * 4;
+  const long bu = i / C4;
+  const int u = (int)(bu % Th), b = (int)(bu / Th);
+  const int d = u - pad;
+  uint2 h0 = make_uint2(0u, 0u), h1 = make_uint2(0u, 0u);
+  if (d >= 0 && d % stride == 0 && d / stride < Tout) {
+    const int r = b * Tout + d / stride;
+    const float* ar = a + (long)r * 2 * C;
+    const float4 av = *reinterpret_cast<const float4*>(ar + c), gv = *reinterpret_cast<const float4*>(ar + c + C);
+    const float4 dv = *reinterpret_cast<const float4*>(dy + split_off(dysp, r) + c);
+    const float as[4] = {av.x, av.y, av.z, av.w}, gt[4] = {gv.x, gv.y, gv.z, gv.w}, gs[4] = {dv.x, dv.y, dv.z, dv.w};
+    float d0[4], d1[4];
+#pragma unroll
+    for (int k = 0; k < 4; ++k) {
+      const float g = gs[k];
+      const float s = sigmoidf_(gt[k]);
+      d0[k] = g * s;
+      d1[k] = g * as[k] * s * (1.f - s);
+    }
+    float* dr = da + split_off(dasp, r);
+    *reinterpret_cast<float4*>(dr + c) = make_float4(d0[0], d0[1], d0[2], d0[3]);
+    *reinterpret_cast<float4*>(dr + c + C) = make_float4(d1[0], d1[1], d1[2], d1[3]);
+    h0 = pack_bf16x4(d0[0], d0[1], d0[2], d0[3]);
+    h1 = pack_bf16x4(d1[0], d1[1], d1[2], d1[3]);
+    if (dah) {
+      *reinterpret_cast<uint2*>(dah + (long)r * ldh + c) = h0;
+      *reinterpret_cast<uint2*>(dah + (long)r * ldh + c + C) = h1;
+    }
+  }
+  *reinterpret_cast<uint2*>(img + bu * (2L * C) + c) = h0;
+  *reinterpret_cast<uint2*>(img + bu * (2L * C) + c + C) = h1;
 }
 
 __global__ __launch_bounds__(256) void add_pe_kernel(const float* __restrict__ x,
@@ -530,6 +587,34 @@
     return make_float2(d, d * d);
   }
 };
+__device__ __forceinline__ float2 fold_slabs_column(const float* __restrict__ part, int slabs, int cols, int c) {
+  float v0[CR_MAX_SLABS], v1[CR_MAX_SLABS];
+#pragma unroll
+  for (int j = 0; j < CR_MAX_SLABS; ++j) {
+    const long s = j < slabs ? j : slabs - 1;
+    v0[j] = part[(s * 2 + 0) * cols + c];
+    v1[j] = part[(s * 2 + 1) * cols + c];
+  }
+  float s0 = 0.f, s1 = 0.f;
+#pragma unroll
+  for (int j = 0; j < CR_MAX_SLABS; ++j)
+    if (j < slabs) { s0 += v0[j]; s1 += v1[j]; }
+  return make_float2(s0, s1);
+}
+__device__ __forceinline__ float2 bn_finalize_column(float s1, float s2, float x0, int rows, float momentum,
+                                                     float* __restrict__ mean, float* __restrict__ var,
+                                                     float* __restrict__ run_mean, float* __restrict__ run_var) {
+  const float d1 = s1 / rows;
+  const float m = x0 + d1;
+  const float v = fmaxf(s2 / rows - d1 * d1, 0.f);
+  if (mean) { *mean = m; *var = v; }
+  if (run_mean) {
+    *run_mean = (1.f - momentum) * *run_mean + momentum * m;
+    float unb = rows > 1 ? v * ((float)rows / (float)(rows - 1)) : v;
+    *run_var = (1.f - momentum) * *run_var + momentum * unb;
+  }
+  return make_float2(m, v);
+}
 __global__ __launch_bounds__(256) void bn_finalize_shift_kernel(const float* __restrict__ x0, const float* __restrict__ part,
                                                                 int slabs, float* __restrict__ mean,
                                                                 float* __restrict__ var, float* __restrict__ run_mean,
@@ -550,16 +635,8 @@
     for (int j = 0; j < 16; ++j)
       if (sb + j < slabs) { s1 += v1[j]; s2 += v2[j]; }
   }
-  const float d1 = s1 / rows;
-  const float m = x0[c] + d1;
-  const float v = fmaxf(s2 / rows - d1 * d1, 0.f);
-  mean[c] = m;
-  var[c] = v;
-  if (run_mean) {
-    run_mean[c] = (1.f - momentum) * run_mean[c] + momentum * m;
-    float unb = rows > 1 ? v * ((float)rows / (float)(rows - 1)) : v;
-    run_var[c] = (1.f - momentum) * run_var[c] + momentum * unb;
-  }
+  bn_finalize_column(s1, s2, x0[c], rows, momentum, mean + c, var + c, run_mean ? run_mean + c : nullptr,
+                     run_mean ? run_var + c : nullptr);
 }
 
 
@@ -610,13 +687,100 @@
   reinterpret_cast<uint2*>(img)[i] = h;
 }
 
+constexpr int BNF_COLS = 64, BNF_ROWS = 64;
+struct BnFoldArgs {
+  const float* x0;
+  const float* part;
+  int slabs, rows;
+  float momentum;
+  float *mean, *var, *run_mean, *run_var;
+};
+__device__ __forceinline__ void bn_fold_prologue(const BnFoldArgs& fa, int C, float (*stat)[BNF_COLS]) {
+  const int c = blockIdx.x * BNF_COLS + threadIdx.x;
+  if (threadIdx.x < BNF_COLS && c < C) {
+    const float2 s = fold_slabs_column(fa.part, fa.slabs, C, c);
+    const bool w = blockIdx.y == 0;
+    const float2 mv = bn_finalize_column(s.x, s.y, fa.x0[c], fa.rows, fa.momentum, w ? fa.mean + c : nullptr,
+                                         w ? fa.var + c : nullptr, (w && fa.run_mean) ? fa.run_mean + c : nullptr,
+                                         (w && fa.run_mean) ? fa.run_var + c : nullptr);
+    stat[0][threadIdx.x] = mv.x;
+    stat[1][threadIdx.x] = mv.y;
+  }
+  __syncthreads();
+}
+
+__global__ __launch_bounds__(256) void bn_apply_fused_kernel(
+    BnFoldArgs fa, const float* __restrict__ x, const float* __restrict__ gamma, const float* __restrict__ beta,
+    float* __restrict__ y, Split ysp, const float* __restrict__ resid, int rows, int C, float eps, int tanh_, float drop_p,
+    uint64_t seed) {
+  __shared__ float stat[2][BNF_COLS];
+  bn_fold_prologue(fa, C, stat);
+  const int tx = threadIdx.x & 63, ty = threadIdx.x >> 6;
+  const int c = blockIdx.x * BNF_COLS + tx;
+  if (c >= C) return;
+  const float mean = stat[0][tx], var = stat[1][tx], ga = gamma[c], be = beta[c];
+  const int r1 = min(rows, (int)(blockIdx.y + 1) * BNF_ROWS);
+  for (int r = blockIdx.y * BNF_ROWS + ty; r < r1; r += 4) {
+    const long i = (long)r * C + c;
+    float u = ga * (x[i] - mean) * rsqrtf(var + eps) + be;
+    if (tanh_ == 1) u = tanhf(u);
+    else if (tanh_ == 2) u = fmaxf(u, 0.f);
+    if (drop_p > 0.f) u *= drop_scale(seed, (uint64_t)i, drop_p, 1.f / (1.f - drop_p));
+    if (resid) u += resid[i];
+    y[split_off(ysp, r) + c] = u;
+  }
+}
+
+__global__ __launch_bounds__(256) void bn_apply_img_fused_kernel(
+    BnFoldArgs fa, const float* __restrict__ x, const float* __restrict__ gamma, const float* __restrict__ beta,
+    float* __restrict__ y, uint16_t* __restrict__ img, int B, int T, int pad, int C, float eps, int tanh_, float drop_p,
+    uint64_t seed) {
+  __shared__ float stat[2][BNF_COLS];
+  bn_fold_prologue(fa, C, stat);
+  const int tx = threadIdx.x & 15, ty = threadIdx.x >> 4;
+  const int c = blockIdx.x * BNF_COLS + 4 * tx;
+  if (c >= C) return;
+  float mean[4], var[4], ga[4], be[4];
+#pragma unroll
+  for (int k = 0; k < 4; ++k) {
+    mean[k] = stat[0][4 * tx + k]; var[k] = stat[1][4 * tx + k];
+    ga[k] = gamma[c + k]; be[k] = beta[c + k];
+  }
+  const int Th = T + 2 * pad;
+  const long nimg = (long)B * Th;
+  const long bu1 = nimg < (long)(blockIdx.y + 1) * BNF_ROWS ? nimg : (long)(blockIdx.y + 1) * BNF_ROWS;
+  for (long bu = (long)blockIdx.y * BNF_ROWS + ty; bu < bu1; bu += 16) {
+    const int u = (int)(bu % Th), b = (int)(bu / Th);
+    uint2 h = make_uint2(0u, 0u);
+    if (u >= pad && u < pad + T) {
+      const long e0 = ((long)b * T + (u - pad)) * C + c;
+      const float4 xv = *reinterpret_cast<const float4*>(x + e0);
+      const float xs[4] = {xv.x, xv.y, xv.z, xv.w};
+      float o[4];
+#pragma unroll
+      for (int k = 0; k < 4; ++k) {
+        float t = ga[k] * (xs[k] - mean[k]) * rsqrtf(var[k] + eps) + be[k];
+        if (tanh_ == 1) t = tanhf(t);
+        else if (tanh_ == 2) t = fmaxf(t, 0.f);
+        if (drop_p > 0.f) t *= drop_scale(seed, (uint64_t)(e0 + k), drop_p, 1.f / (1.f - drop_p));
+        o[k] = t;
+      }
+      if (y) *reinterpret_cast<float4*>(y + e0) = make_float4(o[0], o[1], o[2], o[3]);
+      h = pack_bf16x4(o[0], o[1], o[2], o[3]);
+    }
+    *reinterpret_cast<uint2*>(img + bu * C + c) = h;
+  }
+}
+
 struct BnBwdF {
   const float* dy; Split dysp; const float* x; const float* mean; const float* var;
   const float* gamma; const float* beta; int C; float eps; int tanh_; float drop_p; uint64_t seed;
   __device__ float2 operator()(int r, int c) const {
     long i = (long)r * C + c;
-    float xh = (x[i] - mean[c]) * rsqrtf(var[c] + eps);
-    float g = dy[split_off(dysp, r) + c];
+    return at(x[i], dy[split_off(dysp, r) + c], i, c);
+  }
+  __device__ float2 at(float xv, float g, long i, int c) const {
+    float xh = (xv - mean[c]) * rsqrtf(var[c] + eps);
     if (drop_p > 0.f) g *= drop_scale(seed, (uint64_t)i, drop_p, 1.f / (1.f - drop_p));
     if (tanh_ == 1) {
       float t = tanhf(gamma[c] * xh + beta[c]);
@@ -628,6 +792,14 @@
   }
 };
 
+__device__ __forceinline__ float bn_bwd_dx_value(const BnBwdF& f, float2 v, float xv, int c, float s0, float s1, int rows) {
+  float rstd = rsqrtf(f.var[c] + f.eps);
+  float xh = (xv - f.mean[c]) * rstd;
+  float inv = 1.f / rows;
+  const float t = __builtin_fmaf(-s0, inv, v.x);
+  return f.gamma[c] * rstd * __builtin_fmaf(-(xh * s1), inv, t);
+}
+
 __global__ __launch_bounds__(256) void bn_bwd_dx_kernel(BnBwdF f, const float* __restrict__ sums,
                                                         float* __restrict__ dx, Split dxsp,
                                                         int rows, int C, uint16_t* __restrict__ dxh, long ldh) {
@@ -636,12 +808,57 @@
   if (i >= n) return;
   int r = (int)(i / C), c = (int)(i - (long)r * C);
   float2 v = f(r, c);
-  float rstd = rsqrtf(f.var[c] + f.eps);
-  float xh = (f.x[i] - f.mean[c]) * rstd;
-  float inv = 1.f / rows;
-  const float d = f.gamma[c] * rstd * (v.x - sums[c] * inv - xh * sums[C + c] * inv);
+  const float d = bn_bwd_dx_value(f, v, f.x[i], c, sums[c], sums[C + c], rows);
   dx[split_off(dxsp, r) + c] = d;
   if (dxh) dxh[(long)r * ldh + c] = (uint16_t)(pack_bf16x4(d, 0.f, 0.f, 0.f).x & 0xffffu);
+}
+
+__global__ __launch_bounds__(256) void bn_bwd_dx_fused_kernel(BnBwdF f, const float* __restrict__ part, int slabs,
+                                                              float* __restrict__ dgamma, float* __restrict__ dbeta,
+                                                              float* __restrict__ dx, Split dxsp, int B, int T, int pad,
+                                                              int C, uint16_t* __restrict__ dxh, long ldh,
+                                                              uint16_t* __restrict__ img) {
+  __shared__ float sums[2][BNF_COLS];
+  {
+    const int c = blockIdx.x * BNF_COLS + threadIdx.x;
+    if (threadIdx.x < BNF_COLS && c < C) {
+      const float2 s = fold_slabs_column(part, slabs, C, c);
+      sums[0][threadIdx.x] = s.x;
+      sums[1][threadIdx.x] = s.y;
+      if (blockIdx.y == 0) {
+        if (dbeta) dbeta[c] += s.x;
+        if (dgamma) dgamma[c] += s.y;
+      }
+    }
+    __syncthreads();
+  }
+  const int tx = threadIdx.x & 15, ty = threadIdx.x >> 4;
+  const int c = blockIdx.x * BNF_COLS + 4 * tx;
+  if (c >= C) return;
+  const int rows = B * T, Th = T + 2 * pad;
+  const long nimg = (long)B * Th;
+  const long bu1 = nimg < (long)(blockIdx.y + 1) * BNF_ROWS ? nimg : (long)(blockIdx.y + 1) * BNF_ROWS;
+  for (long bu = (long)blockIdx.y * BNF_ROWS + ty; bu < bu1; bu += 16) {
+    const int u = (int)(bu % Th), b = (int)(bu / Th);
+    uint2 h = make_uint2(0u, 0u);
+    if (u >= pad && u < pad + T) {
+      const int r = b * T + (u - pad);
+      const long e0 = (long)r * C + c;
+      const float4 xv = *reinterpret_cast<const float4*>(f.x + e0);
+      const float4 gv = *reinterpret_cast<const float4*>(f.dy + split_off(f.dysp, r) + c);
+      const float xs[4] = {xv.x, xv.y, xv.z, xv.w}, gs[4] = {gv.x, gv.y, gv.z, gv.w};
+      float d[4];
+#pragma unroll
+      for (int k = 0; k < 4; ++k) {
+        const float2 v = f.at(xs[k], gs[k], e0 + k, c + k);
+        d[k] = bn_bwd_dx_value(f, v, xs[k], c + k, sums[0][4 * tx + k], sums[1][4 * tx + k], rows);
+      }
+      *reinterpret_cast<float4*>(dx + split_off(dxsp, r) + c) = make_float4(d[0], d[1], d[2], d[3]);
+      h = pack_bf16x4(d[0], d[1], d[2], d[3]);
+      if (dxh) *reinterpret_cast<uint2*>(dxh + (long)r * ldh + c) = h;
+    }
+    if (img) *reinterpret_cast<uint2*>(img + bu * C + c) = h;
+  }
 }
 
 __global__ __launch_bounds__(256) void add_vec_kernel(const float* __restrict__ a,
@@ -715,6 +932,28 @@
   long n = (long)rows * C;
   if (n <= 0) return 0;
   S2ST_LAUNCH(glu_fwd_kernel, dim3(ew_grid(n)), dim3(EW_BLOCK), 0, st, a, y, ysp, rows, C);
+  return LAUNCH_OK();
+}
+
+int s2st_glu_fwd_img(const float* a, uint16_t* img, int B, int T, int pad, int C, hipStream_t st) {
+  if (B <= 0 || T <= 0 || C <= 0) return 0;
+  if (C % 4 || pad < 0 || ((uintptr_t)a % 16) || ((uintptr_t)img % 8)) return S2ST_ERR_SHAPE;
+  const long n = (long)B * (T + 2 * pad) * (C / 4);
+  S2ST_LAUNCH(glu_fwd_img_kernel, dim3(ew_grid(n)), dim3(EW_BLOCK), 0, st, a, img, B, T, pad, C / 4);
+  return LAUNCH_OK();
+}
+
+int s2st_glu_bwd_img(const float* a, const float* dy, Split dysp, float* da, Split dasp, int B, int Tout, int Th, int pad,
+                     int stride, int C, hipStream_t st, uint16_t* dah, long ldh, uint16_t* img) {
+  if (B <= 0 || Tout <= 0 || Th <= 0 || C <= 0) return 0;
+  auto sp4 = [](const Split& sp) { return sp.ld % 4 == 0 && sp.bs % 4 == 0; };
+  if (C % 4 || pad < 0 || stride < 1 || pad + (long)stride * (Tout - 1) >= Th || !img || !sp4(dysp) || !sp4(dasp) ||
+      ((uintptr_t)a % 16) || ((uintptr_t)dy % 16) || ((uintptr_t)da % 16) || ((uintptr_t)img % 8) ||
+      (dah && (ldh % 4 || (uintptr_t)dah % 8)))
+    return S2ST_ERR_SHAPE;
+  const long n = (long)B * Th * (C / 4);
+  S2ST_LAUNCH(glu_bwd_img_kernel, dim3(ew_grid(n)), dim3(EW_BLOCK), 0, st, a, dy, dysp, da, dasp, B, Tout, Th, pad, stride, C / 4,
+              dah, ldh, img);
   return LAUNCH_OK();
 }
 
@@ -948,6 +1187,37 @@
   return LAUNCH_OK();
 }
 
+int s2st_bn_stats_apply(const float* x, int rows, int C, float* mean, float* var, float* run_mean, float* run_var,
+                        float momentum, float* tmp, const float* gamma, const float* beta, float* y, Split ysp,
+                        const float* resid, float eps, int tanh_, float drop_p, uint64_t seed, hipStream_t st) {
+  if (rows <= 0 || C <= 0) return 0;
+  int slabs = 0;
+  float* part = tmp + 2 * (long)C;
+  int rc = colreduce2(ShiftSqF{x, C}, rows, C, nullptr, nullptr, part, st, nullptr, nullptr, &slabs);
+  if (rc) return rc;
+  const BnFoldArgs fa{x, part, slabs, rows, momentum, mean, var, run_mean, run_var};
+  S2ST_LAUNCH(bn_apply_fused_kernel, dim3((C + BNF_COLS - 1) / BNF_COLS, (rows + BNF_ROWS - 1) / BNF_ROWS), dim3(256), 0, st,
+              fa, x, gamma, beta, y, ysp, resid, rows, C, eps, tanh_, drop_p, seed);
+  return LAUNCH_OK();
+}
+
+int s2st_bn_stats_apply_img(const float* x, int B, int T, int pad, int C, float* mean, float* var, float* run_mean,
+                            float* run_var, float momentum, float* tmp, const float* gamma, const float* beta, float* y,
+                            uint16_t* img, float eps, int tanh_, float drop_p, uint64_t seed, hipStream_t st) {
+  if (B <= 0 || T <= 0 || C <= 0) return 0;
+  if (C % 4 || pad < 0 || ((uintptr_t)x % 16) || ((uintptr_t)img % 8) || (y && (uintptr_t)y % 16)) return S2ST_ERR_SHAPE;
+  const int rows = B * T;
+  int slabs = 0;
+  float* part = tmp + 2 * (long)C;
+  int rc = colreduce2(ShiftSqF{x, C}, rows, C, nullptr, nullptr, part, st, nullptr, nullptr, &slabs);
+  if (rc) return rc;
+  const BnFoldArgs fa{x, part, slabs, rows, momentum, mean, var, run_mean, run_var};
+  const long nimg = (long)B * (T + 2 * pad);
+  S2ST_LAUNCH(bn_apply_img_fused_kernel, dim3((C + BNF_COLS - 1) / BNF_COLS, (unsigned)((nimg + BNF_ROWS - 1) / BNF_ROWS)),
+              dim3(256), 0, st, fa, x, gamma, beta, y, img, B, T, pad, C, eps, tanh_, drop_p, seed);
+  return LAUNCH_OK();
+}
+
 int s2st_bn_apply(const float* x, const float* mean, const float* var, const float* gamma,
                   const float* beta, float* y, Split ysp, const float* resid, int rows, int C,
                   float eps, int tanh_, float drop_p, uint64_t seed, hipStream_t st) {
@@ -981,3 +1251,25 @@
   S2ST_LAUNCH(bn_bwd_dx_kernel, dim3(ew_grid(n)), dim3(EW_BLOCK), 0, st, f, tmp, dx, dxsp, rows, C, dxh, ldh);
   return LAUNCH_OK();
 }
+
+int s2st_bn_bwd_fused(const float* dy, Split dysp, const float* x, const float* mean, const float* var, const float* gamma,
+                      const float* beta, float* dx, Split dxsp, float* dgamma, float* dbeta, float* tmp, int B, int T, int pad,
+                      int C, float eps, int tanh_, float drop_p, uint64_t seed, hipStream_t st, uint16_t* dxh, long ldh,
+                      uint16_t* img) {
+  if (B <= 0 || T <= 0 || C <= 0) return 0;
+  auto sp4 = [](const Split& sp) { return sp.ld % 4 == 0 && sp.bs % 4 == 0; };
+  if (C % 4 || pad < 0 || !sp4(dysp) || !sp4(dxsp) || ((uintptr_t)x % 16) || ((uintptr_t)dy % 16) || ((uintptr_t)dx % 16) ||
+      (dxh && (ldh % 4 || (uintptr_t)dxh % 8)) || ((uintptr_t)img % 8))
+    return S2ST_ERR_SHAPE;
+  if (!img) pad = 0;
+  const int rows = B * T;
+  BnBwdF f{dy, dysp, x, mean, var, gamma, beta, C, eps, tanh_, drop_p, seed};
+  int slabs = 0;
+  float* part = tmp + 2 * (long)C;
+  int rc = colreduce2(f, rows, C, nullptr, nullptr, part, st, nullptr, nullptr, &slabs);
+  if (rc) return rc;
+  const long nimg = (long)B * (T + 2 * pad);
+  S2ST_LAUNCH(bn_bwd_dx_fused_kernel, dim3((C + BNF_COLS - 1) / BNF_COLS, (unsigned)((nimg + BNF_ROWS - 1) / BNF_ROWS)), dim3(256),
+              0, st, f, (const float*)part, slabs, dgamma, dbeta, dx, dxsp, B, T, pad, C, dxh, ldh, img);
+  return LAUNCH_OK();
+}
diff --git a/speech-to-speech-translation_amd/csrc/engine.cpp b/speech-to-speech-translation_amd/csrc/engine.cpp
--- a/speech-to-speech-translation_amd/csrc/engine.cpp
+++ b/speech-to-speech-translation_amd/csrc/engine.cpp
@@ -27,6 +27,11 @@
   int rows = 0, cols = 0;
   bool needs_grad = true;
   bool want_gh = false;
+  bool gh_only = false;
+  bool img_want = false;
+  int img_B = 0, img_Tout = 0, img_Th = 0, img_pad = 0, img_stride = 1;
+  bf16raw* gimg = nullptr;
+  bool resid_in_loss = false;
   int act_mode = 0;
   float act_p = 0.f;
   long act_bias = -1;
@@ -201,6 +206,8 @@
   bool ordered_sums = true;
   bool use_act_fuse = true;
   bool use_flash = true;
+  bool attn_keep_f32 = s2st_env_on("S2ST_ATTN_KEEP_F32");
+  bool convnet_fuse = s2st_env_int("S2ST_CONVNET_FUSE", 1) != 0;
   int ffn_act = 1;
   bool is_hubert = false;
   s2st_hubert_config hc{};
diff --git a/speech-to-speech-translation_amd/csrc/engine_convnets.h b/speech-to-speech-translation_amd/csrc/engine_convnets.h
--- a/speech-to-speech-translation_amd/csrc/engine_convnets.h
+++ b/speech-to-speech-translation_amd/csrc/engine_convnets.h
@@ -12,6 +12,13 @@
     s.wfh = wfh;
     s.wdh = wdh;
     return s;
+  }
+
+  bool bn_bwd_fusable(const Ten* z, int C) const { return fast() && convnet_fuse && C % 4 == 0 && z->hld() % 4 == 0; }
+  bf16raw* bn_bwd_image(Ten* z, int B, int T) {
+    if (!z->img_want || z->img_stride != 1 || z->img_B != B || z->img_Tout != T || z->img_Th != T + 2 * z->img_pad) return nullptr;
+    z->gimg = alloc_h((long)B * z->img_Th * z->cols);
+    return z->gimg;
   }
 
   Ten* postnet(Ten* feat, int B, int D, bool tr, std::vector<ConvW>& csp, float* post_out) {
@@ -55,11 +62,18 @@
       }
       if (live()) {
         const float *m = BUF + bn.rm, *v = BUF + bn.rv;
-        if (tr) {
+        const bool fuse = tr && fm && convnet_fuse && bn.C % 4 == 0;
+        if (tr && !fuse) {
           chk(s2st_bn_stats(z->d, B * D, bn.C, mean, var, BUF + bn.rm, BUF + bn.rv, 0.1f, bn_tmp, st_));
           m = mean; v = var;
         }
-        if (nexthh)
+        if (fuse && nexthh)
+          chk(s2st_bn_stats_apply_img(z->d, B, D, pp, bn.C, mean, var, BUF + bn.rm, BUF + bn.rv, 0.1f, bn_tmp, P + bn.g, P + bn.b,
+                                      nullptr, nexthh, 1e-5f, 1, pdrop, sd, st_));
+        else if (fuse)
+          chk(s2st_bn_stats_apply(z->d, B * D, bn.C, mean, var, BUF + bn.rm, BUF + bn.rv, 0.1f, bn_tmp, P + bn.g, P + bn.b, out->d,
+                                  osp, last ? feat->d : nullptr, 1e-5f, last ? 0 : 1, pdrop, sd, st_));
+        else if (nexthh)
           chk(s2st_bn_apply_img(z->d, m, v, P + bn.g, P + bn.b, nullptr, nexthh, B, D, pp, bn.C, 1e-5f, 1, pdrop, sd, st_));
         else
           chk(s2st_bn_apply(z->d, m, v, P + bn.g, P + bn.b, out->d, osp, last ? feat->d : nullptr, B * D,
@@ -68,7 +82,7 @@
       BNP bnp = bn;
       tape.push_back([=]() {
         if (!out->g) return;
-        if (last) {
+        if (last && !out->resid_in_loss) {
           bool acc;
           float* df = gradbuf(feat, acc);
           if (live()) chk(s2st_dropout(out->g, df, feat->n(), 1.f, 0.f, 0, acc ? 1 : 0, st_));
@@ -78,7 +92,12 @@
         (void)acc;
         Split ps{(long)bnp.C, 0, 0, 0};
         if (fast() && !z->gh) z->gh = alloc_h((long)z->rows * z->hld());
-        if (live())
+        if (bn_bwd_fusable(z, bnp.C)) {
+          bf16raw* img = bn_bwd_image(z, B, D);
+          if (live())
+            chk(s2st_bn_bwd_fused(out->g, ps, z->d, mean, var, P + bnp.g, P + bnp.b, dz, ps, G + bnp.g, G + bnp.b, bn_tmp, B, D,
+                                  z->img_pad, bnp.C, 1e-5f, last ? 0 : 1, pdrop, sd, st_, z->gh, z->hld(), img));
+        } else if (live())
           chk(s2st_bn_bwd(out->g, ps, z->d, mean, var, P + bnp.g, P + bnp.b, dz, ps, G + bnp.g, G + bnp.b,
                           bn_tmp, B * D, bnp.C, 1e-5f, last ? 0 : 1, pdrop, sd, st_, z->gh, z->hld()));
       });
@@ -131,11 +150,18 @@
       }
       if (live()) {
         const float *m = BUF + bn.rm, *v = BUF + bn.rv;
-        if (tr) {
+        const bool fuse = tr && fm && convnet_fuse && C % 4 == 0;
+        if (tr && !fuse) {
           chk(s2st_bn_stats(z->d, B * T, C, mean, var, BUF + bn.rm, BUF + bn.rv, 0.1f, bn_tmp, st_));
           m = mean; v = var;
         }
-        if (nexthh)
+        if (fuse && nexthh)
+          chk(s2st_bn_stats_apply_img(z->d, B, T, pp, C, mean, var, BUF + bn.rm, BUF + bn.rv, 0.1f, bn_tmp, P + bn.g, P + bn.b,
+                                      nullptr, nexthh, 1e-5f, 2 , pdrop, sd, st_));
+        else if (fuse)
+          chk(s2st_bn_stats_apply(z->d, B * T, C, mean, var, BUF + bn.rm, BUF + bn.rv, 0.1f, bn_tmp, P + bn.g, P + bn.b, out->d,
+                                  osp, nullptr, 1e-5f, 2 , pdrop, sd, st_));
+        else if (nexthh)
           chk(s2st_bn_apply_img(z->d, m, v, P + bn.g, P + bn.b, nullptr, nexthh, B, T, pp, C, 1e-5f, 2 , pdrop, sd, st_));
         else
           chk(s2st_bn_apply(z->d, m, v, P + bn.g, P + bn.b, out->d, osp, nullptr, B * T, C, 1e-5f, 2 , pdrop, sd, st_));
@@ -148,7 +174,12 @@
         (void)acc;
         Split ps{(long)bnp.C, 0, 0, 0};
         if (fast() && !z->gh) z->gh = alloc_h((long)z->rows * z->hld());
-        if (live())
+        if (bn_bwd_fusable(z, bnp.C)) {
+          bf16raw* img = bn_bwd_image(z, B, T);
+          if (live())
+            chk(s2st_bn_bwd_fused(out->g, ps, z->d, mean, var, P + bnp.g, P + bnp.b, dz, ps, G + bnp.g, G + bnp.b, bn_tmp, B, T,
+                                  z->img_pad, bnp.C, 1e-5f, 2, pdrop, sd, st_, z->gh, z->hld(), img));
+        } else if (live())
           chk(s2st_bn_bwd(out->g, ps, z->d, mean, var, P + bnp.g, P + bnp.b, dz, ps, G + bnp.g, G + bnp.b, bn_tmp, B * T,
                           bnp.C, 1e-5f, 2, pdrop, sd, st_, z->gh, z->hld()));
       });
diff --git a/speech-to-speech-translation_amd/csrc/engine_ops.h b/speech-to-speech-translation_amd/csrc/engine_ops.h
--- a/speech-to-speech-translation_amd/csrc/engine_ops.h
+++ b/speech-to-speech-translation_amd/csrc/engine_ops.h
@@ -146,6 +146,7 @@
             g.B = fm ? (has_wt(w, N, K) ? gemm_rowmajor(PHT + w, N) : gemm_colmajor(PH + w, K)) : gemm_colmajor(P + w, K);
             g.C = gemm_out(dx + r0 * x->cols, x->cols);
             if (fm && !acc && x->gh) g.C.h = x->gh + r0 * x->cols;
+            if (fm && !acc && x->gh && x->gh_only) g.C.p = nullptr;
             g.ep = gemm_epi_default();
             if (fuse_act) {
               g.C.p = nullptr;
@@ -261,11 +262,15 @@
     const int C = H * dh;
     const int ld = (S + 7) / 8 * 8;
     const bool fm = fast();
-    Ten* o = newT(B * T, C);
+    const bool flash = fm && use_flash && s2st_flash_attn_supported(dh) && !attn_mean_out && C % 8 == 0 && io.ldq % 8 == 0 &&
+                       io.ldk % 8 == 0 && io.ldv % 8 == 0;
+    const bool skinny_reader = !bt.training && use_skinny && B * T <= S2ST_SKINNY_MAX_ROWS;
+    const bool no_f32 = flash && !attn_keep_f32 && !skinny_reader;
+    Ten* o = newT(B * T, C, nullptr, !no_f32);
     o->want_gh = true;
+    o->gh_only = no_f32;
     if (fm && C % 8 == 0) o->h = alloc_h(o->n());
-    if (fm && use_flash && s2st_flash_attn_supported(dh) && !attn_mean_out && o->h && io.ldq % 8 == 0 &&
-        io.ldk % 8 == 0 && io.ldv % 8 == 0) {
+    if (flash) {
       const uint64_t sd = drop_p > 0.f ? next_seed(S2ST_SITE_ATTN, drop_p, B, H, T, S, ld) : 0;
       float* lse = alloc((long)B * H * T);
       s2st_attn_args fa{};
@@ -276,7 +281,7 @@
       fa.scale = 1.0f / sqrtf((float)dh); fa.drop_p = drop_p; fa.seed = sd; fa.ld_drop = ld;
       auto chain_args = [=](s2st_attn_args a, int b0, int nbat, uint64_t salt) {
         a.q += (long)b0 * T * a.ldq; a.k += (long)b0 * S * a.ldk; a.v += (long)b0 * S * a.ldv;
-        a.o += (long)b0 * T * C; if (a.oh) a.oh += (long)b0 * T * C;
+        if (a.o) a.o += (long)b0 * T * C; if (a.oh) a.oh += (long)b0 * T * C;
         a.lse += (long)b0 * H * T; if (a.klen) a.klen += b0;
         if (a.doh) a.doh += (long)b0 * T * C;
         if (a.dq) a.dq += (long)b0 * T * a.ldq; if (a.dk) a.dk += (long)b0 * S * a.ldk; if (a.dv) a.dv += (long)b0 * S * a.ldv;
@@ -497,6 +502,8 @@
     const int Tin = in.Tin, Tout = (Tin + 2 * pad - p.Kw) / stride + 1;
     const int Th = Tin + 2 * pad;
     Ten* z = newT(B * Tout, p.O);
+    z->img_want = convnet_fuse && fm && p.O % 8 == 0 && in.src && in.src->needs_grad;
+    z->img_B = B; z->img_Tout = Tout; z->img_Th = Th; z->img_pad = pad; z->img_stride = stride;
     touch(p.w + (long)p.O * p.I * p.Kw);
     touch(p.b + p.O);
     if (live()) {
@@ -521,8 +528,9 @@
       const bool direct = fm && pp.O % 8 == 0;
       const bool need_img = !no_dgrad;
       float* up = (need_img && !direct) ? alloc((long)B * Th * pp.O, true) : nullptr;
-      bf16raw* upd = (need_img && direct) ? alloc_h((long)B * Th * pp.O) : nullptr;
-      if (need_img && live()) {
+      const bool have_img = need_img && direct && z->gimg;
+      bf16raw* upd = have_img ? z->gimg : ((need_img && direct) ? alloc_h((long)B * Th * pp.O) : nullptr);
+      if (need_img && !have_img && live()) {
         Split xs{(long)pp.O, 0, 0, 0};
         Split ys{(long)stride * pp.O, (long)Th * pp.O, Tout, 0};
         if (direct) {
@@ -574,9 +582,9 @@
     return z;
   }
 
-  Ten* glu_to(Ten* z, float* y, Split ysp, int Cc) {
-    Ten* holder = newT(z->rows, Cc, y);
-    if (live()) chk(s2st_glu_fwd(z->d, y, ysp, z->rows, Cc, st_));
+  Ten* glu_to(Ten* z, float* y, Split ysp, int Cc, bf16raw* imgh = nullptr, int B = 0, int T = 0, int pad = 0) {
+    Ten* holder = newT(z->rows, Cc, y, y != nullptr);
+    if (live()) chk(imgh ? s2st_glu_fwd_img(z->d, imgh, B, T, pad, Cc, st_) : s2st_glu_fwd(z->d, y, ysp, z->rows, Cc, st_));
     tape.push_back([=]() {
       if (!holder->g) return;
       bool acc;
@@ -584,7 +592,13 @@
       (void)acc;
       Split ds{(long)Cc, 0, 0, 0}, das{(long)2 * Cc, 0, 0, 0};
       if (fast() && !z->gh) z->gh = alloc_h((long)z->rows * z->hld());
-      if (live()) chk(s2st_glu_bwd(z->d, holder->g, ds, dz, das, z->rows, Cc, st_, z->gh, z->hld()));
+      const bool img = fast() && convnet_fuse && z->img_want && Cc % 4 == 0 && z->hld() == z->cols &&
+                       z->rows == z->img_B * z->img_Tout;
+      if (img) z->gimg = alloc_h((long)z->img_B * z->img_Th * z->cols);
+      if (live())
+        chk(img ? s2st_glu_bwd_img(z->d, holder->g, ds, dz, das, z->img_B, z->img_Tout, z->img_Th, z->img_pad, z->img_stride, Cc,
+                                   st_, z->gh, z->hld(), z->gimg)
+                : s2st_glu_bwd(z->d, holder->g, ds, dz, das, z->rows, Cc, st_, z->gh, z->hld()));
     });
     return holder;
   }
diff --git a/speech-to-speech-translation_amd/csrc/engine_step.h b/speech-to-speech-translation_amd/csrc/engine_step.h
--- a/speech-to-speech-translation_amd/csrc/engine_step.h
+++ b/speech-to-speech-translation_amd/csrc/engine_step.h
@@ -188,9 +188,12 @@
     const bf16raw* xh0h = fm ? cast_halo(bt.src, B, S, pad, c.in_dim, true) : nullptr;
     Ten* z1 = conv(ConvIn{xh0, nullptr, S, xh0h}, sub[0], B, 2, cs0);
     const int C1 = c.conv_channels / 2;
-    float* g1h = alloc((long)B * (T1 + 2 * pad) * C1, !fm);
-    Ten* g1 = glu_to(z1, g1h + (long)pad * C1, Split{(long)C1, (long)(T1 + 2 * pad) * C1, T1, 0}, C1);
-    const bf16raw* g1hh = fm ? cast_halo(g1h, B, T1, pad, C1) : nullptr;
+    const bool glu_img = fm && convnet_fuse && C1 % 4 == 0;
+    float* g1h = glu_img ? nullptr : alloc((long)B * (T1 + 2 * pad) * C1, !fm);
+    bf16raw* g1img = glu_img ? alloc_h(((long)B * (T1 + 2 * pad) * C1 + 7) / 8 * 8) : nullptr;
+    Ten* g1 = glu_img ? glu_to(z1, nullptr, Split{(long)C1, 0, 0, 0}, C1, g1img, B, T1, pad)
+                      : glu_to(z1, g1h + (long)pad * C1, Split{(long)C1, (long)(T1 + 2 * pad) * C1, T1, 0}, C1);
+    const bf16raw* g1hh = glu_img ? g1img : (fm ? cast_halo(g1h, B, T1, pad, C1) : nullptr);
     Ten* z2 = conv(ConvIn{g1h, g1, T1, g1hh}, sub[1], B, 2, cs1);
     float* x0d = alloc((long)B * E * C);
     Ten* x0 = glu_to(z2, x0d, Split{(long)C, 0, 0, 0}, C);
@@ -417,10 +420,12 @@
         float* dfeat = gradbuf(feat, a1);
         float* dpost = gradbuf(post, a2);
         float* deos = gradbuf(eos, a3);
+        const bool resid = convnet_fuse && !a1 && !a2;
+        post->resid_in_loss = resid;
         if (live())
           chk(s2st_mel_loss(feat->d, post->d, eos->d, bt.tgt, bt.tgt_lens, B, D, c.out_dim, c.bce_pos_weight,
                             nullptr, gs * c.w_l1 / nf, gs * c.w_mse / nf, gs * c.w_eos / nr, dfeat, dpost, deos,
-                            st_));
+                            st_, nullptr, nullptr, resid ? 1 : 0));
         if (ctc_logits) {
           bool a;
           float* dl = gradbuf(ctc_logits, a);
diff --git a/speech-to-speech-translation_amd/csrc/losses.hip b/speech-to-speech-translation_amd/csrc/losses.hip
--- a/speech-to-speech-translation_amd/csrc/losses.hip
+++ b/speech-to-speech-translation_amd/csrc/losses.hip
@@ -20,7 +20,8 @@
     const float* __restrict__ feat, const float* __restrict__ post, const float* __restrict__ eos,
     const float* __restrict__ tgt, const int* __restrict__ lens, int B, int D, int F,
     float pos_weight, float* __restrict__ stats, float c_l1, float c_mse, float c_eos,
-    float* __restrict__ dfeat, float* __restrict__ dpost, float* __restrict__ deos, float* __restrict__ ordered) {
+    float* __restrict__ dfeat, float* __restrict__ dpost, float* __restrict__ deos, float* __restrict__ ordered,
+    int post_resid) {
   __shared__ float red[3][4];
   const long n = (long)B * D * F;
   float a1 = 0.f, a2 = 0.f, a3 = 0.f;
@@ -39,8 +40,10 @@
     if (dfeat) {
       float s1 = e1 > 0.f ? 1.f : (e1 < 0.f ? -1.f : 0.f);
       float s2 = e2 > 0.f ? 1.f : (e2 < 0.f ? -1.f : 0.f);
-      dfeat[i] = valid ? c_l1 * s1 + c_mse * 2.f * e1 : 0.f;
-      dpost[i] = valid ? c_l1 * s2 + c_mse * 2.f * e2 : 0.f;
+      const float gf = valid ? c_l1 * s1 + c_mse * 2.f * e1 : 0.f;
+      const float gp = valid ? c_l1 * s2 + c_mse * 2.f * e2 : 0.f;
+      dfeat[i] = post_resid ? gf + gp : gf;
+      dpost[i] = gp;
     }
     if (f == 0) {
       float x = eos[row];
@@ -375,13 +378,13 @@
 int s2st_mel_loss(const float* feat, const float* post, const float* eos, const float* tgt,
                   const int* lens, int B, int D, int F, float pos_weight, float* stats, float c_l1,
                   float c_mse, float c_eos, float* dfeat, float* dpost, float* deos,
-                  hipStream_t st, float* ordered, int* nblocks_out) {
+                  hipStream_t st, float* ordered, int* nblocks_out, int post_resid) {
   long n = (long)B * D * F;
   if (n <= 0) return 0;
   long blocks = (n + 256 * 4 - 1) / (256 * 4);
   if (blocks > 2048) blocks = 2048;
   S2ST_LAUNCH(mel_loss_kernel, dim3((unsigned)blocks), dim3(256), 0, st, feat, post, eos, tgt,
-                     lens, B, D, F, pos_weight, stats, c_l1, c_mse, c_eos, dfeat, dpost, deos, ordered);
+                     lens, B, D, F, pos_weight, stats, c_l1, c_mse, c_eos, dfeat, dpost, deos, ordered, post_resid);
   if (nblocks_out) *nblocks_out = (int)blocks;
   return LAUNCH_OK();
 }
diff --git a/speech-to-speech-translation_amd/csrc/s2st_ops.h b/speech-to-speech-translation_amd/csrc/s2st_ops.h
--- a/speech-to-speech-translation_amd/csrc/s2st_ops.h
+++ b/speech-to-speech-translation_amd/csrc/s2st_ops.h
@@ -140,6 +140,9 @@
 int s2st_glu_fwd(const float* a, float* y, Split ysp, int rows, int C, hipStream_t st);
 int s2st_glu_bwd(const float* a, const float* dy, Split dysp, float* da, Split dasp, int rows,
                  int C, hipStream_t st, uint16_t* dah = nullptr , long ldh = 0);
+int s2st_glu_fwd_img(const float* a, uint16_t* img, int B, int T, int pad, int C, hipStream_t st);
+int s2st_glu_bwd_img(const float* a, const float* dy, Split dysp, float* da, Split dasp, int B, int Tout, int Th, int pad,
+                     int stride, int C, hipStream_t st, uint16_t* dah, long ldh, uint16_t* img);
 int s2st_add_pe(const float* x, float* y, const int* pos, const float* table, int rows, int C,
                 float scale, const float* alpha_ptr, float drop_p, uint64_t seed, hipStream_t st,
                 const float* spk_table = nullptr, const long* spk_ids = nullptr, int T = 0);
@@ -180,6 +183,16 @@
 int s2st_bn_apply_img(const float* x, const float* mean, const float* var, const float* gamma, const float* beta, float* y,
                       uint16_t* img, int B, int T, int pad, int C, float eps, int tanh_, float drop_p, uint64_t seed,
                       hipStream_t st);
+int s2st_bn_stats_apply(const float* x, int rows, int C, float* mean, float* var, float* run_mean, float* run_var,
+                        float momentum, float* tmp, const float* gamma, const float* beta, float* y, Split ysp,
+                        const float* resid, float eps, int tanh_, float drop_p, uint64_t seed, hipStream_t st);
+int s2st_bn_stats_apply_img(const float* x, int B, int T, int pad, int C, float* mean, float* var, float* run_mean,
+                            float* run_var, float momentum, float* tmp, const float* gamma, const float* beta, float* y,
+                            uint16_t* img, float eps, int tanh_, float drop_p, uint64_t seed, hipStream_t st);
+int s2st_bn_bwd_fused(const float* dy, Split dysp, const float* x, const float* mean, const float* var, const float* gamma,
+                      const float* beta, float* dx, Split dxsp, float* dgamma, float* dbeta, float* tmp, int B, int T, int pad,
+                      int C, float eps, int tanh_, float drop_p, uint64_t seed, hipStream_t st, uint16_t* dxh, long ldh,
+                      uint16_t* img);
 int s2st_bn_bwd(const float* dy, Split dysp, const float* x, const float* mean, const float* var,
                 const float* gamma, const float* beta, float* dx, Split dxsp, float* dgamma,
                 float* dbeta, float* tmp, int rows, int C, float eps, int tanh_, float drop_p,
@@ -294,7 +307,7 @@
 int s2st_mel_loss(const float* feat, const float* post, const float* eos, const float* tgt,
                   const int* lens, int B, int D, int F, float pos_weight, float* stats, float c_l1,
                   float c_mse, float c_eos, float* dfeat, float* dpost, float* deos,
-                  hipStream_t st, float* ordered = nullptr, int* nblocks_out = nullptr);
+                  hipStream_t st, float* ordered = nullptr, int* nblocks_out = nullptr, int post_resid = 0);
 #define S2ST_LOSS_ORDERED_FLOATS (4 * 2048)
 struct s2st_loss_parts {
   const float* part[3];
```

Result: faster. 1.510 million mel-frames/s (median of 6 runs) (+2.2%).
